# fdrmrc/fictitious_domain_AL_preconditioners

Hardware: AMD Instinct MI355X
Metric: FGMRES iterations/sec to 1e-8 residual, 3D Stokes-immersed (AL-preconditioned) (higher is better)
Workload: dtype f64

## Files before the change

### fictitious_domain_al_preconditioners_amd/_abi.py

```python
import ctypes as C

ALFD_MAX_BLOCKS = 3

OK, E_INVALID, E_HIP, E_NO_CONVERGENCE_OUTER, E_NO_CONVERGENCE_INNER, E_BREAKDOWN, E_NOT_SETUP, \
    E_COMM, E_UNSUPPORTED = range(9)
A, BT, B, CT, C_, M, MP, A2, KIMM = range(9)
NSLOTS = 9
SLOT_BY_NAME = {"A": A, "Bt": BT, "B": B, "Ct": CT, "C": C_, "M": M, "Mp": MP, "A2": A2, "K": KIMM}
INVW, MP_LUMPED_INV = 0, 1
NDIAGS = 2
AL2, AL_STOKES, AL_STOKES_DIAG, AL_ELL_IDEAL, AL_ELL_MODIFIED, RATIONAL = range(6)
CTRL_ABS, CTRL_REDUCTION, CTRL_FIXED_ITERS = range(3)
PREC_IDENTITY, PREC_JACOBI, PREC_CHEBYSHEV, PREC_MULTILEVEL = range(4)
INNER_OP_AUG, INNER_OP_A22, INNER_OP_AUG2 = range(3)
SPECTRUM_CCT = 0
ORTH_MGS, ORTH_CGS, ORTH_CGS2 = range(3)
OUTER_FGMRES, OUTER_MINRES = range(2)
FGMRES_DEALII_96, FGMRES_DEALII_95 = range(2)
W_DIAGONAL, W_MASS_INV_SQUARED, W_MASS_INV = range(3)
INNER_THROW, INNER_ACCEPT = range(2)
T_SPMV_A, T_SPMV_OTHER, T_DOT, T_VEC = range(4)
T_NCLASSES = 4
SC_PRODUCTS_A, SC_PRODUCTS_C, SC_LEVEL_A_UPLOADS, SC_TRANSFER_UPLOADS, SC_PATCH_BUILDS, SC_POWER_ITERATIONS = range(6)
SC_NCOUNTS = 6
# ... 32 lines not shown
class Result(C.Structure):
    _fields_ = [
        ("status", C.c_int32), ("outer_iterations", C.c_int32),
        ("initial_residual", C.c_double), ("last_residual", C.c_double),
        ("inner_iterations", C.c_int64), ("mp_iterations", C.c_int64),
        ("inner_failures", C.c_int32), ("precond_applications", C.c_int32),
        ("solve_seconds", C.c_double), ("lambda_max", C.c_double),
        ("rational_iterations", C.c_int64), ("mass_iterations", C.c_int64),
    ]

    def as_dict(self):
        return {k: getattr(self, k) for k, _ in self._fields_}


class Spectrum(C.Structure):
    _fields_ = [
        ("converged", C.c_int32), ("steps", C.c_int32),
        ("initial_residual", C.c_double), ("last_residual", C.c_double),
        ("lambda_min", C.c_double), ("lambda_max", C.c_double), ("condition", C.c_double),
    ]

    def as_dict(self):
        return {k: getattr(self, k) for k, _ in self._fields_}


class MatrixInfo(C.Structure):
    _fields_ = [
        ("lanes", C.c_int32), ("windowed", C.c_int32), ("value_indexed", C.c_int32), ("batch_major", C.c_int32),
        ("nnz", C.c_int64), ("window_blocks", C.c_int64), ("window_fallback_blocks", C.c_int64),
        ("value_indexed_blocks", C.c_int64), ("value_indexed_nnz", C.c_int64),
        ("dictionary_entries", C.c_int64), ("value_wide_nnz", C.c_int64),
        ("algorithmic_bytes", C.c_double), ("streamed_bytes", C.c_double),
        ("shared_nnz", C.c_int64), ("batch_major_blocks", C.c_int64), ("batch_major_wide", C.c_int64),
        ("batch_major_interior_blocks", C.c_int64),
    ]


SPMV_PLAIN, SPMV_SPARSE_ROWS, SPMV_STREAM, SPMV_WINDOW, SPMV_WINDOW_VI, SPMV_WINDOW_VIB, SPMV_WINDOW_GROUP, \
    SPMV_BATCH_MAJOR, SPMV_BATCH_MAJOR_SHORT, SPMV_PLAIN_F32, SPMV_STREAM_F32, SPMV_WINDOW_F32 = range(12)
SPMV_NFAMILIES = 12
SPMV_FAMILY_NAMES = ("plain", "sparse_rows", "stream", "window", "window_vi", "window_vib", "window_group",
                     "batch_major", "batch_major_short", "plain_f32", "stream_f32", "window_f32")


class SpmvLaunch(C.Structure):
    _fields_ = [
        ("family", C.c_int32), ("lanes", C.c_int32), ("R", C.c_int32), ("U", C.c_int32), ("nontemporal", C.c_int32),
        ("epilogue", C.c_int32), ("xcd_order", C.c_int32),
        ("grid", C.c_int64), ("lds_bytes", C.c_int64),
    ]

    def as_dict(self):
        return {k: getattr(self, k) for k, _ in self._fields_}


class BatchMajorShape(C.Structure):
    _fields_ = [
        ("batch_major", C.c_int32), ("lanes", C.c_int32),
        ("nrows", C.c_int64), ("nnz", C.c_int64), ("shared_nnz", C.c_int64),
        ("rows", C.c_int64), ("waves", C.c_int64), ("small", C.c_int64),
        ("blocks", C.c_int64), ("batches", C.c_int64), ("lds_bytes", C.c_int64), ("compute_units", C.c_int64),
    ]

    def as_dict(self):
        plain = ("batch_major", "lanes", "nrows", "nnz", "shared_nnz")
        return {(k if k in plain else "batch_major_" + k): getattr(self, k) for k, _ in self._fields_}


PREC_VALUES_FP64, PREC_VALUES_FP32 = range(2)
PREC_VALUES_BY_NAME = {"fp64": PREC_VALUES_FP64, "fp32": PREC_VALUES_FP32}
PV_NONE, PV_NOT_REQUESTED, PV_NO_MATRIX, PV_SHORT_ROWS, PV_SPARSE_ROWS, PV_DICTIONARY_FORM, PV_PARTITIONED, \
    PV_OUT_OF_RANGE, PV_NOT_APPLIED = range(9)
PREC_VALUES_REASON_NAMES = ("none", "not_requested", "no_matrix", "short_rows", "sparse_rows", "dictionary_form",
                            "partitioned", "out_of_range", "not_applied")
PREC_VALUES_FAMILY_NAMES = ("plain", "stream", "window")


class PrecValuesInfo(C.Structure):
    _fields_ = [
        ("requested", C.c_int32), ("stored", C.c_int32), ("used", C.c_int32), ("reason", C.c_int32),
        ("family", C.c_int32), ("reserved", C.c_int32),
        ("nnz", C.c_int64), ("flushed_to_zero", C.c_int64), ("copy_bytes", C.c_int64),
        ("streamed_bytes_fp64", C.c_double), ("streamed_bytes_fp32", C.c_double),
    ]


OPERATOR_LEVEL, OPERATOR_PATCH_SS, OPERATOR_PATCH_S = 0, 1, 2


class WindowPlanInfo(C.Structure):
    _fields_ = [
        ("windowed", C.c_int32), ("value_indexed", C.c_int32), ("row_block", C.c_int32), ("max_window", C.c_int32),
        ("blocks", C.c_int64), ("fallback_blocks", C.c_int64), ("segments", C.c_int64),
        ("value_indexed_blocks", C.c_int64), ("value_indexed_nnz", C.c_int64), ("value_wide_nnz", C.c_int64),
        ("dictionary_entries", C.c_int64), ("batches", C.c_int64), ("decode_mismatches", C.c_int64),
    ]


class StreamPlanInfo(C.Structure):
    _fields_ = [
        ("ok", C.c_int32), ("max_window", C.c_int32), ("max_rows", C.c_int32), ("max_batches", C.c_int32),
        ("blocks", C.c_int64), ("batches", C.c_int64), ("segments", C.c_int64), ("dictionary_entries", C.c_int64),
        ("stream_bytes", C.c_int64), ("decode_mismatches", C.c_int64), ("rows_covered", C.c_int64),
        ("shared_nnz", C.c_int64),
    ]

# ... 44 lines not shown
```

### fictitious_domain_al_preconditioners_amd/csrc/alfd.hip

```cpp

#include <hip/hip_runtime.h>
#include <rccl/rccl.h>

#include <algorithm>
#include <atomic>
#include <chrono>
#include <cmath>
#include <cstdio>
#include <cstdlib>
#include <cstring>
#include <memory>
#include <climits>
#include <condition_variable>
#include <functional>
#include <limits>
#include <mutex>
#include <string>
#include <thread>
#include <unordered_set>
#include <vector>

#include "alfd/alfd.h"
#include "kernels.hpp"
#include "kernels_vs.hpp"
// ... 7 lines not shown
    if (e__ != hipSuccess) {                                                                \
      ctx->err = std::string(#call) + ": " + hipGetErrorString(e__) + " (" + __FILE__ + ":" + \
                 std::to_string(__LINE__) + ")";                                            \
      return ALFD_E_HIP;                                                                    \
    }                                                                                       \
  } while (0)
#define RC(call)                  \
  do {                            \
    int rc__ = (call);            \
    if (rc__ != ALFD_OK) return rc__; \
  } while (0)

static inline int64_t pad_chunk(int64_t n) { return (n + kChunk - 1) / kChunk * kChunk; }

struct DevCsr {
  bool present = false;
  int64_t nrows = 0, ncols = 0, nnz = 0;
  int64_t n_list = 0;
  bool sparse = false;
  bool rep = false;
  bool derived = false;
  int L = 64;
  int32_t n_local_cols = 0;
  int64_t *rp = nullptr;
  int32_t *col = nullptr;
  double *val = nullptr;
  int32_t *rows = nullptr;
  std::vector<int64_t> send_off, recv_off;
  std::vector<int32_t> halo_globals;
  int32_t *send_idx = nullptr;
  double *send_buf = nullptr, *halo = nullptr;
  int64_t n_halo = 0;
  std::vector<void *> owned;
  bool win = false;
  bool win_deferred = false, win_user = true;
  int tag = 0;
  int32_t win_RB = 0, win_maxW = 0;
  int64_t win_nblocks = 0, win_fallback_blocks = 0, win_nseg = 0;
  uint16_t *lcol = nullptr;
  bool vi = false;
  uint8_t *vidx = nullptr;
  int32_t *blk_dict_off = nullptr, *blk_dict_n = nullptr;
  double *dict = nullptr;
  int64_t vi_blocks = 0, vi_nnz = 0, vi_dict_total = 0, vi_wide_nnz = 0;
  uint16_t *vidw = nullptr;
  uint64_t *vib_tab = nullptr;
  int32_t *vib_cnt = nullptr;
  int32_t vib_stride = 0;
  int32_t *blk_seg_begin = nullptr, *blk_W = nullptr, *seg_col = nullptr, *seg_off = nullptr;
  struct Vs {
    bool on = false, bricks = false;
    int64_t nb = 0, nseg = 0, stream_bytes = 0, nbatch = 0, dict_total = 0, shared_nnz = 0;
    int32_t stride = 0, maxW = 0;
    int32_t L = 64, tab_u64 = 16;
    int32_t wide = 0;
    int32_t RB = 0, NW = 4;
    bool small = false;
    uint8_t *stream = nullptr;
    int64_t *sb = nullptr;
    uint64_t *tab = nullptr;
    int32_t *cnt = nullptr, *seg_begin = nullptr, *blkW = nullptr, *seg_col = nullptr,
            *seg_off = nullptr, *doff = nullptr, *dn = nullptr;
    int32_t *hdrb = nullptr, *segx = nullptr;
    int32_t seg_stride = 0;
    int64_t nb_interior = 0;
    double *dict = nullptr;
  } vs;
  double streamed_bytes(bool use_vi, bool use_vs = false) const {
    const double vec = (double)(n_list + 1) * 8.0 + (double)n_list * 8.0 + (double)(sparse ? n_list : ncols) * 8.0;
    if (vs.on && use_vs && use_vi)
      return (double)vs.stream_bytes + 8.0 * vs.tab_u64 * (double)vs.nbatch + 28.0 * (double)vs.nb +
             8.0 * (double)vs.nseg + 8.0 * (double)vs.dict_total + 8.0 * (double)nrows +
             8.0 * (double)(sparse ? n_list : ncols);
    if (!win) return (double)nnz * 12.0 + vec;
    const double meta = (double)win_nblocks * 8.0 + (double)win_nseg * 8.0;
    if (!(vi && use_vi)) return (double)nnz * 10.0 + vec + meta;
    return (double)(vi_nnz - vi_wide_nnz) * 3.0 + (double)vi_wide_nnz * 4.0 + (double)(nnz - vi_nnz) * 10.0 + vec + meta + (double)vi_dict_total * 8.0 +
           (double)win_nblocks * (8.0 + (vib_tab ? 32.0 * vib_stride + 4.0 : 0.0));
  }
  float *val32 = nullptr;
  int64_t val32_flushed = 0;
  double streamed_bytes32() const {
    const double vec = (double)(n_list + 1) * 8.0 + (double)n_list * 8.0 + (double)ncols * 8.0;
    if (!win) return (double)nnz * 8.0 + vec;
    return (double)nnz * 6.0 + vec + (double)win_nblocks * 8.0 + (double)win_nseg * 8.0;
  }
  double algorithmic_bytes() const {
    return (double)nnz * 12.0 + (double)(n_list + 1) * 8.0 + (double)n_list * 8.0 +
           (double)(sparse ? n_list : ncols) * 8.0;
  }
};

struct HostCsr {
  int64_t nrows = 0, ncols = 0;
  std::vector<int64_t> rp;
  std::vector<int32_t> col;
  std::vector<double> val;
  int64_t nnz() const { return rp.empty() ? 0 : rp.back(); }
};

constexpr int kScratchSlot = ALFD_NSLOTS;

struct LevelStore {
  DevCsr A, C, Ct;
  DevCsr P, R;
  int64_t n = 0, npad = 0;
  double *dinv = nullptr, *r = nullptr, *z = nullptr, *t = nullptr, *cd = nullptr, *cres = nullptr, *ctmp = nullptr;
};

struct MlLevel {
  LevelStore loc, rep;
  double lmax = 0;
  uint8_t *tail_mask = nullptr;
  bool P_global_cols = false;
  std::vector<int64_t> offs;
  int64_t maxpiece = 0;
  double *send = nullptr, *stage = nullptr;
};

enum State { ITERATE = 0, SUCCESS = 1, FAILURE = 2 };
struct Control {
  alfd_control c;
  double initial = 0, reduced_tol = 0, last_value = 0;
  int last_step = 0;
  State check(int step, double v) {
    last_step = step;
    last_value = v;
    if (step == 0) {
      initial = v;
      reduced_tol = v * c.reduce;
    }
    if (c.kind == ALFD_CTRL_REDUCTION && v < reduced_tol) return SUCCESS;
    if (c.kind == ALFD_CTRL_FIXED_ITERS && step >= c.max_steps) return SUCCESS;
    if (v <= c.tol) return SUCCESS;
    if (step >= c.max_steps || std::isnan(v)) return FAILURE;
    return ITERATE;
  }
};

struct TimedLaunch {
  int cls;
  hipEvent_t a, b;
};

}

using namespace alfd;

struct alfd_ctx {
  int device = 0;
  hipStream_t stream = nullptr;
  hipStream_t xstream = nullptr;
  hipEvent_t ev_x = nullptr, ev_halo = nullptr;
  hipEvent_t ev_in = nullptr;
  int overlap_halo = -1;
  std::string err;
  int rank = 0, nranks = 1;
  ncclComm_t nccl = nullptr;
  struct alfd_local_group *local = nullptr;
  alfd_host_allgather_fn host_allgather = nullptr;
  alfd_host_alltoallv_fn host_alltoallv = nullptr;
  void *host_user = nullptr;
  std::vector<char> host_send, host_recv;
  std::vector<std::vector<int64_t>> part;
  int nblocks = 0;
  int64_t n[ALFD_MAX_BLOCKS] = {0, 0, 0};
// ... 30 lines not shown
    DevCsr own_Cs, own_Cts;
    DevCsr *Cs = nullptr, *Cts = nullptr;
    int64_t m = 0;
    double *t = nullptr, *ones = nullptr, *x = nullptr, *coef = nullptr, *linf = nullptr;
    int64_t coef_cap = 0;
    std::vector<void *> owned;
    std::vector<double> alpha, beta;
    bool have = false;
  } spec;
  int spec_group = 16;
  int spec_host_stepped = 0;
  HostCsr h_M, h_K;
  struct Hierarchy {
    std::vector<int32_t> agg[ALFD_MAX_LEVELS];
    std::vector<double> wgt[ALFD_MAX_LEVELS];
    int64_t ncoarse[ALFD_MAX_LEVELS] = {0, 0, 0, 0, 0, 0, 0, 0};
    HostCsr P[ALFD_MAX_LEVELS];
    DevCsr inv;
    HostCsr coarse_A, coarse_C, coarse_Ct;
    std::vector<MlLevel> ml;
    TailTable *tail_tab = nullptr;
    bool built_partitioned = false;
    void clear_input() {
      for (int l = 0; l < ALFD_MAX_LEVELS; ++l) agg[l].clear(), wgt[l].clear(), P[l] = HostCsr(), ncoarse[l] = 0;
      built_partitioned = false;
    }
  } hier[2];
  struct Patch {
    bool on = false;
    int64_t m = 0, mpad = 0;
    DevCsr Ass, As, Ats, Cs, Cts;
    int32_t *S = nullptr;
    double *dinv = nullptr, *rS = nullptr, *zS = nullptr, *uS = nullptr, *eS = nullptr, *cd = nullptr,
           *cres = nullptr, *ctmp = nullptr, *rr = nullptr;
    double lmax = 0;
    uint8_t *tail_mask = nullptr;
    bool rep = false;
    int64_t m_loc = 0, piece = 1, lam_piece = 1;
    std::vector<int64_t> soff;
    DevCsr Cts_loc, Ctg;
    double *send = nullptr, *stage = nullptr, *lam_send = nullptr, *lam_stage = nullptr, *loc = nullptr;
  } patch;
  struct StrengthGraph {
    bool have = false, on_device = false;
    int64_t n_nodes = 0, node0 = 0;
    std::vector<int64_t> gp;
    std::vector<int32_t> gc, fixed;
    std::vector<double> gw, d;
  } sg;
  int ml_rep_level = -1;
  bool dots_replicated = false;
  int64_t ml_rep_threshold = 300000;
  int ml_fuse = 2;
  int ml_tail_rows = 0;
  int ml_gpu_galerkin = 1;
  double *g_w = nullptr, *g_tlam = nullptr;
  std::vector<int64_t> ml_coff[ALFD_MAX_LEVELS];
  const int64_t *up_col_offsets = nullptr;
  bool up_local_only = false;
  DevCsr rat_mat;
  double *rt_r = nullptr, *rt_z = nullptr, *rt_p = nullptr, *rt_Ap = nullptr, *rt_x = nullptr;
  double *rt_dinv = nullptr, *rt_partial = nullptr, *rt_scb = nullptr, *rt_coef = nullptr;
  double *rt_scb_host = nullptr;
  int64_t rational_its = 0;
  int64_t wmax = 0;
  std::vector<void *> ws_allocs;
  double *w_r = nullptr, *w_z = nullptr, *w_p = nullptr, *w_Ap = nullptr;
  double *c_d = nullptr, *c_res = nullptr, *c_tmp = nullptr;
  double *t_lam = nullptr;
  double *q_tmp = nullptr, *rhs_tmp = nullptr;
  double *V = nullptr, *Z = nullptr, *xb = nullptr, *bb = nullptr, *io = nullptr;
  double *st_in = nullptr, *st_out = nullptr;
  double lambda_max = 0, lambda_min = 0;
  int64_t inner_its = 0, mp_its = 0;
  int64_t inner_its_op[3] = {0, 0, 0};
  int inner_failures = 0, precond_applications = 0;
  std::vector<double> history;
  int timing = 0;
  std::vector<TimedLaunch> timed;
  double t_ms[ALFD_T_NCLASSES] = {0, 0, 0, 0};
  int64_t t_launches[ALFD_T_NCLASSES] = {0, 0, 0, 0};
  double t_bytes[ALFD_T_NCLASSES] = {0, 0, 0, 0};
  double t_fbytes[ALFD_T_NCLASSES] = {0, 0, 0, 0};
  double setup_s[ALFD_SETUP_NPHASES] = {0, 0, 0, 0, 0, 0, 0, 0};
  bool upload_since_setup = false;
  uint64_t gen[ALFD_NSLOTS + 1] = {}, gen_setup[ALFD_NSLOTS + 1] = {};
  uint64_t dgen[ALFD_NDIAGS] = {}, dgen_setup[ALFD_NDIAGS] = {};
  alfd_config cfg_setup;
  const char *needs_full = nullptr;
  bool coupling_ready = false;
  int64_t setup_counts[ALFD_SC_NCOUNTS] = {};
  std::vector<void *> cp_allocs[2];
  std::vector<void *> allocs;
  int spmv_stream_R = 2, spmv_stream_U = 8, spmv_nt = 0, spmv_grid_mult = 8;
  int spmv_group_R = 4, spmv_group_U = 4;
  bool vi_off = false;
  int vi_rows_R = 4, vi_rows_J = 2;
  int vi_xcd = 0;
  int vi_levels = 1;
  int vi_batched = 1;
  int win_RB_vi = 96;
  int win_vi = 1;
  int win_short_scale = 2;
  int vs_enable = 1, vs_NW = 4, vs_RB = 96, vs_xcd = 0, vs_share = 1, vs_wide = 1;
  int vs_small = 1;
  int vs_cus = 0;
// ... 463 lines not shown
  const DevCsr::Vs &v = m.vs;
  const size_t lds = (size_t)kVsWinOff + (size_t)v.maxW * sizeof(double);
#define ALFD_VSS(EPI, TAG)                                                                                            \
  do {                                                                                                                \
    note_spmv(ctx, ALFD_SPMV_BATCH_MAJOR_SHORT, L, 0, 0, false, EPI, 0, v.nb, lds);                                   \
    hipLaunchKernelGGL((spmv_vss_kernel<L, EPI, TAG>), dim3((unsigned)v.nb), dim3(256), lds, ctx->stream, v.stream, \
                       v.sb, v.tab, v.cnt, v.stride, v.seg_begin, v.blkW, v.seg_col, v.seg_off, v.doff, v.dn, v.dict, \
                       x, m.halo, m.n_local_cols, y, alpha, d, y2);                                                   \
  } while (0)
  if (m.tag == 0) {
    if (epi == 0) ALFD_VSS(0, 0);
    else if (epi == 1) ALFD_VSS(1, 0);
    else if (epi == 2) ALFD_VSS(2, 0);
    else ALFD_VSS(3, 0);
  } else {
    if (epi == 0) ALFD_VSS(0, 1);
    else if (epi == 1) ALFD_VSS(1, 1);
    else if (epi == 2) ALFD_VSS(2, 1);
    else ALFD_VSS(3, 1);
  }
#undef ALFD_VSS
}

static bool vs_lds_base_ok(alfd_ctx *ctx) {
  if (ctx->vs_lds_base_ok < 0) {
    uint32_t *probe = nullptr, base = 1;
    if (hipMalloc((void **)&probe, sizeof(uint32_t)) == hipSuccess) {
      hipLaunchKernelGGL(vs_lds_base_probe_kernel, dim3(1), dim3(64), 4096, ctx->stream, probe);
      hipMemcpyAsync(&base, probe, sizeof(uint32_t), hipMemcpyDeviceToHost, ctx->stream);
      hipStreamSynchronize(ctx->stream);
      hipFree(probe);
    }
    ctx->vs_lds_base_ok = base == 0 ? 1 : 0;
    if (!ctx->vs_lds_base_ok)
      std::fprintf(stderr, "[alfd] dynamic LDS does not start at offset 0 (%u): batch-major SpMV formats disabled\n", base);
  }
  return ctx->vs_lds_base_ok != 0;
}

static bool launch_vs(alfd_ctx *ctx, const DevCsr &m, const double *x, double *y, int epi, double alpha,
                      const double *d, double *y2, int64_t first_block = 0, int64_t n_blocks = -1) {
  const DevCsr::Vs &v = m.vs;
  if (!vs_lds_base_ok(ctx)) return false;
  if (v.L == 32) return launch_vss<32>(ctx, m, x, y, epi, alpha, d, y2), true;
  if (v.L == 16) return launch_vss<16>(ctx, m, x, y, epi, alpha, d, y2), true;
  if (v.L == 8) return launch_vss<8>(ctx, m, x, y, epi, alpha, d, y2), true;
  const int NW = v.NW;
  const size_t lds = (size_t)(v.wide ? VsFmt<1>::kWinOff : VsFmt<0>::kWinOff) + (size_t)v.maxW * sizeof(double);
  if (n_blocks < 0) n_blocks = v.nb - first_block;
  if (n_blocks <= 0) return true;
  const unsigned grid = (unsigned)n_blocks;
  const int32_t base = (int32_t)first_block;
#define ALFD_VS_ARGS \
  v.stream, v.tab, v.stride, v.hdrb, v.segx, v.seg_stride, v.dict, x, m.halo, m.n_local_cols, y, alpha, d, y2, ctx->vs_xcd, base, NoPair()
#define ALFD_VS(EPI, NWV)                                                                                        \
  do {                                                                                                           \
    if (v.wide) {                                   \
      note_spmv(ctx, ALFD_SPMV_BATCH_MAJOR, 64, 4, 1, false, EPI, ctx->vs_xcd, grid, lds);                       \
      hipLaunchKernelGGL((spmv_vs_kernel<EPI, 0, 4, 1>), dim3(grid), dim3(256), lds, ctx->stream,     \
                         ALFD_VS_ARGS);                                                                          \
    } else if (m.tag == 0) {                                                                                     \
      note_spmv(ctx, ALFD_SPMV_BATCH_MAJOR, 64, NWV, 0, false, EPI, ctx->vs_xcd, grid, lds);                     \
      hipLaunchKernelGGL((spmv_vs_kernel<EPI, 0, NWV>), dim3(grid), dim3(64 * NWV), lds, ctx->stream, \
                         ALFD_VS_ARGS);                                                                          \
    } else {   \
      note_spmv(ctx, ALFD_SPMV_BATCH_MAJOR, 64, (NWV > 4 ? 4 : NWV), 0, false, EPI, ctx->vs_xcd, grid, lds);     \
      hipLaunchKernelGGL((spmv_vs_kernel<EPI, 1, (NWV > 4 ? 4 : NWV)>), dim3(grid), dim3(64 * (NWV > 4 ? 4 : NWV)), lds, \
                         ctx->stream, ALFD_VS_ARGS);                                                             \
    }                                                                                                            \
  } while (0)
#define ALFD_VS_E(NWV)                  \
  do {                                  \
    if (epi == 0) ALFD_VS(0, NWV);      \
    else if (epi == 1) ALFD_VS(1, NWV); \
    else if (epi == 2) ALFD_VS(2, NWV); \
    else ALFD_VS(3, NWV);               \
  } while (0)
  if (NW == 8) ALFD_VS_E(8);
  else if (NW == 2) ALFD_VS_E(2);
  else if (NW == 1) ALFD_VS_E(1);
  else ALFD_VS_E(4);
#undef ALFD_VS_E
#undef ALFD_VS
#undef ALFD_VS_ARGS
  return true;
}

static int halo_exchange(alfd_ctx *ctx, DevCsr &m, const double *x, hipStream_t st = nullptr);
static int spmv_launch_local(alfd_ctx *ctx, DevCsr &m, const double *x, double *y, int epi, double alpha, const double *d,
                             double *y2);

static int spmv_m(alfd_ctx *ctx, DevCsr &m, int cls, const double *x, double *y, int epi, double alpha = 0.0,
                  const double *d = nullptr, double *y2 = nullptr) {
  if (!m.present) return ctx->err = "matrix not set", ALFD_E_NOT_SETUP;
  if (a32_active(ctx, m)) {
    if (m.n_list == 0) return ALFD_OK;
    Timer tm(ctx, cls, m.algorithmic_bytes(), m.streamed_bytes32());
    return spmv_launch_a32(ctx, m, x, y, epi, alpha);
  }
  const bool exchange = ctx->nranks > 1 && !m.rep && (ctx->local || ctx->host_alltoallv || m.n_halo > 0 || m.send_off.back() > 0);
  const bool overlap = exchange && (ctx->overlap_halo > 0 || (ctx->overlap_halo < 0 && (ctx->local || ctx->host_alltoallv))) && ctx->xstream && m.vs.on && m.vs.L == 64 && ctx->vs_enable && !ctx->vi_off &&
                       m.vs.nb_interior > 0 && !m.sparse && m.n_list > 0;
  if (overlap) {
    Timer tm(ctx, cls, m.algorithmic_bytes(), m.streamed_bytes(true, true));
    HIPC(hipEventRecord(ctx->ev_x, ctx->stream));
    if (!launch_vs(ctx, m, x, y, epi, alpha, d, y2, 0, m.vs.nb_interior)) return ctx->err = "batch-major launch failed", ALFD_E_HIP;
    HIPC(hipStreamWaitEvent(ctx->xstream, ctx->ev_x, 0));
// ... 141 lines not shown
                                          c.variant == ALFD_AL_STOKES_DIAG || c.variant == ALFD_AL_ELL_MODIFIED);
  ctx->a32_reason = ctx->a32_used ? ALFD_PREC_VALUES_NONE : ALFD_PREC_VALUES_NOT_APPLIED;
}

static int spmv(alfd_ctx *ctx, int slot, const double *x, double *y, int epi, double alpha = 0.0,
                const double *d = nullptr, double *y2 = nullptr) {
  DevCsr &m = ctx->mat[slot];
  if (!m.present) return ctx->err = "matrix slot " + std::to_string(slot) + " not set", ALFD_E_NOT_SETUP;
  return spmv_m(ctx, m, slot == ALFD_A ? ALFD_T_SPMV_A : ALFD_T_SPMV_OTHER, x, y, epi, alpha, d, y2);
}

static bool tail_form(const DevCsr &m) { return m.present && !m.vs.on && !m.win; }


static int pair_form_A(alfd_ctx *ctx, const DevCsr &A) {
  if (!A.present || A.sparse || A.n_list == 0) return 0;
  if (a32_active(ctx, A)) return 0;
  if (A.vs.on && ctx->vs_enable && !ctx->vi_off)
    return A.vs.L == 64 && !A.vs.wide && A.vs.NW <= 4 && A.vs.nb > 0 && vs_lds_base_ok(ctx) ? 1 : 0;
  if (A.win) return 0;
  return A.L == 64 && ctx->spmv_stream_R == 2 && ctx->spmv_stream_U == 8 && !ctx->spmv_nt ? 2 : 0;
}

static inline bool gd_nested(const alfd_ctx *ctx);
static int pair_forms(alfd_ctx *ctx, const DevCsr &A, const DevCsr &C) {
  const bool ok = ctx->nranks == 1 && ctx->cfg.w_inverse == ALFD_W_DIAGONAL && !ctx->cfg.aug_assembled && !gd_nested(ctx) &&
                  tail_form(C) && !C.sparse && C.nrows > 0 && (C.L == 16 || C.L == 32 || C.L == 64) && A.ncols == C.ncols;
  return ok ? pair_form_A(ctx, A) : 0;
}
static int pair_ok(alfd_ctx *ctx, const DevCsr &A, const DevCsr &C) {
  const bool fine = &A == &ctx->mat[ALFD_A] || &A == &ctx->mat[ALFD_A2];
  return ctx->ml_fuse >= (fine ? 3 : 2) ? pair_forms(ctx, A, C) : 0;
}

static int launch_pair(alfd_ctx *ctx, int form, const DevCsr &A, int clsA, const DevCsr &C, const double *w,
                       const double *x, double *y, double *t) {
  const bool vi = !ctx->vi_off, vs = ctx->vs_enable != 0 && !ctx->vi_off;
  Timer tm(ctx, clsA, A.algorithmic_bytes() + C.algorithmic_bytes(), A.streamed_bytes(vi, vs) + C.streamed_bytes(vi, vs));
  PairC pc;
  pc.nrows = C.n_list, pc.rp = C.rp, pc.col = C.col, pc.val = C.val, pc.x_halo = C.halo, pc.d = w, pc.t = t;
  pc.n_local = C.n_local_cols, pc.L = C.L;
  pc.nC = (uint32_t)grid_for_rows(C.n_list, C.L);
  if (form == 1) {
    const DevCsr::Vs &v = A.vs;
    const size_t lds = (size_t)VsFmt<0>::kWinOff + (size_t)v.maxW * sizeof(double);
    pc.nA = (uint32_t)v.nb;
    const int64_t rpb = 64 * v.NW / C.L;
    pc.nC = (uint32_t)std::max<int64_t>(1, std::min<int64_t>((C.n_list + rpb - 1) / rpb, 256 * 8));
#define ALFD_VS_PAIR(TAG, NWV)                                                                                               \
  do {                                                                                                                       \
    note_spmv(ctx, ALFD_SPMV_BATCH_MAJOR, 64, NWV, 0, false, 0, ctx->vs_xcd, (int64_t)pc.nA + pc.nC, lds);                   \
    hipLaunchKernelGGL((spmv_vs_kernel<0, TAG, NWV, 0, true>), dim3(pc.nA + pc.nC), dim3(64 * NWV), lds, ctx->stream,       \
                       v.stream, v.tab, v.stride, v.hdrb, v.segx, v.seg_stride, v.dict, x, A.halo, A.n_local_cols, y, 0.0,  \
                       (const double *)nullptr, (double *)nullptr, ctx->vs_xcd, 0, pc);                                      \
  } while (0)
#define ALFD_VS_PAIR_T(TAG)              \
  do {                                   \
    if (v.NW == 1) ALFD_VS_PAIR(TAG, 1); \
    else if (v.NW == 2) ALFD_VS_PAIR(TAG, 2); \
    else ALFD_VS_PAIR(TAG, 4);           \
  } while (0)
    if (A.tag == 0) ALFD_VS_PAIR_T(0);
    else ALFD_VS_PAIR_T(1);
#undef ALFD_VS_PAIR_T
#undef ALFD_VS_PAIR
  } else {
    const int64_t nbatches = (A.nrows + 1) / 2;
    pc.nA = (uint32_t)std::max<int64_t>(1, std::min<int64_t>((nbatches + 3) / 4, 256 * ctx->spmv_grid_mult));
    note_spmv(ctx, ALFD_SPMV_STREAM, 64, 2, 8, false, 0, 0, (int64_t)pc.nA + pc.nC, 0);
    hipLaunchKernelGGL((spmv_stream_kernel<2, 8, 0, false, true>), dim3(pc.nA + pc.nC), dim3(kBlock), 0, ctx->stream,
                       A.nrows, A.rp, A.col, A.val, x, A.halo, A.n_local_cols, y, 0.0, (const double *)nullptr,
                       (double *)nullptr, pc);
  }
  HIPC(hipGetLastError());
  return ALFD_OK;
}

static int spmv_AC(alfd_ctx *ctx, DevCsr &A, int clsA, DevCsr &C, const double *w, const double *x, double *y, double *t) {
  if (const int form = pair_ok(ctx, A, C)) return launch_pair(ctx, form, A, clsA, C, w, x, y, t);
  RC(spmv_m(ctx, A, clsA, x, y, 0));
  return spmv_m(ctx, C, ALFD_T_SPMV_OTHER, x, t, 2, 0.0, w);
}

static int finish_dots(alfd_ctx *ctx, int64_t nb, int count, int out, int fin) {
  if (ctx->nranks == 1 || ctx->dots_replicated) {
    hipLaunchKernelGGL(dot_final_kernel, dim3(count), dim3(kBlock), 0, ctx->stream, ctx->partial, nb,
                       ctx->pstride, ctx->sc, out, fin);
    HIPC(hipGetLastError());
    return ALFD_OK;
  }
  hipLaunchKernelGGL(dot_final_kernel, dim3(count), dim3(kBlock), 0, ctx->stream, ctx->partial, nb,
                     ctx->pstride, ctx->sc, (int)S_STAGE, (int)FIN_STORE);
  HIPC(hipGetLastError());
  RC(comm_allgather(ctx, ctx->sc + S_STAGE, ctx->gather, (size_t)count * sizeof(double)));
  const int tgt = fin == FIN_STORE ? out : (int)S_TMP;
  hipLaunchKernelGGL(rank_sum_kernel, dim3(1), dim3(64), 0, ctx->stream, ctx->gather, ctx->nranks, count,
                     ctx->sc, tgt);
  if (fin != FIN_STORE) {
    hipLaunchKernelGGL(dot_final_kernel, dim3(1), dim3(kBlock), 0, ctx->stream, ctx->sc + S_TMP,
                       (int64_t)1, (int64_t)0, ctx->sc, out, fin);
  }
  HIPC(hipGetLastError());
  return ALFD_OK;
}

static int dot_async(alfd_ctx *ctx, int64_t npad, const double *x, const double *y, int out,
                     int fin = FIN_STORE) {
// ... 1998 lines not shown
  const int64_t nlc = (ctx->nranks > 1 && !m.rep) ? (int64_t)m.n_local_cols : -1;
  bool hint = slot >= 0 && slot < ALFD_NSLOTS && !ctx->rb_ptr[slot].empty();
  if (hint && ctx->rb_ptr[slot].back() != m.nrows) {
    if (ctx->cfg.log_level > 0)
      std::fprintf(stderr, "[alfd] row-block hint of slot %d dropped: it lists %lld rows, the matrix has %lld\n", slot,
                   (long long)ctx->rb_ptr[slot].back(), (long long)m.nrows);
    ctx->rb_ptr[slot].clear();
    ctx->rb_rows[slot].clear();
    hint = false;
  }
  if (hint) {
    const auto &bp = ctx->rb_ptr[slot];
    const auto &br = ctx->rb_rows[slot];
    bool good = bp.front() == 0 && bp.back() == m.nrows && (int64_t)br.size() == m.nrows;
    std::vector<uint8_t> seen(good ? m.nrows : 0, 0);
    for (size_t i = 0; good && i < br.size(); ++i) {
      good = br[i] >= 0 && br[i] < m.nrows && !seen[br[i]];
      if (good) seen[br[i]] = 1;
    }
    for (size_t i = 0; good && i + 1 < bp.size(); ++i) good = bp[i] <= bp[i + 1];
    if (!good) return ctx->err = "alfd_set_row_blocks: the blocks are not a partition of the matrix rows", ALFD_E_INVALID;
    plan_vs(m.nrows, rp, col, val, RB, ctx->win_maxW, ctx->win_gap, (int64_t)bp.size() - 1, bp.data(),
            br.data(), pl, ctx->vs_share != 0, 0, nlc);
  } else {
    plan_vs(m.nrows, rp, col, val, RB, ctx->win_maxW, ctx->win_gap, 0, nullptr, nullptr, pl, ctx->vs_share != 0, 0, nlc);
  }
  if (ctx->vs_wide && (!pl.ok || pl.dict_split)) {
    VsPlan pw;
    if (hint)
      plan_vs(m.nrows, rp, col, val, RB, ctx->win_maxW, ctx->win_gap, (int64_t)ctx->rb_ptr[slot].size() - 1,
              ctx->rb_ptr[slot].data(), ctx->rb_rows[slot].data(), pw, ctx->vs_share != 0, 1, nlc);
    else
      plan_vs(m.nrows, rp, col, val, RB, ctx->win_maxW, ctx->win_gap, 0, nullptr, nullptr, pw, ctx->vs_share != 0, 1, nlc);
    if (pw.ok && (!pl.ok || pw.stream.size() + 128 * (size_t)pw.nbatch < pl.stream.size() + 128 * (size_t)pl.nbatch)) pl = std::move(pw);
  }
  if (!pl.ok) return ALFD_OK;
  bool small = false;
  if (ctx->vs_small && !forced && !hint && slot == kScratchSlot && !pl.wide) {
    int rs = RB, ws = NW;
    vs_small_shape(m.nrows, pl.nb, pl.nbatch, RB, NW, ctx->vs_cus, &rs, &ws);
    if (rs != RB || ws != NW) {
      VsPlan ps;
      plan_vs(m.nrows, rp, col, val, rs, ctx->win_maxW, ctx->win_gap, 0, nullptr, nullptr, ps, ctx->vs_share != 0, 0, nlc);
      if (ps.ok && !ps.dict_split) {
        pl = std::move(ps);
        RB = rs, NW = ws, small = true;
      }
    }
  }
  DevCsr::Vs &v = m.vs;
  v.RB = RB;
  v.NW = pl.wide ? 4 : NW;
  v.small = small;
  int32_t max_nseg = 0;
  for (int64_t b = 0; b < pl.nb; ++b) max_nseg = std::max(max_nseg, pl.seg_begin[b + 1] - pl.seg_begin[b]);
  const int32_t S = std::max(max_nseg + 1, 33);
  if ((double)pl.nb * S * 8.0 > 2.0e9) return ALFD_OK;
  std::vector<int32_t> hdrb((size_t)pl.nb * 8, 0), segx((size_t)pl.nb * S * 2 + 16, 0);
  for (int64_t b = 0; b < pl.nb; ++b) {
    const int32_t s0 = pl.seg_begin[b], ns = pl.seg_begin[b + 1] - s0;
    int32_t *h = &hdrb[(size_t)b * 8];
    h[0] = pl.cnt[b];
    h[1] = pl.blkW[b];
    h[2] = ns;
    h[3] = pl.dn[b];
    h[4] = pl.doff[b];
    h[5] = (int32_t)(uint32_t)((uint64_t)pl.sb[b] & 0xffffffffull);
    h[6] = (int32_t)((uint64_t)pl.sb[b] >> 32);
    for (int32_t q = 0; q < ns; ++q) {
      segx[((size_t)b * S + q) * 2] = pl.seg_col[s0 + q];
      segx[((size_t)b * S + q) * 2 + 1] = pl.seg_off[s0 + q];
    }
  }
  pl.tab.resize(pl.tab.size() + (size_t)16 * kVsBatchRows, 0);
  RC(upload_vec(ctx, m, &v.stream, pl.stream));
  RC(upload_vec(ctx, m, &v.tab, pl.tab));
  RC(upload_vec(ctx, m, &v.hdrb, hdrb));
  RC(upload_vec(ctx, m, &v.segx, segx));
  RC(upload_vec(ctx, m, &v.dict, pl.dict));
  HIPC(hipStreamSynchronize(ctx->stream));
  v.seg_stride = S;
  v.nb_interior = pl.nb_interior;
  v.nb = pl.nb;
  v.nseg = (int64_t)pl.seg_col.size();
  v.stream_bytes = (int64_t)pl.stream.size() - 4096;
  v.nbatch = pl.nbatch;
  v.shared_nnz = pl.shared_nnz;
  v.dict_total = (int64_t)pl.dict.size();
  v.stride = pl.stride;
  v.maxW = pl.maxW;
  v.wide = pl.wide;
  v.bricks = hint;
  v.on = true;
  if (ctx->cfg.log_level > 0)
    std::fprintf(stderr,
                 "[alfd] batch-major format%s: %lld blocks (%s), %lld batches, window <= %d slots, %.2f B/nnz, %.1f %% of the "
                 "entries in template-shared batches\n", pl.wide ? " (10-bit codes)" : "",
                 (long long)pl.nb, hint ? "caller's row blocks" : "runs of the numbering", (long long)pl.nbatch, pl.maxW,
                 (double)v.stream_bytes / (double)std::max<int64_t>(m.nnz, 1),
                 100.0 * (double)pl.shared_nnz / (double)std::max<int64_t>(m.nnz, 1));
  return ALFD_OK;
}

static int build_vss(alfd_ctx *ctx, DevCsr &m, const int64_t *rp, const int32_t *col, const double *val) {
  VsPlan pl;
  const int RB = std::min(kVssMaxRows, std::max(64, ctx->win_RB * std::max(1, ctx->win_short_scale) * 64 / m.L));
  plan_vss(m.nrows, m.L, rp, col, val, RB, ctx->win_maxW, ctx->win_gap, pl);
  if (!pl.ok || pl.shared_nnz * 2 < m.nnz) return ALFD_OK;
  DevCsr::Vs &v = m.vs;
  RC(upload_vec(ctx, m, &v.stream, pl.stream));
  RC(upload_vec(ctx, m, &v.sb, pl.sb));
  RC(upload_vec(ctx, m, &v.tab, pl.tab));
  RC(upload_vec(ctx, m, &v.cnt, pl.cnt));
  RC(upload_vec(ctx, m, &v.seg_begin, pl.seg_begin));
  RC(upload_vec(ctx, m, &v.blkW, pl.blkW));
  RC(upload_vec(ctx, m, &v.seg_col, pl.seg_col));
  RC(upload_vec(ctx, m, &v.seg_off, pl.seg_off));
  RC(upload_vec(ctx, m, &v.doff, pl.doff));
  RC(upload_vec(ctx, m, &v.dn, pl.dn));
  RC(upload_vec(ctx, m, &v.dict, pl.dict));
  HIPC(hipStreamSynchronize(ctx->stream));
  v.nb = pl.nb;
  v.nseg = (int64_t)pl.seg_col.size();
  v.stream_bytes = (int64_t)pl.stream.size() - 4096;
  v.nbatch = pl.nbatch;
  v.shared_nnz = pl.shared_nnz;
  v.dict_total = (int64_t)pl.dict.size();
  v.stride = pl.stride;
  v.maxW = pl.maxW;
  v.L = m.L;
  v.tab_u64 = 1 + 4 * (64 / m.L);
  v.bricks = false;
  v.on = true;
  if (ctx->cfg.log_level > 0)
    std::fprintf(stderr, "[alfd] batch-major format (L = %d): %lld blocks, %lld batches, window <= %d slots, %.2f B/nnz, "
                 "%.1f %% of the entries in shared batches\n", m.L, (long long)pl.nb, (long long)pl.nbatch, pl.maxW,
                 (double)(v.stream_bytes + 8.0 * v.tab_u64 * v.nbatch) / (double)std::max<int64_t>(m.nnz, 1),
                 100.0 * (double)pl.shared_nnz / (double)std::max<int64_t>(m.nnz, 1));
  return ALFD_OK;
}

static int upload_matrix(alfd_ctx *ctx, int slot, int64_t nrows, int64_t ncols, const int64_t *rp,
                         const int32_t *col, const double *val) {
  DevCsr &m = ctx->mat[slot];
  csr_free(m);
  const auto t_up0 = std::chrono::steady_clock::now();
// ... 427 lines not shown
              marker[J] = (int64_t)row.size();
              row.emplace_back(J, c);
            } else {
              row[marker[J]].second = row[marker[J]].second + c;
            }
          }
        }
        for (auto &e : row) marker[e.first] = -1;
        std::sort(row.begin(), row.end(), [](const auto &a, const auto &b) { return a.first < b.first; });
        t_cnt[t].push_back((int64_t)row.size());
        for (auto &e : row) {
          t_col[t].push_back(e.first);
          t_val[t].push_back(e.second);
        }
      }
    });
  for (auto &x : th) x.join();
  out.nrows = n_rows_c;
  out.ncols = n_cols_c;
  out.rp.assign(1, 0);
  out.col.clear();
  out.val.clear();
  for (int t = 0; t < T; ++t) {
    for (int64_t c : t_cnt[t]) out.rp.push_back(out.rp.back() + c);
    out.col.insert(out.col.end(), t_col[t].begin(), t_col[t].end());
    out.val.insert(out.val.end(), t_val[t].begin(), t_val[t].end());
  }
}

static int upload_matrix(alfd_ctx *ctx, int slot, int64_t nrows, int64_t ncols, const int64_t *rp,
                         const int32_t *col, const double *val);
static int upload_level(alfd_ctx *ctx, DevCsr &dst, const HostCsr &h) {
  static const int32_t no_col = 0;
  static const double no_val = 0;
  RC(upload_matrix(ctx, kScratchSlot, h.nrows, h.ncols, h.rp.data(), h.col.empty() ? &no_col : h.col.data(),
                   h.val.empty() ? &no_val : h.val.data()));
  csr_free(dst);
  dst = std::move(ctx->mat[kScratchSlot]);
  ctx->mat[kScratchSlot] = DevCsr();
  dst.tag = 1;
  return ALFD_OK;
}

struct AugOp {
  DevCsr *A = nullptr, *C = nullptr, *Ct = nullptr;
  int clsA = ALFD_T_SPMV_OTHER;
  const double *w = nullptr;
  double gamma = 0;
  double *tlam = nullptr;
  const uint8_t *mask = nullptr;
  int64_t npad = 0;
  const double *dinv = nullptr;
  double *cd = nullptr, *cres = nullptr, *ctmp = nullptr;
  double lmax = 0;
};

struct LevelView {
  AugOp op;
  double *r = nullptr, *z = nullptr, *t = nullptr;
  DevCsr *R = nullptr, *P = nullptr;
  double *rc = nullptr, *zc = nullptr;
};

static LevelView level_view(alfd_ctx *ctx, int h, int l) {
  MlLevel &L = ctx->hier[h].ml[l];
  const bool rep = h == 0 && ctx->ml_rep_level >= 0 && l >= ctx->ml_rep_level;
  LevelStore &S = rep ? L.rep : L.loc;
  LevelView V;
  AugOp &F = V.op;
  F.A = l > 0 ? &S.A : &ctx->mat[h == 0 ? ALFD_A : ALFD_A2];
  F.C = l > 0 ? &S.C : &ctx->mat[h == 0 ? ALFD_C : ALFD_M];
  F.Ct = l > 0 ? &S.Ct : &ctx->mat[h == 0 ? ALFD_CT : ALFD_M];
  F.clsA = l == 0 && h == 0 ? ALFD_T_SPMV_A : ALFD_T_SPMV_OTHER;
  F.w = rep ? ctx->g_w : ctx->diag[ALFD_INVW];
  F.gamma = h == 0 ? ctx->cfg.gamma : ctx->cfg.gamma2;
  F.tlam = rep ? ctx->g_tlam : ctx->t_lam;
  F.mask = L.tail_mask;
  F.npad = S.npad;
  F.dinv = S.dinv;
  F.cd = S.cd, F.cres = S.cres, F.ctmp = S.ctmp;
  F.lmax = L.lmax;
  V.r = S.r, V.z = S.z, V.t = S.t;
  if (l + 1 < (int)ctx->hier[h].ml.size()) {
    MlLevel &M = ctx->hier[h].ml[l + 1];
    LevelStore &N = rep ? M.rep : M.loc;
    V.R = &N.R, V.P = &N.P;
    V.rc = N.r, V.zc = N.z;
  }
  return V;
}

static AugOp patch_aug(alfd_ctx *ctx) {
  alfd_ctx::Patch &Q = ctx->patch;
  AugOp F;
  F.A = &Q.Ass, F.C = &Q.Cs, F.Ct = &Q.Cts;
  F.w = Q.rep ? ctx->g_w : ctx->diag[ALFD_INVW];
  F.tlam = Q.rep ? ctx->g_tlam : ctx->t_lam;
  F.gamma = ctx->cfg.gamma;
  F.mask = Q.tail_mask;
  F.npad = Q.mpad;
  F.dinv = Q.dinv;
  F.cd = Q.cd, F.cres = Q.cres, F.ctmp = Q.ctmp;
  F.lmax = Q.lmax;
  return F;
}

static int fused_AC(alfd_ctx *ctx, const AugOp &F, const double *x, double *y) {
  return spmv_AC(ctx, *F.A, F.clsA, *F.C, F.w, x, y, F.tlam);
}

static int aug_apply(alfd_ctx *ctx, const AugOp &F, const double *x, double *y) {
  if (ctx->cfg.aug_assembled) return spmv_m(ctx, *F.A, F.clsA, x, y, 0);
  RC(fused_AC(ctx, F, x, y));
  return spmv_m(ctx, *F.Ct, ALFD_T_SPMV_OTHER, F.tlam, y, 1, F.gamma);
}

static int aug_lambda_max(alfd_ctx *ctx, const AugOp &F, int64_t n, int64_t goff, double *v, double *wv, double *lmax) {
  if (n > 0)
    hipLaunchKernelGGL(hash_vector_kernel, dim3((unsigned)((n + 255) / 256)), dim3(256), 0, ctx->stream, n, goff, v);
  double lam = 0;
  RC(power_lambda(ctx, F.npad, F.dinv, v, wv, [&](const double *x, double *y) { return aug_apply(ctx, F, x, y); }, &lam));
  *lmax = lam * ctx->cfg.cheb_safety;
  HIPC(hipMemsetAsync(v, 0, F.npad * sizeof(double), ctx->stream));
  HIPC(hipMemsetAsync(wv, 0, F.npad * sizeof(double), ctx->stream));
  return ALFD_OK;
}


static bool plain_form(const alfd_ctx *ctx, const DevCsr &m) {
  return m.present && !m.vs.on && !m.win && !(m.L == 64 && !m.sparse && ctx->spmv_stream_R > 0);
}

static bool fused_ok(const alfd_ctx *ctx, const AugOp &F) {
  return ctx->ml_fuse && ctx->nranks == 1 && !ctx->cfg.aug_assembled && !gd_nested(ctx) &&
         ctx->cfg.w_inverse == ALFD_W_DIAGONAL && F.mask && F.A->present && F.C->present && plain_form(ctx, *F.Ct);
}

static int aug_tail(alfd_ctx *ctx, const AugOp &F, int mode, const AugTailArgs &p, double vec_bytes) {
  const DevCsr &m = *F.Ct;
  const int nb_rows = m.n_list > 0 ? grid_for_rows(m.n_list, m.L) : 0;
  const unsigned grid = (unsigned)nb_rows + (unsigned)(F.npad / kChunk);
  if (grid == 0) return ALFD_OK;
  Timer tm(ctx, ALFD_T_SPMV_OTHER, m.algorithmic_bytes() + vec_bytes * (double)F.npad,
           m.streamed_bytes(false) + vec_bytes * (double)F.npad);
#define ALFD_TAIL(LL, MM)                                                                                         \
  hipLaunchKernelGGL((aug_tail_kernel<LL, MM>), dim3(grid), dim3(kBlock), 0, ctx->stream, m.n_list, m.rp, m.col,  \
                     m.val, m.sparse ? m.rows : (const int32_t *)nullptr, F.tlam, nb_rows, F.mask, p)
#define ALFD_TAIL_L(LL)                                      \
  switch (mode) {                                            \
    case TAIL_STEP: ALFD_TAIL(LL, TAIL_STEP); break;         \
    case TAIL_LAST: ALFD_TAIL(LL, TAIL_LAST); break;         \
    case TAIL_LAST_ADD: ALFD_TAIL(LL, TAIL_LAST_ADD); break; \
    case TAIL_RES: ALFD_TAIL(LL, TAIL_RES); break;           \
    case TAIL_RES_INIT: ALFD_TAIL(LL, TAIL_RES_INIT); break; \
    default: ALFD_TAIL(LL, TAIL_RES_INIT_ADD); break;        \
  }
  switch (m.L) {
    case 4: ALFD_TAIL_L(4) break;
    case 8: ALFD_TAIL_L(8) break;
    case 16: ALFD_TAIL_L(16) break;
    case 32: ALFD_TAIL_L(32) break;
    default: ALFD_TAIL_L(64) break;
  }
#undef ALFD_TAIL_L
#undef ALFD_TAIL
  HIPC(hipGetLastError());
  return ALFD_OK;
}

static int cheb_fused(alfd_ctx *ctx, const AugOp &F, int degree, double ratio, const double *r, double *z, double *zout,
                      bool have_init) {
  ChebCoef k(F.lmax, ratio);
  if (!have_init) VEC_LAUNCH(cheb_init_z_kernel, F.npad, 24, 1.0 / k.theta, F.dinv, r, z);
  for (int j = 1; j < degree; ++j) {
    RC(fused_AC(ctx, F, j == 1 ? z : F.cd, F.ctmp));
    AugTailArgs p;
    k.step(p.c1, p.c2);
    p.gamma = F.gamma;
    p.dinv = F.dinv, p.y = F.ctmp, p.rin = j == 1 ? r : F.cres, p.din = j == 1 ? z : F.cd;
    p.res = F.cres, p.d = F.cd, p.z = z, p.zout = zout;
    const bool last = j == degree - 1;
    RC(aug_tail(ctx, F, !last ? TAIL_STEP : zout ? TAIL_LAST_ADD : TAIL_LAST, p, last && zout ? 88.0 : 64.0));
  }
  HIPC(hipGetLastError());
  return ALFD_OK;
}

static int aug_cheb(alfd_ctx *ctx, const AugOp &F, int degree, double ratio, const double *r, double *z) {
  if (fused_ok(ctx, F)) return cheb_fused(ctx, F, degree, ratio, r, z, nullptr, false);
  return cheb_sweep(ctx, F.npad, F.dinv, F.lmax, ratio, degree, F.cd, F.cres, F.ctmp, r, z,
                    [&](const double *x, double *y) { return aug_apply(ctx, F, x, y); });
}

static int fused_residual(alfd_ctx *ctx, const AugOp &F, const double *r, double *t) {
  AugTailArgs p;
  p.gamma = F.gamma, p.y = t, p.rin = r, p.res = t;
  return aug_tail(ctx, F, TAIL_RES, p, 24.0);
}

static int fused_correct(alfd_ctx *ctx, const AugOp &F, int degree, double ratio, const double *r, double *t, double *zc,
                         double *zout) {
  AugTailArgs p;
  p.gamma = F.gamma, p.c1 = 1.0 / ChebCoef(F.lmax, ratio).theta;
  p.dinv = F.dinv, p.y = t, p.rin = r, p.res = t, p.z = zc, p.zout = zout;
  p.store_res = degree > 1;
  if (degree <= 1 && zout) return aug_tail(ctx, F, TAIL_RES_INIT_ADD, p, 24.0 + 32.0 + 24.0);
  RC(aug_tail(ctx, F, TAIL_RES_INIT, p, 24.0 + (degree > 1 ? 40.0 : 32.0)));
  return cheb_fused(ctx, F, degree, ratio, t, zc, zout, true);
}

static int build_tail_mask(alfd_ctx *ctx, int h, const DevCsr &m, int64_t npad, uint8_t **mask) {
  *mask = nullptr;
  if (ctx->nranks > 1 || !m.present || npad == 0 || m.nrows > npad) return ALFD_OK;
  double *q = nullptr;
  RC(cp_alloc_zero(ctx, h, &q, npad / 8));
  *mask = reinterpret_cast<uint8_t *>(q);
  if (m.n_list > 0)
    hipLaunchKernelGGL(mark_rows_kernel, dim3((unsigned)((m.n_list + 255) / 256)), dim3(256), 0, ctx->stream, m.n_list,
                       m.sparse ? m.rows : (const int32_t *)nullptr, *mask);
  HIPC(hipGetLastError());
  return ALFD_OK;
}

static_assert(kTailMaxLevels == ALFD_MAX_LEVELS + 1, "TailTable holds every level of a hierarchy");

static TailCsr tail_csr(const DevCsr &m) {
  TailCsr t;
  t.rp = m.rp, t.col = m.col, t.val = m.val, t.rows = m.sparse ? m.rows : nullptr;
  t.n_list = m.n_list, t.nrows = m.nrows;
  t.L = m.L, t.sparse = m.sparse ? 1 : 0;
  return t;
}

static int build_tail_table(alfd_ctx *ctx) {
  const alfd_config &c = ctx->cfg;
  alfd_ctx::Hierarchy &H = ctx->hier[1];
  const int last = (int)H.ml.size() - 1;
  std::vector<TailTable> tab(1);
  TailTable &T = tab[0];
  std::memset(&T, 0, sizeof(T));
  T.nlev = last + 1;
  T.has_inv = H.inv.present ? 1 : 0;
  if (H.inv.present) T.inv = tail_csr(H.inv);
  for (int l = 1; l <= last; ++l) {
    const LevelView V = level_view(ctx, 1, l);
    TailLevel &F = T.lev[l];
    F.A = tail_csr(*V.op.A), F.C = tail_csr(*V.op.C), F.Ct = tail_csr(*V.op.Ct);
    if (l < last) F.R = tail_csr(*V.R), F.P = tail_csr(*V.P);
    F.dinv = V.op.dinv, F.w = V.op.w, F.tlam = V.op.tlam;
    F.r = V.r, F.z = V.z, F.t = V.t, F.cd = V.op.cd, F.cres = V.op.cres, F.ctmp = V.op.ctmp;
    F.gamma = V.op.gamma, F.npad = V.op.npad;
    F.degree = l == last ? c.ml_coarse_degree : c.ml_smooth_degree_coarse > 0 ? c.ml_smooth_degree_coarse : c.ml_smooth_degree;
    ChebCoef k(V.op.lmax, l == last ? c.ml_coarse_ratio : c.ml_smooth_ratio);
    F.inv_theta = 1.0 / k.theta;
    for (int j = 1; j < F.degree && j <= kTailMaxDegree; ++j) k.step(F.c1[j - 1], F.c2[j - 1]);
  }
  double *q = nullptr;
  RC(cp_alloc_zero(ctx, 1, &q, (int64_t)((sizeof(TailTable) + 7) / 8)));
  H.tail_tab = reinterpret_cast<TailTable *>(q);
  HIPC(hipMemcpyAsync(H.tail_tab, &T, sizeof(TailTable), hipMemcpyHostToDevice, ctx->stream));
  HIPC(hipStreamSynchronize(ctx->stream));
// ... 1 lines not shown
}

static bool tail_ok(alfd_ctx *ctx, int l, const double *r, const double *z) {
  const alfd_config &c = ctx->cfg;
  alfd_ctx::Hierarchy &H = ctx->hier[1];
  const int last = (int)H.ml.size() - 1;
  if (!H.tail_tab || l < 1 || H.ml[l].loc.n > ctx->ml_tail_rows || r != H.ml[l].loc.r || z != H.ml[l].loc.z) return false;
  if (ctx->nranks != 1 || c.aug_assembled || c.w_inverse != ALFD_W_DIAGONAL) return false;
  const int sdeg = c.ml_smooth_degree_coarse > 0 ? c.ml_smooth_degree_coarse : c.ml_smooth_degree;
  if (sdeg - 1 > kTailMaxDegree || (!H.inv.present && c.ml_coarse_degree - 1 > kTailMaxDegree)) return false;
  if (H.inv.present && !tail_form(H.inv)) return false;
  for (int j = l; j <= last; ++j) {
    const LevelStore &L = H.ml[j].loc;
    if (!tail_form(L.A) || !tail_form(L.C) || !tail_form(L.Ct)) return false;
    if (j > l && (!tail_form(L.R) || !tail_form(L.P))) return false;
  }
  return true;
}

static int allgather_pieces(alfd_ctx *ctx, const double *mine, const std::vector<int64_t> &offs, int64_t piece, double *send,
                            double *stage, double *whole) {
  const int64_t n_me = offs[ctx->rank + 1] - offs[ctx->rank];
  if (n_me > 0) HIPC(hipMemcpyAsync(send, mine, n_me * sizeof(double), hipMemcpyDeviceToDevice, ctx->stream));
  RC(comm_allgather(ctx, send, stage, (size_t)piece * sizeof(double)));
  for (int p = 0; p < ctx->nranks; ++p) {
    const int64_t np = offs[p + 1] - offs[p];
    if (np > 0)
      HIPC(hipMemcpyAsync(whole + offs[p], stage + (int64_t)p * piece, np * sizeof(double), hipMemcpyDeviceToDevice, ctx->stream));
  }
  return ALFD_OK;
}

static int ml_cycle(alfd_ctx *ctx, int h, int l, const double *r, double *z) {
  const alfd_config &c = ctx->cfg;
  alfd_ctx::Hierarchy &H = ctx->hier[h];
  const int last = (int)H.ml.size() - 1;
  if (h == 1 && ctx->ml_tail_rows > 0 && tail_ok(ctx, l, r, z)) {
    Timer tm(ctx, ALFD_T_SPMV_OTHER, 0.0);
    hipLaunchKernelGGL(ml_tail_kernel, dim3(1), dim3(kTailBlock), 0, ctx->stream, H.tail_tab, l);
    HIPC(hipGetLastError());
    return ALFD_OK;
  }
  const LevelView L = level_view(ctx, h, l);
  const AugOp &F = L.op;
  const A32Scope a32(ctx, h == 0 && l == 0 && ctx->a32_used);
  if (l == last) {
    if (H.inv.present) return spmv_m(ctx, H.inv, ALFD_T_SPMV_OTHER, r, z, 0);
    return aug_cheb(ctx, F, c.ml_coarse_degree, c.ml_coarse_ratio, r, z);
  }
  const int sdeg = l > 0 && c.ml_smooth_degree_coarse > 0 ? c.ml_smooth_degree_coarse : c.ml_smooth_degree;
  const bool fuse = fused_ok(ctx, F);
  RC(aug_cheb(ctx, F, sdeg, c.ml_smooth_ratio, r, z));
  if (fuse) {
    RC(fused_AC(ctx, F, z, L.t));
    RC(fused_residual(ctx, F, r, L.t));
  } else {
    RC(aug_apply(ctx, F, z, L.t));
    VEC_LAUNCH(sub_from_kernel, F.npad, 24, r, L.t);
  }
  RC(spmv_m(ctx, *L.R, ALFD_T_SPMV_OTHER, L.t, L.rc, 0));
  if (h == 0 && l + 1 == ctx->ml_rep_level) {
    MlLevel &N = H.ml[l + 1];
    RC(allgather_pieces(ctx, N.loc.r, N.offs, N.maxpiece, N.send, N.stage, N.rep.r));
    RC(ml_cycle(ctx, h, l + 1, N.rep.r, N.rep.z));
    RC(spmv_m(ctx, N.loc.P, ALFD_T_SPMV_OTHER, N.P_global_cols ? N.rep.z : N.rep.z + N.offs[ctx->rank], z, 1, 1.0));
  } else {
    RC(ml_cycle(ctx, h, l + 1, L.rc, L.zc));
    RC(spmv_m(ctx, *L.P, ALFD_T_SPMV_OTHER, L.zc, z, 1, 1.0));
  }
  if (fuse) {
    RC(fused_AC(ctx, F, z, L.t));
    RC(fused_correct(ctx, F, sdeg, c.ml_smooth_ratio, r, L.t, L.r, z));
    return ALFD_OK;
  }
  RC(aug_apply(ctx, F, z, L.t));
  VEC_LAUNCH(sub_from_kernel, F.npad, 24, r, L.t);
  RC(aug_cheb(ctx, F, sdeg, c.ml_smooth_ratio, L.t, L.r));
  VEC_LAUNCH(axpy_kernel, F.npad, 24, (const double *)nullptr, 0, 1.0, L.r, z);
  HIPC(hipGetLastError());
  return ALFD_OK;
}

static int ml_apply_rep(alfd_ctx *ctx, const double *r, double *z) {
  alfd_ctx::Patch &Q = ctx->patch;
  const int64_t n0p = pad_chunk(ctx->n[0]);
  const unsigned gm = (unsigned)std::max<int64_t>(1, (Q.m_loc + 255) / 256);
  const bool pen = !ctx->cfg.aug_assembled;
  const int last = ctx->nblocks - 1;
  const int64_t s0 = Q.soff[ctx->rank];
  const AugOp F = patch_aug(ctx);
  const int pdeg = ctx->cfg.ml_patch_degree;
  const double pratio = ctx->cfg.ml_patch_ratio;
  if (Q.m_loc > 0) hipLaunchKernelGGL(gather_kernel, dim3(gm), dim3(256), 0, ctx->stream, Q.m_loc, Q.S, r, Q.loc);
  RC(allgather_pieces(ctx, Q.loc, Q.soff, Q.piece, Q.send, Q.stage, Q.rS));
  RC(aug_cheb(ctx, F, pdeg, pratio, Q.rS, Q.zS));
  VEC_LAUNCH(scale_copy_kernel, n0p, 16, 1.0, r, Q.rr);
  RC(spmv_m(ctx, Q.Ats, ALFD_T_SPMV_OTHER, Q.zS, Q.rr, 1, -1.0));
  if (pen) {
    RC(spmv_m(ctx, Q.Cs, ALFD_T_SPMV_OTHER, Q.zS, ctx->g_tlam, 2, 0.0, ctx->g_w));
    RC(spmv_m(ctx, Q.Ctg, ALFD_T_SPMV_OTHER, ctx->g_tlam, Q.rr, 1, -ctx->cfg.gamma));
  }
  RC(ml_cycle(ctx, 0, 0, Q.rr, z));
  if (Q.m_loc > 0) hipLaunchKernelGGL(scatter_add_kernel, dim3(gm), dim3(256), 0, ctx->stream, Q.m_loc, Q.S, Q.zS + s0, z);
  RC(spmv_m(ctx, Q.As, ALFD_T_SPMV_OTHER, z, Q.loc, 0));
  if (pen) {
    RC(spmv(ctx, ALFD_C, z, ctx->t_lam, 2, 0.0, ctx->diag[ALFD_INVW]));
    RC(allgather_pieces(ctx, ctx->t_lam, ctx->part[last], Q.lam_piece, Q.lam_send, Q.lam_stage, ctx->g_tlam));
    RC(spmv_m(ctx, Q.Cts_loc, ALFD_T_SPMV_OTHER, ctx->g_tlam, Q.loc, 1, ctx->cfg.gamma));
  }
  RC(allgather_pieces(ctx, Q.loc, Q.soff, Q.piece, Q.send, Q.stage, Q.uS));
  VEC_LAUNCH(sub_from_kernel, Q.mpad, 24, Q.rS, Q.uS);
  RC(aug_cheb(ctx, F, pdeg, pratio, Q.uS, Q.eS));
  if (Q.m_loc > 0) hipLaunchKernelGGL(scatter_add_kernel, dim3(gm), dim3(256), 0, ctx->stream, Q.m_loc, Q.S, Q.eS + s0, z);
  HIPC(hipGetLastError());
  return ALFD_OK;
}

static int ml_apply(alfd_ctx *ctx, const double *r, double *z) {
  alfd_ctx::Patch &Q = ctx->patch;
  if (!Q.on) return ml_cycle(ctx, 0, 0, r, z);
  if (Q.rep) return ml_apply_rep(ctx, r, z);
  const int64_t n0p = pad_chunk(ctx->n[0]);
  const unsigned gm = (unsigned)((Q.m + 255) / 256);
  const bool pen = !ctx->cfg.aug_assembled;
  const double *w = ctx->diag[ALFD_INVW];
  const AugOp F = patch_aug(ctx);
  const int pdeg = ctx->cfg.ml_patch_degree;
  const double pratio = ctx->cfg.ml_patch_ratio;
  hipLaunchKernelGGL(gather_kernel, dim3(gm), dim3(256), 0, ctx->stream, Q.m, Q.S, r, Q.rS);
  RC(aug_cheb(ctx, F, pdeg, pratio, Q.rS, Q.zS));
  VEC_LAUNCH(scale_copy_kernel, n0p, 16, 1.0, r, Q.rr);
  RC(spmv_m(ctx, Q.Ats, ALFD_T_SPMV_OTHER, Q.zS, Q.rr, 1, -1.0));
  if (pen) {
    RC(spmv_m(ctx, Q.Cs, ALFD_T_SPMV_OTHER, Q.zS, ctx->t_lam, 2, 0.0, w));
    RC(spmv(ctx, ALFD_CT, ctx->t_lam, Q.rr, 1, -ctx->cfg.gamma));
  }
  RC(ml_cycle(ctx, 0, 0, Q.rr, z));
  hipLaunchKernelGGL(scatter_add_kernel, dim3(gm), dim3(256), 0, ctx->stream, Q.m, Q.S, Q.zS, z);
  if (pen) RC(spmv_AC(ctx, Q.As, ALFD_T_SPMV_OTHER, ctx->mat[ALFD_C], w, z, Q.uS, ctx->t_lam));
  else RC(spmv_m(ctx, Q.As, ALFD_T_SPMV_OTHER, z, Q.uS, 0));
  if (fused_ok(ctx, F)) {
    RC(fused_correct(ctx, F, pdeg, pratio, Q.rS, Q.uS, Q.eS, nullptr));
  } else {
    if (pen) RC(spmv_m(ctx, Q.Cts, ALFD_T_SPMV_OTHER, ctx->t_lam, Q.uS, 1, ctx->cfg.gamma));
    VEC_LAUNCH(sub_from_kernel, Q.mpad, 24, Q.rS, Q.uS);
    RC(aug_cheb(ctx, F, pdeg, pratio, Q.uS, Q.eS));
  }
  hipLaunchKernelGGL(scatter_add_kernel, dim3(gm), dim3(256), 0, ctx->stream, Q.m, Q.S, Q.eS, z);
  HIPC(hipGetLastError());
  return ALFD_OK;
}

static void spgemm_host(const HostCsr &A, const HostCsr &Pm, HostCsr &out) {
  const int64_t nrows = A.nrows, nc = Pm.ncols;
  const int T = (int)std::max<int64_t>(1, std::min<int64_t>(std::min(16u, std::max(1u, std::thread::hardware_concurrency())),
                                                           (nrows + 4095) / 4096));
  std::vector<std::vector<int32_t>> t_cnt(T), t_col(T);
  std::vector<std::vector<double>> t_val(T);
  std::vector<std::thread> th;
  for (int t = 0; t < T; ++t)
    th.emplace_back([&, t]() {
      const int64_t i0 = nrows * t / T, i1 = nrows * (t + 1) / T;
      std::vector<int64_t> stamp(nc, -1);
      std::vector<double> acc(nc, 0.0);
      std::vector<int32_t> touched;
      t_cnt[t].reserve(i1 - i0);
      for (int64_t i = i0; i < i1; ++i) {
        touched.clear();
        for (int64_t k = A.rp[i]; k < A.rp[i + 1]; ++k) {
          const double a = A.val[k];
          const int64_t j = A.col[k];
          for (int64_t e = Pm.rp[j]; e < Pm.rp[j + 1]; ++e) {
            const int32_t J = Pm.col[e];
            if (stamp[J] != i) {
              stamp[J] = i;
              acc[J] = std::fma(a, Pm.val[e], 0.0);
              touched.push_back(J);
            } else {
              acc[J] = std::fma(a, Pm.val[e], acc[J]);
            }
          }
        }
        std::sort(touched.begin(), touched.end());
        t_cnt[t].push_back((int32_t)touched.size());
        for (int32_t J : touched) {
          t_col[t].push_back(J);
          t_val[t].push_back(acc[J]);
        }
      }
    });
  for (auto &x : th) x.join();
  out.nrows = nrows;
  out.ncols = nc;
  out.rp.assign(1, 0);
  out.rp.reserve(nrows + 1);
// ... 1971 lines not shown
    RC(upload_level_part(ctx, Nx.R, R, nullptr, true));
    ctx->setup_counts[ALFD_SC_PRODUCTS_A] += 2;
    ctx->setup_counts[ALFD_SC_PRODUCTS_C]++;
    ctx->setup_counts[ALFD_SC_LEVEL_A_UPLOADS]++;
    ctx->setup_counts[ALFD_SC_TRANSFER_UPLOADS] += 2;
    if (rep_from > 0 && l + 1 >= rep_from) {
      stash[l + 1].A = An;
      stash[l + 1].C = Cn;
      stash[l + 1].Ct = Ctn;
      stash[l + 1].P = P;
      stash[l + 1].R = R;
    }
    if (l + 1 < nlev) {
      RC(download_csr(ctx, Nx.A, A));
      RC(download_csr(ctx, Nx.C, C));
      RC(download_csr(ctx, Nx.Ct, Ct));
    }
  }
  if (c.ml_coarse_direct > 0 && ctx->hier[0].ml[nlev].loc.n > 0 && ctx->hier[0].ml[nlev].loc.n <= c.ml_coarse_direct) {
    alfd_ctx::Hierarchy &H = ctx->hier[0];
    if (full) H.coarse_A = std::move(An);
    if (full || c_changed) H.coarse_C = std::move(Cn), H.coarse_Ct = std::move(Ctn);
    std::vector<double> w(ctx->n[last]);
    HIPC(hipMemcpyAsync(w.data(), ctx->diag[ALFD_INVW], w.size() * sizeof(double), hipMemcpyDeviceToHost, ctx->stream));
    HIPC(hipStreamSynchronize(ctx->stream));
    PhaseClock pc(ctx, ALFD_SETUP_ML_COARSE);
    RC(coarse_inverse(ctx, H.coarse_A, H.coarse_C, H.coarse_Ct, w, c.gamma, H.inv));
  }
  if (rep_from > 0) {
    const int64_t lam_pad = pad_chunk(lam_global);
    RC(ws_alloc_zero(ctx, &ctx->g_w, lam_pad));
    RC(ws_alloc_zero(ctx, &ctx->g_tlam, lam_pad));
    RC(gather_vec(ctx, ctx->diag[ALFD_INVW], ctx->n[last], ctx->g_w));
    for (int l = rep_from; l <= nlev; ++l) {
      MlLevel &L = ctx->hier[0].ml[l];
      const int64_t n_all = off[l].back();
      HostCsr wholeA, wholeC, wholeCt, g;
      RC(gather_csr(ctx, stash[l].A, nullptr, n_all, wholeA));
      RC(gather_csr(ctx, stash[l].C, nullptr, n_all, wholeC));
      RC(gather_csr(ctx, stash[l].Ct, nullptr, lam_global, wholeCt));
      RC(replicate_level(ctx, l, wholeA, wholeC, wholeCt, off[l], l == rep_from));
      if (l > rep_from) {
        RC(gather_csr(ctx, stash[l].P, off[l].data(), n_all, g));
        RC(upload_level_part(ctx, L.rep.P, g, nullptr, true));
        RC(gather_csr(ctx, stash[l].R, off[l - 1].data(), off[l - 1].back(), g));
        RC(upload_level_part(ctx, L.rep.R, g, nullptr, true));
        L.rep.P.rep = L.rep.R.rep = true;
      }
      RC(gather_vec(ctx, L.loc.dinv, L.loc.n, L.rep.dinv));
    }
    ctx->ml_rep_level = rep_from;
  }
  for (int l = 0; l <= nlev; ++l)
    RC(build_tail_mask(ctx, 0, l == 0 ? ctx->mat[ALFD_CT] : ctx->hier[0].ml[l].loc.Ct, ctx->hier[0].ml[l].loc.npad, &ctx->hier[0].ml[l].tail_mask));
  return ALFD_OK;
}

static int ml_setup_immersed(alfd_ctx *ctx, bool full, bool c_changed) {
  const alfd_config &c = ctx->cfg;
  alfd_ctx::Hierarchy &H = ctx->hier[1];
  int nlev = 0;
  H.tail_tab = nullptr;
  while (nlev < ALFD_MAX_LEVELS && !H.P[nlev].rp.empty()) ++nlev;
  if (nlev == 0) return ALFD_OK;
  if (!is_elliptic(c.variant))
    return ctx->err = "a block-1 hierarchy needs the immersed operators A2 and M of the elliptic-interface variants", ALFD_E_INVALID;
  if (ctx->nranks > 1) return ctx->err = "the block-1 hierarchy is single-rank", ALFD_E_UNSUPPORTED;
  for (int l = 0; l < nlev; ++l)
    if (H.P[l].nrows != (l == 0 ? ctx->n[1] : H.P[l - 1].ncols))
      return ctx->err = "block-1 prolongator of level " + std::to_string(l) + " does not match the unknowns of that level",
             ALFD_E_INVALID;
  if (full)
    H.ml.assign(nlev + 1, MlLevel());
  else
    free_coupling(ctx, 1, c_changed);
  const bool gpu_products = ctx->ml_gpu_galerkin != 0;
  HostCsr An, Cn, Ctn, A, C;
  for (int l = 0; l <= nlev; ++l) {
    LevelStore &L = H.ml[l].loc;
    if (full) RC(level_vectors(ctx, 1, l, l == 0 ? ctx->n[1] : H.ncoarse[l - 1]));
    RC(level_penalty(ctx, 1, l, 0));
    if (l == nlev) break;
    LevelStore &Nx = H.ml[l + 1].loc;
    if (full) RC(csr_level_A(ctx, H.P[l], l == 0 ? ctx->mat[ALFD_A2] : L.A, gpu_products, l == 0 ? nullptr : &A, Nx, An));
    if (full || c_changed)
      RC(csr_level_C(ctx, H.P[l], l == 0 ? ctx->mat[ALFD_M] : L.C, gpu_products, l == 0 ? nullptr : &C, Nx, Cn, Ctn));
    if (l + 1 < nlev) {
      if (full) A = std::move(An);
      if (full || c_changed) C = std::move(Cn);
    }
  }
  if (c.ml_coarse_direct > 0 && H.ml[nlev].loc.n <= c.ml_coarse_direct) {
    if (full) H.coarse_A = std::move(An);
    if (full || c_changed) H.coarse_C = std::move(Cn), H.coarse_Ct = std::move(Ctn);
    std::vector<double> w(ctx->n[2]);
    HIPC(hipMemcpyAsync(w.data(), ctx->diag[ALFD_INVW], w.size() * sizeof(double), hipMemcpyDeviceToHost, ctx->stream));
    HIPC(hipStreamSynchronize(ctx->stream));
    PhaseClock pc(ctx, ALFD_SETUP_ML_COARSE);
    RC(coarse_inverse(ctx, H.coarse_A, H.coarse_C, H.coarse_Ct, w, c.gamma2, H.inv));
  }
  for (int l = 0; l <= nlev; ++l)
    RC(build_tail_mask(ctx, 1, l == 0 ? ctx->mat[ALFD_M] : H.ml[l].loc.Ct, H.ml[l].loc.npad, &H.ml[l].tail_mask));
  return build_tail_table(ctx);
}

static int mass_diagonal(alfd_ctx *ctx) {
  const HostCsr &M = ctx->h_M;
  const int last = ctx->nblocks - 1;
  if (!ctx->mat[ALFD_M].present || M.rp.empty() || M.nrows != ctx->n[last])
    return ctx->err = "slot M (immersed mass matrix) must be set for the exact W^-1", ALFD_E_NOT_SETUP;
  const int64_t nlp = pad_chunk(ctx->n[last]);
  const int64_t row0 = ctx->nranks > 1 ? ctx->part[last][ctx->rank] : 0;
  std::vector<double> dm(nlp, 0.0);
  for (int64_t i = 0; i < M.nrows; ++i) {
    double dii = 0.0;
    for (int64_t k = M.rp[i]; k < M.rp[i + 1]; ++k)
      if (M.col[k] == row0 + i) dii = M.val[k];
    if (!(dii > 0.0)) return ctx->err = "mass matrix needs a positive diagonal", ALFD_E_INVALID;
    dm[i] = 1.0 / dii;
  }
  HIPC(hipMemcpyAsync(ctx->dinv_m, dm.data(), nlp * sizeof(double), hipMemcpyHostToDevice, ctx->stream));
  HIPC(hipStreamSynchronize(ctx->stream));
  return ALFD_OK;
}

static int diag_lambda(alfd_ctx *ctx) {
  const alfd_config &c = ctx->cfg;
  const bool ell = is_elliptic(c.variant);
  const bool gd_off = !c.grad_div_in_A && (c.variant == ALFD_AL_STOKES || c.variant == ALFD_AL_STOKES_DIAG);
  const bool cheb = c.inner_prec == ALFD_PREC_CHEBYSHEV || c.inner_prec == ALFD_PREC_MULTILEVEL;
  const int64_t n0p = pad_chunk(ctx->n[0]);
  for (int k = 0; k < 7; ++k) ctx->lam_max[k] = 0;
  PhaseClock diag_clock(ctx, ALFD_SETUP_DIAG_LAMBDA);
  if (gd_off) {
    RC(diag_plus_m(ctx, &ctx->mat[ALFD_A], ctx->mat[ALFD_CT], ctx->diag[ALFD_INVW], c.gamma, ctx->n[0], ctx->dA, false));
    RC(diag_plus_m(ctx, nullptr, ctx->mat[ALFD_BT], ctx->diag[ALFD_MP_LUMPED_INV], c.gamma_grad_div, ctx->n[0],
                   ctx->dinv_aug, true));
  } else {
    RC(diag_plus(ctx, ALFD_A, ALFD_CT, c.aug_assembled ? 0.0 : c.gamma, ctx->n[0], ctx->dinv_aug));
  }
  if (ell) {
    RC(diag_plus(ctx, ALFD_A2, ALFD_M, c.gamma2, ctx->n[1], ctx->dinv_a22));
    if (c.variant == ALFD_AL_ELL_IDEAL) {
      HIPC(hipMemcpyAsync(ctx->dinv_aug2, ctx->dinv_aug, n0p * sizeof(double), hipMemcpyDeviceToDevice,
                          ctx->stream));
      HIPC(hipMemcpyAsync(ctx->dinv_aug2 + ctx->off[1], ctx->dinv_a22, pad_chunk(ctx->n[1]) * sizeof(double),
                          hipMemcpyDeviceToDevice, ctx->stream));
      if (cheb) RC(power_iteration(ctx, OP_AUG2));
    }
    if (cheb && (c.variant == ALFD_AL_ELL_MODIFIED || c.inner_prec == ALFD_PREC_MULTILEVEL)) {
      RC(power_iteration(ctx, OP_AUG));
      RC(power_iteration(ctx, OP_A22));
    }
  } else if (cheb) {
    RC(power_iteration(ctx, OP_AUG));
// ... 451 lines not shown

int alfd_abi_version(void) { return ALFD_ABI_VERSION; }

const char *alfd_strerror(int s) {
  switch (s) {
    case ALFD_OK: return "ok";
    case ALFD_E_INVALID: return "invalid argument";
    case ALFD_E_HIP: return "HIP runtime error";
    case ALFD_E_NO_CONVERGENCE_OUTER: return "FGMRES: no convergence (SolverControl::NoConvergence)";
    case ALFD_E_NO_CONVERGENCE_INNER: return "inner CG: no convergence (SolverControl::NoConvergence)";
    case ALFD_E_BREAKDOWN: return "breakdown (NaN residual)";
    case ALFD_E_NOT_SETUP: return "context not set up";
    case ALFD_E_COMM: return "RCCL error";
    case ALFD_E_UNSUPPORTED: return "not implemented";
    default: return "unknown status";
  }
}

const char *alfd_last_error(alfd_ctx_t ctx) { return ctx ? ctx->err.c_str() : "null context"; }

int alfd_create(alfd_ctx_t *out, int device_id) {
  if (!out) return ALFD_E_INVALID;
  *out = nullptr;
  int ndev = 0;
  if (hipGetDeviceCount(&ndev) != hipSuccess || ndev <= 0 || device_id < 0 || device_id >= ndev)
    return ALFD_E_HIP;
  if (hipSetDevice(device_id) != hipSuccess) return ALFD_E_HIP;
  alfd_ctx *ctx = new alfd_ctx;
  ctx->device = device_id;
  if (hipStreamCreateWithFlags(&ctx->xstream, hipStreamNonBlocking) != hipSuccess ||
      hipEventCreateWithFlags(&ctx->ev_x, hipEventDisableTiming) != hipSuccess ||
      hipEventCreateWithFlags(&ctx->ev_halo, hipEventDisableTiming) != hipSuccess)
    ctx->xstream = nullptr;
  if (const char *e = std::getenv("ALFD_SPMV_OVERLAP_HALO")) ctx->overlap_halo = std::atoi(e);
  if (hipStreamCreateWithFlags(&ctx->stream, hipStreamNonBlocking) != hipSuccess) {
    delete ctx;
    return ALFD_E_HIP;
  }
  alfd_default_config(&ctx->cfg, ALFD_AL_STOKES);
  if (const char *e = std::getenv("ALFD_SPMV_STREAM_R")) ctx->spmv_stream_R = std::atoi(e);
  if (const char *e = std::getenv("ALFD_SPMV_STREAM_U")) ctx->spmv_stream_U = std::atoi(e);
  if (const char *e = std::getenv("ALFD_SPMV_PREC32_R")) ctx->a32_R = std::atoi(e);
  if (const char *e = std::getenv("ALFD_SPMV_PREC32_U")) ctx->a32_U = std::atoi(e);
  if (const char *e = std::getenv("ALFD_SPMV_NT")) ctx->spmv_nt = std::atoi(e);
  if (const char *e = std::getenv("ALFD_SPMV_GRID")) ctx->spmv_grid_mult = std::max(1, std::atoi(e));
  if (const char *e = std::getenv("ALFD_SPMV_WINDOW")) ctx->win_enable = std::atoi(e);
  if (const char *e = std::getenv("ALFD_SPMV_WINDOW_RB")) ctx->win_RB = std::max(4, std::atoi(e));
  if (const char *e = std::getenv("ALFD_SPMV_WINDOW_MIN_BLOCKS")) ctx->win_min_blocks = std::max(1, std::atoi(e));
  if (const char *e = std::getenv("ALFD_SPMV_WINDOW_SHORT_MIN_BLOCKS")) ctx->win_short_min_blocks = std::max(1, std::atoi(e));
  if (const char *e = std::getenv("ALFD_SPMV_WINDOW_MAXW")) ctx->win_maxW = std::min(16384, std::max(256, std::atoi(e)));
  if (const char *e = std::getenv("ALFD_ML_REPLICATE")) ctx->ml_rep_threshold = std::atoll(e);
  if (const char *e = std::getenv("ALFD_ML_GPU_GALERKIN")) ctx->ml_gpu_galerkin = std::atoi(e);
  if (const char *e = std::getenv("ALFD_ML_FUSE")) ctx->ml_fuse = std::max(0, std::min(3, std::atoi(e)));
  if (const char *e = std::getenv("ALFD_SPMV_VI_LEVELS")) ctx->vi_levels = std::atoi(e);
  if (const char *e = std::getenv("ALFD_SPMV_BATCH_MAJOR")) ctx->vs_enable = std::atoi(e);
  if (const char *e = std::getenv("ALFD_SPMV_BATCH_MAJOR_ROWS")) ctx->vs_RB = std::max(4, std::min(kVsMaxRows, std::atoi(e)));
  if (const char *e = std::getenv("ALFD_SPMV_SMALL_SHAPES")) ctx->vs_small = std::atoi(e) != 0;
  {
    hipDeviceProp_t prop;
    if (hipGetDeviceProperties(&prop, device_id) == hipSuccess) ctx->vs_cus = prop.multiProcessorCount;
  }
  if (const char *e = std::getenv("ALFD_SPMV_VI_XCD")) ctx->vi_xcd = std::atoi(e);
  if (const char *e = std::getenv("ALFD_SPMV_VI_BATCHED")) ctx->vi_batched = std::atoi(e);
  if (const char *e = std::getenv("ALFD_SPMV_WINDOW_RB_VI")) ctx->win_RB_vi = std::atoi(e);
  if (const char *e = std::getenv("ALFD_SPMV_VI_R")) ctx->vi_rows_R = std::atoi(e);
  if (const char *e = std::getenv("ALFD_SPMV_VI_J")) ctx->vi_rows_J = std::atoi(e);
  if (const char *e = std::getenv("ALFD_SPMV_VALUE_INDEX")) ctx->win_vi = std::atoi(e);
  if (const char *e = std::getenv("ALFD_SPMV_GROUP_R")) ctx->spmv_group_R = std::atoi(e);
  if (const char *e = std::getenv("ALFD_SPMV_GROUP_U")) ctx->spmv_group_U = std::atoi(e);
  if (const char *e = std::getenv("ALFD_SPMV_WINDOW_SHORT")) ctx->win_short_scale = std::max(0, std::atoi(e));
  if (const char *e = std::getenv("ALFD_SPMV_WINDOW_GAP")) ctx->win_gap = std::max(1, std::atoi(e));
  if (const char *e = std::getenv("ALFD_SPMV_WINDOW_XCD")) ctx->win_xcd = std::atoi(e);
  *out = ctx;
  return ALFD_OK;
}

int alfd_destroy(alfd_ctx_t ctx) {
  if (!ctx) return ALFD_E_INVALID;
  hipSetDevice(ctx->device);
  hipStreamSynchronize(ctx->stream);
  flush_timers(ctx);
  free_levels(ctx);
  spectrum_release(ctx);
  csr_free(ctx->rat_mat);
  for (DevCsr &m : ctx->mat) csr_free(m);
  for (void *p : ctx->ws_allocs) hipFree(p);
  for (void *p : ctx->allocs) hipFree(p);
  if (ctx->sc_host) hipHostFree(ctx->sc_host);
  if (ctx->n_sc_host) hipHostFree(ctx->n_sc_host);
  if (ctx->rt_scb_host) hipHostFree(ctx->rt_scb_host);
  if (ctx->nccl) ncclCommDestroy(ctx->nccl);
  if (ctx->xstream) hipStreamDestroy(ctx->xstream);
  if (ctx->ev_x) hipEventDestroy(ctx->ev_x);
  if (ctx->ev_halo) hipEventDestroy(ctx->ev_halo);
  if (ctx->ev_in) hipEventDestroy(ctx->ev_in);
  hipStreamDestroy(ctx->stream);
  delete ctx;
  return ALFD_OK;
}

int alfd_comm_unique_id(void *id_out, size_t bytes) {
  static_assert(sizeof(ncclUniqueId) <= ALFD_UNIQUE_ID_BYTES, "unique id size");
  if (!id_out || bytes < sizeof(ncclUniqueId)) return ALFD_E_INVALID;
  ncclUniqueId id;
  if (ncclGetUniqueId(&id) != ncclSuccess) return ALFD_E_COMM;
  std::memset(id_out, 0, bytes);
// ... 1266 lines not shown
  const size_t rows = std::max<int64_t>(m.nrows, 1) * sizeof(double), nb = m.nrows * sizeof(double);
  double *dx = nullptr, *dd = nullptr, *dy = nullptr, *dy2 = nullptr;
  HIPC(hipMalloc((void **)&dx, std::max<int64_t>(nx, 1) * sizeof(double)));
  HIPC(hipMalloc((void **)&dd, rows));
  HIPC(hipMalloc((void **)&dy, rows));
  if (y2) HIPC(hipMalloc((void **)&dy2, rows));
  HIPC(hipMemcpyAsync(dx, x, nx * sizeof(double), hipMemcpyHostToDevice, ctx->stream));
  HIPC(hipMemcpyAsync(dd, d, nb, hipMemcpyHostToDevice, ctx->stream));
  HIPC(hipMemcpyAsync(dy, y, nb, hipMemcpyHostToDevice, ctx->stream));
  if (y2) HIPC(hipMemcpyAsync(dy2, y2, nb, hipMemcpyHostToDevice, ctx->stream));
  const int rc = spmv(ctx, slot, dx, dy, y2 ? 3 : 2, 0.0, dd, dy2);
  if (rc == ALFD_OK) {
    HIPC(hipMemcpyAsync(y, dy, nb, hipMemcpyDeviceToHost, ctx->stream));
    if (y2) HIPC(hipMemcpyAsync(y2, dy2, nb, hipMemcpyDeviceToHost, ctx->stream));
    HIPC(hipStreamSynchronize(ctx->stream));
  }
  hipFree(dx);
  hipFree(dd);
  hipFree(dy);
  hipFree(dy2);
  return rc;
}

int alfd_spmv_pair(alfd_ctx_t ctx, int slot_a, int slot_c, const double *x, const double *d, double *y, double *t) {
  CHECK_CTX();
  for (int slot : {slot_a, slot_c})
    if (slot < 0 || slot >= ALFD_NSLOTS || !ctx->mat[slot].present) return ALFD_E_INVALID;
  if (!x || !d || !y || !t || t == y) return ALFD_E_INVALID;
  const DevCsr &A = ctx->mat[slot_a], &Cm = ctx->mat[slot_c];
  const int form = pair_forms(ctx, A, Cm);
  if (!form) return ctx->err = "alfd_spmv_pair: the two slots do not qualify for the pair launch", ALFD_E_UNSUPPORTED;
  double *dx = nullptr, *dd = nullptr, *dy = nullptr, *dt = nullptr;
  HIPC(hipMalloc((void **)&dx, A.ncols * sizeof(double)));
  HIPC(hipMalloc((void **)&dd, Cm.nrows * sizeof(double)));
  HIPC(hipMalloc((void **)&dy, A.nrows * sizeof(double)));
  HIPC(hipMalloc((void **)&dt, Cm.nrows * sizeof(double)));
  HIPC(hipMemcpyAsync(dx, x, A.ncols * sizeof(double), hipMemcpyHostToDevice, ctx->stream));
  HIPC(hipMemcpyAsync(dd, d, Cm.nrows * sizeof(double), hipMemcpyHostToDevice, ctx->stream));
  HIPC(hipMemcpyAsync(dy, y, A.nrows * sizeof(double), hipMemcpyHostToDevice, ctx->stream));
  HIPC(hipMemcpyAsync(dt, t, Cm.nrows * sizeof(double), hipMemcpyHostToDevice, ctx->stream));
  const int rc = launch_pair(ctx, form, A, slot_a == ALFD_A ? ALFD_T_SPMV_A : ALFD_T_SPMV_OTHER, Cm, dd, dx, dy, dt);
  if (rc == ALFD_OK) {
    HIPC(hipMemcpyAsync(y, dy, A.nrows * sizeof(double), hipMemcpyDeviceToHost, ctx->stream));
    HIPC(hipMemcpyAsync(t, dt, Cm.nrows * sizeof(double), hipMemcpyDeviceToHost, ctx->stream));
    HIPC(hipStreamSynchronize(ctx->stream));
  }
  hipFree(dx);
  hipFree(dd);
  hipFree(dy);
  hipFree(dt);
  return rc;
}

int alfd_inner_prec_apply(alfd_ctx_t ctx, int op, const double *r, double *z) {
  CHECK_CTX();
  CHECK_SETUP();
  if (!r || !z) return ALFD_E_INVALID;
  const int v = ctx->cfg.variant;
  int kind = -1;
  if (op == ALFD_INNER_OP_AUG &&
      (v == ALFD_AL2 || v == ALFD_AL_STOKES || v == ALFD_AL_STOKES_DIAG || v == ALFD_AL_ELL_MODIFIED))
    kind = OP_AUG;
  else if (op == ALFD_INNER_OP_A22 && v == ALFD_AL_ELL_MODIFIED)
    kind = OP_A22;
  else if (op == ALFD_INNER_OP_AUG2 && v == ALFD_AL_ELL_IDEAL)
    kind = OP_AUG2;
  if (kind < 0)
    return ctx->err = "alfd_inner_prec_apply: the configured variant has no such inner operator", ALFD_E_INVALID;
  const int b0 = kind == OP_A22 ? 1 : 0, b1 = kind == OP_AUG2 ? 1 : b0;
  const int64_t npad = op_npad(ctx, kind);
  double *dr = ctx->st_in + ctx->off[b0], *dz = ctx->st_out + ctx->off[b0];
  HIPC(hipMemsetAsync(ctx->st_in, 0, ctx->ntot() * sizeof(double), ctx->stream));
  HIPC(hipMemsetAsync(ctx->st_out, 0, ctx->ntot() * sizeof(double), ctx->stream));
  int64_t at = 0;
  for (int b = b0; b <= b1; ++b) {
    HIPC(hipMemcpyAsync(ctx->st_in + ctx->off[b], r + at, ctx->n[b] * sizeof(double), hipMemcpyHostToDevice,
                        ctx->stream));
    at += ctx->n[b];
  }
  const int prec = ctx->cfg.inner_prec;
  if (prec == ALFD_PREC_IDENTITY) {
    HIPC(hipMemcpyAsync(dz, dr, npad * sizeof(double), hipMemcpyDeviceToDevice, ctx->stream));
  } else if (prec == ALFD_PREC_JACOBI) {
    VEC_LAUNCH(jacobi_dot_kernel, npad, 24, op_dinv(ctx, kind), dr, dz, ctx->partial);
    HIPC(hipGetLastError());
  } else if (prec == ALFD_PREC_MULTILEVEL && ml_covers(ctx, kind)) {
    RC(ml_prec(ctx, kind, dr, dz));
  } else {
    RC(cheb_apply(ctx, kind, dr, dz, npad));
  }
  at = 0;
  for (int b = b0; b <= b1; ++b) {
    HIPC(hipMemcpyAsync(z + at, ctx->st_out + ctx->off[b], ctx->n[b] * sizeof(double), hipMemcpyDeviceToHost,
                        ctx->stream));
    at += ctx->n[b];
  }
  HIPC(hipStreamSynchronize(ctx->stream));
  return ALFD_OK;
}

int alfd_dot(alfd_ctx_t ctx, int64_t n, const double *x, const double *y, double *result) {
  CHECK_CTX();
  if (n < 0 || !x || !y || !result) return ALFD_E_INVALID;
  const int64_t npad = pad_chunk(std::max<int64_t>(n, 1));
  double *dx = nullptr, *dy = nullptr, *part = nullptr, *sc = nullptr;
  HIPC(hipMalloc((void **)&dx, npad * sizeof(double)));
// ... 731 lines not shown
  size_t f = 0, t = 0;
  HIPC(hipMemGetInfo(&f, &t));
  if (free_bytes) *free_bytes = (int64_t)f;
  if (total_bytes) *total_bytes = (int64_t)t;
  return ALFD_OK;
}

int alfd_set_tunable(alfd_ctx_t ctx, const char *name, int value) {
  if (!ctx || !name) return ALFD_E_INVALID;
  if (std::strcmp(name, "value_index") == 0) {
    ctx->vi_off = value == 0;
    if (value == 0) RC(ensure_window_plans(ctx));
    return ALFD_OK;
  }
  if (std::strcmp(name, "batch_major") == 0) {
    ctx->vs_enable = value != 0;
    if (value == 0) RC(ensure_window_plans(ctx));
    return ALFD_OK;
  }
  if (std::strcmp(name, "batch_major_share") == 0) {
    ctx->vs_share = value != 0;
    return ALFD_OK;
  }
  if (std::strcmp(name, "batch_major_wide") == 0) {
    ctx->vs_wide = value != 0;
    return ALFD_OK;
  }
  if (std::strcmp(name, "batch_major_waves") == 0) {
    if (value != 1 && value != 2 && value != 4 && value != 8) return ctx->err = "batch_major_waves: 1, 2, 4 or 8", ALFD_E_INVALID;
    ctx->vs_NW = value;
    for (int sl = 0; sl < ALFD_NSLOTS; ++sl) {
      DevCsr::Vs &v = ctx->mat[sl].vs;
      if (v.on && v.L == 64 && !v.small && !v.wide) v.NW = value;
    }
    return ALFD_OK;
  }
  if (std::strcmp(name, "batch_major_small") == 0) {
    ctx->vs_small = value != 0;
    return ALFD_OK;
  }
  if (std::strcmp(name, "batch_major_rows") == 0) {
    if (value < 4 || value > kVsMaxRows) return ctx->err = "batch_major_rows: 4..250", ALFD_E_INVALID;
    ctx->vs_RB = value;
    return ALFD_OK;
  }
  if (std::strcmp(name, "batch_major_xcd") == 0) {
    ctx->vs_xcd = value != 0;
    return ALFD_OK;
  }
  if (std::strcmp(name, "ml_fuse") == 0) {
    ctx->ml_fuse = std::max(0, std::min(3, value));
    return ALFD_OK;
  }
  if (std::strcmp(name, "ml_gpu_galerkin") == 0) {
    if (value != 0 && value != 1) return ctx->err = "ml_gpu_galerkin: 0 or 1", ALFD_E_INVALID;
    ctx->ml_gpu_galerkin = value;
    return ALFD_OK;
  }
  if (std::strcmp(name, "ml_tail_rows") == 0) {
    if (value < 0) return ctx->err = "ml_tail_rows: >= 0", ALFD_E_INVALID;
    ctx->ml_tail_rows = value;
    return ALFD_OK;
  }
  if (std::strcmp(name, "nested_mp_group") == 0) {
    if (value < 1 || value > 1000) return ctx->err = "nested_mp_group: 1..1000", ALFD_E_INVALID;
    ctx->nmp_group = value;
    return ALFD_OK;
  }
  if (std::strcmp(name, "nested_mp_host_stepped") == 0) {
    ctx->nmp_host_stepped = value != 0;
    return ALFD_OK;
  }
  if (std::strcmp(name, "spectrum_group") == 0) {
    if (value < 1 || value > 1000) return ctx->err = "spectrum_group: 1..1000", ALFD_E_INVALID;
    ctx->spec_group = value;
    return ALFD_OK;
  }
  if (std::strcmp(name, "spectrum_host_stepped") == 0) {
    ctx->spec_host_stepped = value != 0;
    return ALFD_OK;
  }
  return ctx->err = std::string("unknown tunable ") + name, ALFD_E_INVALID;
}

int alfd_host_tridiagonal_extremes(int32_t k, const double *alpha, const double *beta, double *lambda_min,
                                   double *lambda_max) {
  return host_tridiagonal_extremes(k, alpha, beta, lambda_min, lambda_max);
}

int alfd_estimate_spectrum(alfd_ctx_t ctx, int op, const alfd_control *ctrl, alfd_spectrum *out) {
  CHECK_CTX();
  CHECK_SETUP();
  if (!out) return ALFD_E_INVALID;
  if (op != ALFD_SPECTRUM_CCT) return ctx->err = "alfd_estimate_spectrum: unknown operator", ALFD_E_INVALID;
  if (ctx->nranks > 1) return ctx->err = "alfd_estimate_spectrum: single rank only", ALFD_E_UNSUPPORTED;
  const int64_t nl = ctx->n[ctx->nblocks - 1];
  alfd_control c;
  if (ctrl) {
    c = *ctrl;
  } else {
    c.kind = ALFD_CTRL_ABS;
    c.max_steps = (int32_t)std::min<int64_t>(nl, INT32_MAX);
    c.tol = 1e-12;
    c.reduce = 0.0;
  }
  if (c.kind < ALFD_CTRL_ABS || c.kind > ALFD_CTRL_FIXED_ITERS || c.max_steps < 1)
// ... 70 lines not shown
```

### fictitious_domain_al_preconditioners_amd/csrc/kernels.hpp

```cpp
#pragma once
#include <hip/hip_runtime.h>
#include <stdint.h>
#include <type_traits>

namespace alfd {

constexpr int kBlock = 256;
constexpr int64_t kChunk = 4096;
constexpr int kMaxBasis = 64;

__device__ __forceinline__ double dpp_xor_mov(double v, int which) {
  int lo = __double2loint(v), hi = __double2hiint(v), rl, rh;
  if (which == 8) {
    rl = __builtin_amdgcn_update_dpp(0, lo, 0x128, 0xf, 0xf, true);
    rh = __builtin_amdgcn_update_dpp(0, hi, 0x128, 0xf, 0xf, true);
  } else if (which == 4) {
    rl = __builtin_amdgcn_update_dpp(0, lo, 0x104, 0xf, 0x5, false);
    rl = __builtin_amdgcn_update_dpp(rl, lo, 0x114, 0xf, 0xa, false);
    rh = __builtin_amdgcn_update_dpp(0, hi, 0x104, 0xf, 0x5, false);
    rh = __builtin_amdgcn_update_dpp(rh, hi, 0x114, 0xf, 0xa, false);
  } else if (which == 2) {
    rl = __builtin_amdgcn_update_dpp(0, lo, 0x4E, 0xf, 0xf, true);
    rh = __builtin_amdgcn_update_dpp(0, hi, 0x4E, 0xf, 0xf, true);
  } else {
// ... 1065 lines not shown
__global__ __launch_bounds__(kBlock) void xr_update_dot_kernel(const double *__restrict__ sc,
                                                               const double *__restrict__ p,
                                                               const double *__restrict__ Ap,
                                                               double *__restrict__ x,
                                                               double *__restrict__ r,
                                                               double *__restrict__ partial) {
  __shared__ double lds4[4];
  const double a = sc[S_ALPHA], na = sc[S_NALPHA];
  double acc = 0.0;
  ALFD_FOR_PAIRS(i) {
    const double2 pv = ld2(p, i), av = ld2(Ap, i);
    double2 xv = ld2(x, i), rv = ld2(r, i);
    xv.x = fma(a, pv.x, xv.x);
    xv.y = fma(a, pv.y, xv.y);
    rv.x = fma(na, av.x, rv.x);
    rv.y = fma(na, av.y, rv.y);
    st2(x, i, xv);
    st2(r, i, rv);
    acc = fma(rv.x, rv.x, acc);
    acc = fma(rv.y, rv.y, acc);
  }
  const double s = block_reduce_256(acc, lds4);
  if (threadIdx.x == 0) partial[blockIdx.x] = s;
}

__global__ __launch_bounds__(kBlock) void cheb_init_kernel(double inv_theta, const double *__restrict__ dinv,
                                                           const double *__restrict__ r,
                                                           double *__restrict__ d, double *__restrict__ z,
                                                           double *__restrict__ res, int keep_res) {
  ALFD_FOR_PAIRS(i) cheb_init_pair(i, inv_theta, dinv, r, d, z, res, keep_res);
}
__global__ __launch_bounds__(kBlock) void cheb_step_kernel(double c1, double c2,
                                                           const double *__restrict__ dinv,
                                                           const double *__restrict__ tmp,
                                                           double *__restrict__ res, double *__restrict__ d,
                                                           double *__restrict__ z) {
  ALFD_FOR_PAIRS(i) cheb_step_pair(i, c1, c2, dinv, tmp, res, d, z);
}

__global__ __launch_bounds__(kBlock) void cheb_init_z_kernel(double inv_theta, const double *__restrict__ dinv,
                                                             const double *__restrict__ r, double *__restrict__ z) {
  ALFD_FOR_PAIRS(i) {
    const double2 dv = ld2(dinv, i), rv = ld2(r, i);
    double2 o;
    o.x = inv_theta * (dv.x * rv.x);
    o.y = inv_theta * (dv.y * rv.y);
    st2(z, i, o);
  }
}

enum { TAIL_STEP = 0, TAIL_LAST = 1, TAIL_LAST_ADD = 2, TAIL_RES = 3, TAIL_RES_INIT = 4, TAIL_RES_INIT_ADD = 5 };
struct AugTailArgs {
  double gamma = 0, c1 = 0, c2 = 0;
  const double *dinv = nullptr, *y = nullptr, *rin = nullptr, *din = nullptr;
  double *res = nullptr, *d = nullptr, *z = nullptr, *zout = nullptr;
  int store_res = 0;
};

template <int MODE>
__device__ __forceinline__ void aug_tail_math(const AugTailArgs &p, double y, double dinv, double rin, double din,
                                              double zin, double zo, double &res, double &d, double &z, double &zout) {
  res = rin - y;
  if (MODE <= TAIL_LAST_ADD) {
    d = fma(p.c1, din, p.c2 * (dinv * res));
    z = zin + d;
    if (MODE == TAIL_LAST_ADD) zout = fma(1.0, z, zo);
  } else if (MODE >= TAIL_RES_INIT) {
    z = p.c1 * (dinv * res);
    if (MODE == TAIL_RES_INIT_ADD) zout = fma(1.0, z, zo);
  }
}

template <int MODE>
__device__ __forceinline__ void aug_tail_elem(const AugTailArgs &p, int64_t i, double y) {
  constexpr bool kStep = MODE <= TAIL_LAST_ADD, kAdd = MODE == TAIL_LAST_ADD || MODE == TAIL_RES_INIT_ADD;
  const double dinv = MODE != TAIL_RES ? p.dinv[i] : 0.0, rin = p.rin[i];
  const double din = kStep ? p.din[i] : 0.0, zin = kStep ? p.z[i] : 0.0, zo = kAdd ? p.zout[i] : 0.0;
  double res, d = 0.0, z = 0.0, zout = 0.0;
  aug_tail_math<MODE>(p, y, dinv, rin, din, zin, zo, res, d, z, zout);
  if (MODE == TAIL_STEP || MODE == TAIL_RES || (MODE == TAIL_RES_INIT && p.store_res)) p.res[i] = res;
  if (MODE == TAIL_STEP) p.d[i] = d;
  if (MODE == TAIL_STEP || MODE == TAIL_LAST || MODE == TAIL_RES_INIT) p.z[i] = z;
  if (kAdd) p.zout[i] = zout;
}

template <int L, int MODE>
__global__ __launch_bounds__(kBlock) void aug_tail_kernel(int64_t n_list, const int64_t *__restrict__ rp,
                                                          const int32_t *__restrict__ col,
                                                          const double *__restrict__ val,
                                                          const int32_t *__restrict__ rows,
                                                          const double *__restrict__ t, int nb_rows,
                                                          const uint8_t *__restrict__ mask, AugTailArgs p) {
  if ((int)blockIdx.x < nb_rows) {
    constexpr int RPB = kBlock / L;
    const int lane = threadIdx.x % L;
    const int sub = threadIdx.x / L;
    const int64_t ngroups = (n_list + RPB - 1) / RPB;
    for (int64_t g = blockIdx.x; g < ngroups; g += nb_rows) {
      const int64_t r = g * RPB + sub;
      if (r < n_list) {
        const int64_t k0 = rp[r], k1 = rp[r + 1];
        double acc = 0.0;
        for (int64_t k = k0 + lane; k < k1; k += L) acc = fma(val[k], t[col[k]], acc);
        acc = group_reduce<L>(acc);
        if (lane == 0) {
          const int64_t ro = rows ? (int64_t)rows[r] : r;
          aug_tail_elem<MODE>(p, ro, fma(p.gamma, acc, p.y[ro]));
        }
      }
    }
    return;
  }
  constexpr bool kStep = MODE <= TAIL_LAST_ADD, kAdd = MODE == TAIL_LAST_ADD || MODE == TAIL_RES_INIT_ADD;
  const int64_t base = (int64_t)((int)blockIdx.x - nb_rows) * kChunk;
#pragma unroll
  for (int e = 0; e < 8; ++e) {
    const int64_t i = base + e * 512 + 2 * threadIdx.x;
    const uchar2 mk = *reinterpret_cast<const uchar2 *>(mask + i);
    if (mk.x | mk.y) {
      if (!mk.x) aug_tail_elem<MODE>(p, i, p.y[i]);
      if (!mk.y) aug_tail_elem<MODE>(p, i + 1, p.y[i + 1]);
      continue;
    }
    const double2 zero = {0.0, 0.0};
    const double2 yv = ld2(p.y, i), rv = ld2(p.rin, i);
    const double2 dv = MODE != TAIL_RES ? ld2(p.dinv, i) : zero;
    const double2 dd = kStep ? ld2(p.din, i) : zero, zi = kStep ? ld2(p.z, i) : zero;
    const double2 zo = kAdd ? ld2(p.zout, i) : zero;
    double2 res, d = zero, z = zero, zout = zero;
    aug_tail_math<MODE>(p, yv.x, dv.x, rv.x, dd.x, zi.x, zo.x, res.x, d.x, z.x, zout.x);
    aug_tail_math<MODE>(p, yv.y, dv.y, rv.y, dd.y, zi.y, zo.y, res.y, d.y, z.y, zout.y);
    if (MODE == TAIL_STEP || MODE == TAIL_RES || (MODE == TAIL_RES_INIT && p.store_res)) st2(p.res, i, res);
    if (MODE == TAIL_STEP) st2(p.d, i, d);
    if (MODE == TAIL_STEP || MODE == TAIL_LAST || MODE == TAIL_RES_INIT) st2(p.z, i, z);
    if (kAdd) st2(p.zout, i, zout);
  }
}

__global__ void mark_rows_kernel(int64_t n_list, const int32_t *__restrict__ rows, uint8_t *__restrict__ mask) {
  const int64_t i = (int64_t)blockIdx.x * blockDim.x + threadIdx.x;
  if (i < n_list) mask[rows ? (int64_t)rows[i] : i] = 1;
}

constexpr int kTailBlock = 1024;
constexpr int kTailMaxDegree = 64;
constexpr int kTailMaxLevels = 9;
struct TailCsr {
  const int64_t *rp;
  const int32_t *col;
  const double *val;
  const int32_t *rows;
  int64_t n_list, nrows;
  int32_t L, sparse;
};
struct TailLevel {
  TailCsr A, C, Ct;
  TailCsr R, P;
  const double *dinv, *w;
  double *tlam, *r, *z, *t, *cd, *cres, *ctmp;
  double gamma, inv_theta;
  int64_t npad;
  int32_t degree, pad_;
  double c1[kTailMaxDegree], c2[kTailMaxDegree];
};
struct TailTable {
  int32_t nlev, has_inv;
  TailCsr inv;
  TailLevel lev[kTailMaxLevels];
};

template <int L>
__device__ __forceinline__ void tail_rows(const TailCsr &m, const double *x, double *y, int epi, double alpha,
                                          const double *d) {
  constexpr int RPB = kTailBlock / L;
  const int lane = threadIdx.x % L;
  const int sub = threadIdx.x / L;
  const int64_t ngroups = (m.n_list + RPB - 1) / RPB;
  for (int64_t g = 0; g < ngroups; ++g) {
    const int64_t r = g * RPB + sub;
    if (r < m.n_list) {
// ... 1217 lines not shown
```

### fictitious_domain_al_preconditioners_amd/csrc/kernels_vs.hpp

```cpp
#pragma once

namespace alfd {

constexpr int kVsMaxDict = 512;
constexpr int kVsDictOff = 0;
constexpr int kVsWinOff = kVsMaxDict * 8;
constexpr int kVsMaxRows = 250;
template <int WD>
struct VsFmt {
  static constexpr uint32_t kColMask = WD ? 0x3ff8u : 0x7ff8u;
  static constexpr int kDictShift = WD ? 11 : 12;
  static constexpr uint32_t kDictMask = WD ? 0x1ff8u : 0xff8u;
  static constexpr int kWinOff = WD ? 8192 : 4096;
  static constexpr int kCodeShift = WD ? 14 : 15;
  static constexpr int kMaxDict = WD ? 1024 : 512;
  static constexpr int kMaxSlots = WD ? 2048 : 4096;
};
constexpr int kVsMaxLen = 384;

__device__ __forceinline__ uint32_t vs_off(uint32_t d) { return d & 0xfffffu; }
__device__ __forceinline__ int32_t vs_len(uint32_t d) { return (int32_t)((d >> 20) & 0x1ffu); }
__device__ __forceinline__ int vs_cls(uint32_t d) { return (int)((d >> 29) & 7u); }

__device__ __forceinline__ double vs_lds_f64(uint32_t byte_off) {
// ... 44 lines not shown
  const int32_t rem = vs_len(d0) - 64 * (cls - 1);
  uint32_t l4 = 4u * (uint32_t)lane, r4 = 4u * (uint32_t)(lane < rem ? lane : rem - 1);
  asm volatile("" : "+v"(l4), "+v"(r4));
  w[0] = *(const uint32_t *)(fb + 256 * (cls - 1) + r4);
#pragma unroll
  for (int j = 0; j < 5; ++j)
    if (j < cls - 1) w[1 + j] = *(const uint32_t *)(fb + 256 * j + l4);
}

template <int NCH, int R, int WD>
__device__ __forceinline__ void vs_shared(int32_t rem, const int32_t (&sh)[R], int lane, const uint32_t (&w)[6],
                                          double (&acc)[R]) {
#pragma unroll
  for (int j = 0; j < NCH; ++j) {
    const uint32_t wj = j == NCH - 1 ? w[0] : w[1 + (j < 5 ? j : 0)];
    const uint32_t lc = wj & VsFmt<WD>::kColMask;
    double v = vs_lds_f64(kVsDictOff + ((wj >> VsFmt<WD>::kDictShift) & VsFmt<WD>::kDictMask));
    constexpr int G = R > 8 ? 4 : R;
    auto rounds = [&]() __attribute__((always_inline)) {
#pragma unroll
      for (int g = 0; g < R; g += G) {
        double xv[G];
#pragma unroll
        for (int i = 0; i < G; ++i) xv[i] = vs_lds_f64(VsFmt<WD>::kWinOff + (uint32_t)((int32_t)lc + sh[g + i]));
        if constexpr (G == 4) {
          if (g == 0)
            asm volatile("" : "+v"(xv[0]), "+v"(xv[1]), "+v"(xv[2]), "+v"(xv[3]), "+v"(v));
          else
            asm volatile("" : "+v"(xv[0]), "+v"(xv[1]), "+v"(xv[2]), "+v"(xv[3]));
        } else {
          static_assert(G == 8, "one pinning statement per round: written out for rounds of 4 and of 8 gathers");
          asm volatile("" : "+v"(xv[0]), "+v"(xv[1]), "+v"(xv[2]), "+v"(xv[3]), "+v"(xv[4]), "+v"(xv[5]), "+v"(xv[6]),
                       "+v"(xv[7]), "+v"(v));
        }
#pragma unroll
        for (int i = 0; i < G; ++i) acc[g + i] = fma(v, xv[i], acc[g + i]);
        if (R > 8) {
#pragma unroll
          for (int i = 0; i < G; ++i) asm volatile("" : "+v"(acc[g + i]));
        }
      }
    };
    if (j == NCH - 1) {
      if (lane < rem) {
        asm volatile("");
        rounds();
      }
    } else {
      rounds();
    }
  }
}

template <int EPI, int TAG, int NW, int WD = 0, bool PAIR = false>
__global__ __launch_bounds__(64 * NW) __attribute__((amdgpu_waves_per_eu(8, 8))) void spmv_vs_kernel(
    const uint8_t *__restrict__ stream, const uint64_t *__restrict__ tab, int32_t stride,
    const int32_t *__restrict__ hdrb, const int32_t *__restrict__ segx, int32_t seg_stride,
    const double *__restrict__ dict, const double *__restrict__ x, const double *__restrict__ x_halo,
    int32_t n_local, double *__restrict__ y, double alpha, const double *__restrict__ d, double *__restrict__ y2,
    int xcd_remap, int32_t block_base, PairArg<PAIR> pc) {
  static_assert(!PAIR || NW <= 4, "the second party needs a lane group of 64 within 64 NW <= kBlock threads");
  if (pair_rows<64 * NW>(pc, x)) return;
  extern __shared__ double xs[];
  char *sm = (char *)xs;
  double *ds = (double *)(sm + kVsDictOff);
  double *xw = (double *)(sm + VsFmt<WD>::kWinOff);
  const int lane = threadIdx.x & 63;
  const int wave = __builtin_amdgcn_readfirstlane(threadIdx.x >> 6);
  int64_t b = blockIdx.x;
  if (xcd_remap) {
    const int64_t nwg = pair_nA(pc), q = nwg / 8, rm = nwg % 8, xcd = b % 8, idx = b / 8;
    b = (xcd < rm ? xcd * (q + 1) : rm * (q + 1) + (xcd - rm) * q) + idx;
  }
  b += block_base;
  const int32_t *hb = hdrb + 8 * b;
  const int32_t nbatch = hb[0], W = hb[1], nseg = hb[2], nd = hb[3], doff = hb[4];
  const uint8_t *sbase = stream + (int64_t)(((uint64_t)(uint32_t)hb[6] << 32) | (uint64_t)(uint32_t)hb[5]);
  const int32_t *sx = segx + 2 * b * (int64_t)seg_stride;
  const uint32_t *tb = (const uint32_t *)(tab + (int64_t)b * stride * 16);
  const int hl = lane & 31;
  auto hdr_at = [&](int32_t q) {
    uint32_t h4 = 4u * (uint32_t)hl;
    asm volatile("" : "+v"(h4));
    return *(const uint32_t *)((const char *)(tb + 32 * (int64_t)q) + h4);
  };
  auto hdr_load = [&](int32_t q) {
    return hdr_at(q < nbatch ? q : (nbatch > 0 ? nbatch - 1 : 0));
  };
  auto hdr = [](uint32_t hv, int k) { return (uint32_t)__builtin_amdgcn_readlane((int)hv, k); };
  uint32_t hv1 = hdr_at(wave);
  uint32_t hv2 = hdr_at(wave + NW);
  uint32_t w[6];
  {
    constexpr int U = 4;
    auto stage = [&](int32_t s) {
      int32_t c0[U], o0[U], sl[U];
      double v[U];
#pragma unroll
      for (int u = 0; u < U; ++u) {
        const int32_t q = s + u;
        c0[u] = sx[2 * q];
        o0[u] = sx[2 * q + 1];
        const int32_t on = sx[2 * q + 3];
        sl[u] = q < nseg ? ((q + 1 < nseg ? on : W) - o0[u]) : 0;
      }
#pragma unroll
      for (int u = 0; u < U; ++u) {
        const int32_t c = c0[u] + (lane < sl[u] ? lane : 0);
        v[u] = (c < n_local) ? x[c] : x_halo[c - n_local];
      }
#pragma unroll
      for (int u = 0; u < U; ++u)
        if (lane < sl[u]) xw[o0[u] + lane] = v[u];
    };
    for (int t = threadIdx.x; t < nd; t += 64 * NW) ds[t] = dict[doff + t];
    if (wave < nbatch && (int32_t)hdr(hv1, 1) < 0) vs_shared_fetch(hdr(hv1, 0), sbase, lane, w);
    stage(wave * U);
    for (int32_t s = (wave + NW) * U; s < nseg; s += NW * U) stage(s);
  }
  __syncthreads();
  const int q16 = lane >> 4;
  const int rsel = 4 * (2 * ((((q16 & 1) << 1) | (q16 >> 1)) + 4 * ((lane >> 3) & 1) + 8 * ((lane >> 2) & 1)) + 1);
  auto store = [&](double s, int32_t r, bool mine) {
    if (mine && r >= 0) {
      if (EPI == 0)
        y[r] = s;
      else if (EPI == 1)
        y[r] = fma(alpha, s, y[r]);
      else if (EPI == 2)
        y[r] = d[r] * s;
      else {
        y[r] = s;
        y2[r] = d[r] * s;
      }
    }
  };
  auto batch = [&](uint32_t &hc, uint32_t &hn, const int32_t bi) __attribute__((always_inline)) {
    uint32_t lo[16];
#pragma unroll
    for (int i = 0; i < 16; ++i) lo[i] = hdr(hc, 2 * i);
    const bool shared = (int32_t)hdr(hc, 1) < 0;
    const bool sixteen = shared && (int32_t)hdr(hc, 17) >= 0;
    const bool eight = shared && !sixteen && (int32_t)hdr(hc, 9) >= 0;
    const uint32_t eb = vs_off(lo[0]);
    const int cls = vs_cls(lo[0]);
    const int32_t full = cls > 0 ? 64 * (cls - 1) : 0;
    const uint8_t *fb = sbase + 16u * (size_t)eb;
    double sres;
    int mstep;
    uint32_t n0, n1;
    if (sixteen) {
      const int32_t rem = vs_len(lo[0]) - full;
      int32_t sh[16];
      sh[0] = 0;
#pragma unroll
      for (int i = 1; i < 16; ++i) sh[i] = (int32_t)lo[i];
      double acc[16] = {0.0, 0.0, 0.0, 0.0, 0.0, 0.0, 0.0, 0.0, 0.0, 0.0, 0.0, 0.0, 0.0, 0.0, 0.0, 0.0};
      switch (cls) {
        case 1: vs_shared<1, 16, WD>(rem, sh, lane, w, acc); break;
        case 2: vs_shared<2, 16, WD>(rem, sh, lane, w, acc); break;
        case 3: vs_shared<3, 16, WD>(rem, sh, lane, w, acc); break;
        case 4: vs_shared<4, 16, WD>(rem, sh, lane, w, acc); break;
        case 5: vs_shared<5, 16, WD>(rem, sh, lane, w, acc); break;
        default: vs_shared<6, 16, WD>(rem, sh, lane, w, acc); break;
      }
      sres = reduce_rows16(acc, lane);
      mstep = 4;
    } else if (eight) {
      const int32_t rem = vs_len(lo[0]) - full;
      int32_t sh[8];
      sh[0] = 0;
#pragma unroll
      for (int i = 1; i < 8; ++i) sh[i] = (int32_t)lo[i];
      double acc[8] = {0.0, 0.0, 0.0, 0.0, 0.0, 0.0, 0.0, 0.0};
      switch (cls) {
        case 1: vs_shared<1, 8, WD>(rem, sh, lane, w, acc); break;
        case 2: vs_shared<2, 8, WD>(rem, sh, lane, w, acc); break;
        case 3: vs_shared<3, 8, WD>(rem, sh, lane, w, acc); break;
        case 4: vs_shared<4, 8, WD>(rem, sh, lane, w, acc); break;
        case 5: vs_shared<5, 8, WD>(rem, sh, lane, w, acc); break;
        default: vs_shared<6, 8, WD>(rem, sh, lane, w, acc); break;
      }
      sres = reduce_rows8(acc[0], acc[1], acc[2], acc[3], acc[4], acc[5], acc[6], acc[7], lane);
      mstep = 8;
    } else if (shared) {
      double acc[4] = {0.0, 0.0, 0.0, 0.0};
      const int32_t rem = vs_len(lo[0]) - full;
      const int32_t sh[4] = {0, (int32_t)lo[1], (int32_t)lo[2], (int32_t)lo[3]};
      switch (cls) {
        case 1: vs_shared<1, 4, WD>(rem, sh, lane, w, acc); break;
        case 2: vs_shared<2, 4, WD>(rem, sh, lane, w, acc); break;
        case 3: vs_shared<3, 4, WD>(rem, sh, lane, w, acc); break;
        case 4: vs_shared<4, 4, WD>(rem, sh, lane, w, acc); break;
        case 5: vs_shared<5, 4, WD>(rem, sh, lane, w, acc); break;
        default: vs_shared<6, 4, WD>(rem, sh, lane, w, acc); break;
      }
      sres = reduce_rows4(acc[0], acc[1], acc[2], acc[3]);
      mstep = 16;
    } else {
      double acc[4] = {0.0, 0.0, 0.0, 0.0};
      int32_t rem[4], maxrem = 1;
#pragma unroll
      for (int i = 0; i < 4; ++i) {
        rem[i] = vs_len(lo[i]) - full;
        maxrem = rem[i] > maxrem ? rem[i] : maxrem;
      }
      switch (cls) {
        case 1: vs_batch<1, WD>(rem, maxrem, lane, fb, sm, acc); break;
        case 2: vs_batch<2, WD>(rem, maxrem, lane, fb, sm, acc); break;
        case 3: vs_batch<3, WD>(rem, maxrem, lane, fb, sm, acc); break;
        case 4: vs_batch<4, WD>(rem, maxrem, lane, fb, sm, acc); break;
        case 5: vs_batch<5, WD>(rem, maxrem, lane, fb, sm, acc); break;
        case 6: vs_batch<6, WD>(rem, maxrem, lane, fb, sm, acc); break;
        default: break;
      }
      n0 = hdr(hn, 0);
      n1 = hdr(hn, 1);
      store(reduce_rows4(acc[0], acc[1], acc[2], acc[3]), (int32_t)__builtin_amdgcn_ds_bpermute(rsel, (int)hc), (lane & 15) == 0);
      mstep = 0;
    }
    int32_t rid = -1;
    if (mstep) {
      rid = (int32_t)((uint32_t)__builtin_amdgcn_ds_bpermute(rsel, (int)hc) &
                      (lane < 8 ? 0x7fffffffu : 0xffffffffu));
      n0 = hdr(hn, 0);
      n1 = hdr(hn, 1);
    }
    if (bi + NW < nbatch && (int32_t)n1 < 0) vs_shared_fetch(n0, sbase, lane, w);
    hc = hdr_load(bi + 2 * NW);
    if (mstep) store(sres, rid, (lane & (mstep - 1)) == 0);
  };
  for (int32_t bi = wave; bi < nbatch; bi += 2 * NW) {
    batch(hv1, hv2, bi);
    if (bi + NW >= nbatch) break;
    batch(hv2, hv1, bi + NW);
  }
}

template <int L, int EPI, int TAG>
__global__ __launch_bounds__(256) __attribute__((amdgpu_waves_per_eu(8, 8))) void spmv_vss_kernel(
    const uint8_t *__restrict__ stream, const int64_t *__restrict__ sb, const uint64_t *__restrict__ tab,
    const int32_t *__restrict__ cnt, int32_t stride, const int32_t *__restrict__ blk_seg_begin,
    const int32_t *__restrict__ blk_W, const int32_t *__restrict__ seg_col, const int32_t *__restrict__ seg_off,
    const int32_t *__restrict__ blk_dict_off, const int32_t *__restrict__ blk_dict_n,
    const double *__restrict__ dict, const double *__restrict__ x, const double *__restrict__ x_halo,
    int32_t n_local, double *__restrict__ y, double alpha, const double *__restrict__ d, double *__restrict__ y2) {
  extern __shared__ double xs[];
  constexpr int G = 64 / L, W64 = 1 + 4 * G, NW = 4;
  char *sm = (char *)xs;
  double *ds = (double *)(sm + kVsDictOff);
  double *xw = (double *)(sm + kVsWinOff);
  const int lane = threadIdx.x & 63;
  const int wave = __builtin_amdgcn_readfirstlane(threadIdx.x >> 6);
  const int l = lane & (L - 1), g = lane / L;
  const int64_t b = blockIdx.x;
  const int32_t nbatch = cnt[b];
  const uint8_t *sbase = stream + sb[b];
  {
    const int32_t nd = blk_dict_n[b];
    for (int t = threadIdx.x; t < nd; t += 64 * NW) ds[t] = dict[blk_dict_off[b] + t];
    const int32_t W = blk_W[b];
    const int32_t s0 = blk_seg_begin[b], s1 = blk_seg_begin[b + 1];
    constexpr int U = 4;
    for (int32_t s = s0 + wave * U; s < s1; s += NW * U) {
      int32_t c0[U], o0[U], sl[U];
      double v[U];
#pragma unroll
      for (int u = 0; u < U; ++u) {
        const int32_t q = s + u < s1 ? s + u : s1 - 1;
        c0[u] = seg_col[q];
        o0[u] = seg_off[q];
        sl[u] = ((q + 1 < s1) ? seg_off[q + 1] : W) - o0[u];
      }
#pragma unroll
      for (int u = 0; u < U; ++u) {
        const int32_t c = c0[u] + (lane < sl[u] ? lane : 0);
        v[u] = (c < n_local) ? x[c] : x_halo[c - n_local];
      }
#pragma unroll
      for (int u = 0; u < U; ++u)
        if (lane < sl[u]) xw[o0[u] + lane] = v[u];
    }
  }
  __syncthreads();
  const uint64_t *dsc = tab + ((int64_t)b * stride + wave) * W64;
  auto load_batch = [&](const uint64_t *dp, uint64_t hh, uint64_t (&e)[4], uint32_t (&f)[4]) {
    const uint8_t *fbp = sbase + 16u * (size_t)vs_off(hh);
    const int32_t ln = vs_len(hh);
// ... 107 lines not shown
```

### fictitious_domain_al_preconditioners_amd/solver.py

```python
from __future__ import annotations

import ctypes as C
import os

import numpy as np

from . import _abi

_HERE = os.path.dirname(os.path.abspath(__file__))
LIB_PATH = os.path.join(_HERE, "lib", "libalfd.so")
_lib = None

ABI_SYMBOLS = [
    "alfd_abi_version", "alfd_strerror", "alfd_last_error", "alfd_create", "alfd_destroy",
    "alfd_comm_unique_id", "alfd_comm_init", "alfd_set_partition", "alfd_set_matrix", "alfd_set_diag",
    "alfd_configure", "alfd_default_config", "alfd_setup", "alfd_precond_apply", "alfd_system_apply",
    "alfd_augment_rhs", "alfd_solve", "alfd_upload_rhs", "alfd_solve_resident", "alfd_download_solution",
    "alfd_get_history", "alfd_spmv", "alfd_dot", "alfd_matrix_lanes", "alfd_bench_spmv",
    "alfd_enable_timing", "alfd_get_timing", "alfd_host_halo_plan", "alfd_local_group_create",
    "alfd_local_group_destroy", "alfd_comm_init_local", "alfd_set_aggregates",
    "alfd_set_aggregate_partition", "alfd_get_matrix_info", "alfd_bench_spmv_format",
    "alfd_host_window_plan", "alfd_set_tunable", "alfd_build_aggregates", "alfd_get_aggregates",
    "alfd_host_aggregate_level", "alfd_comm_init_host",
    "alfd_get_device_memory", "alfd_set_row_blocks", "alfd_host_stream_plan",
    "alfd_host_row_blocks_from_points", "alfd_host_stream_plan_short", "alfd_set_prolongator", "alfd_set_controls", "alfd_get_timing_streamed", "alfd_get_setup_seconds",
    "alfd_host_numbering_from_points", "alfd_host_brick_blocks_from_points", "alfd_host_permute_csr",
    "alfd_build_smoothed_aggregation", "alfd_get_prolongator", "alfd_host_smoothed_prolongator",
    "alfd_build_smoothed_aggregation_truncated", "alfd_host_truncate_prolongator",
    "alfd_inner_prec_apply", "alfd_spmv_scaled", "alfd_spmv_pair", "alfd_get_last_spmv_launch",
    "alfd_estimate_spectrum", "alfd_get_cg_coefficients", "alfd_host_tridiagonal_extremes",
    "alfd_constraint_residual",
    "alfd_set_prolongator_block", "alfd_build_smoothed_aggregation_block", "alfd_get_prolongator_block",
    "alfd_clear_hierarchy", "alfd_get_inner_iterations", "alfd_get_aggregates_block",
    "alfd_host_strength_graph", "alfd_host_aggregate_graph", "alfd_build_strength_graph", "alfd_get_strength_graph",
    "alfd_upload_rhs_device", "alfd_download_solution_device", "alfd_solve_device", "alfd_precond_apply_device",
    "alfd_system_apply_device", "alfd_augment_rhs_device",
    "alfd_get_matrix_shape", "alfd_get_operator_shape", "alfd_bench_operator", "alfd_host_small_shape",
    "alfd_host_sparse_product", "alfd_sparse_product", "alfd_smoothed_prolongator",
    "alfd_setup_coupling", "alfd_get_setup_counts",
    "alfd_set_preconditioner_values", "alfd_get_preconditioner_values", "alfd_spmv_preconditioner",
    "alfd_bench_spmv_preconditioner",
]


class AlfdError(RuntimeError):

    def __init__(self, status, message):
        super().__init__(f"alfd status {status}: {message}")
        self.status = status


class NoConvergence(AlfdError):
    pass


def load_library():
    global _lib
    if _lib is not None:
        return _lib
    if not os.path.exists(LIB_PATH):
        raise ImportError(f"{LIB_PATH} is missing: the HIP extension is required (no CPU fallback). "
                          "Build it with `python -c 'import __graft_entry__ as g; g.build()'`.")
    lib = C.CDLL(LIB_PATH)
    vp, i32, i64, dbl = C.c_void_p, C.c_int32, C.c_int64, C.c_double
    PP = C.POINTER(C.c_void_p)
    sig = {
        "alfd_abi_version": (C.c_int, []),
        "alfd_strerror": (C.c_char_p, [C.c_int]),
        "alfd_last_error": (C.c_char_p, [vp]),
        "alfd_create": (C.c_int, [C.POINTER(vp), C.c_int]),
        "alfd_destroy": (C.c_int, [vp]),
        "alfd_comm_unique_id": (C.c_int, [vp, C.c_size_t]),
        "alfd_comm_init": (C.c_int, [vp, C.c_int, C.c_int, vp, C.c_size_t]),
        "alfd_set_partition": (C.c_int, [vp, C.c_int, PP]),
        "alfd_set_matrix": (C.c_int, [vp, C.c_int, i64, i64, vp, vp, vp]),
        "alfd_set_diag": (C.c_int, [vp, C.c_int, i64, vp]),
        "alfd_configure": (C.c_int, [vp, C.POINTER(_abi.Config)]),
        "alfd_default_config": (None, [C.POINTER(_abi.Config), C.c_int]),
        "alfd_setup": (C.c_int, [vp]),
        "alfd_setup_coupling": (C.c_int, [vp]),
        "alfd_get_setup_counts": (C.c_int, [vp, vp]),
        "alfd_precond_apply": (C.c_int, [vp, PP, PP, C.POINTER(_abi.Result)]),
        "alfd_system_apply": (C.c_int, [vp, PP, PP]),
        "alfd_augment_rhs": (C.c_int, [vp, PP]),
        "alfd_solve": (C.c_int, [vp, PP, PP, C.POINTER(_abi.Result)]),
        "alfd_upload_rhs": (C.c_int, [vp, PP, PP]),
        "alfd_solve_resident": (C.c_int, [vp, C.POINTER(_abi.Result)]),
        "alfd_download_solution": (C.c_int, [vp, PP]),
        "alfd_get_history": (C.c_int, [vp, vp, i32, C.POINTER(i32)]),
        "alfd_spmv": (C.c_int, [vp, C.c_int, vp, vp, C.c_int, dbl]),
        "alfd_spmv_scaled": (C.c_int, [vp, C.c_int, vp, vp, vp, vp]),
        "alfd_spmv_pair": (C.c_int, [vp, C.c_int, C.c_int, vp, vp, vp, vp]),
        "alfd_get_last_spmv_launch": (C.c_int, [vp, C.POINTER(_abi.SpmvLaunch)]),
        "alfd_dot": (C.c_int, [vp, i64, vp, vp, C.POINTER(dbl)]),
        "alfd_inner_prec_apply": (C.c_int, [vp, C.c_int, vp, vp]),
        "alfd_matrix_lanes": (C.c_int, [vp, C.c_int, C.POINTER(i32)]),
        "alfd_bench_spmv": (C.c_int, [vp, C.c_int, i32, C.POINTER(dbl), C.POINTER(dbl)]),
        "alfd_enable_timing": (C.c_int, [vp, C.c_int]),
        "alfd_get_timing": (C.c_int, [vp, vp, vp, vp]),
        "alfd_host_halo_plan": (C.c_int, [i64, vp, vp, C.c_int, C.c_int, vp, vp, i64, C.POINTER(i64), vp]),
        "alfd_local_group_create": (C.c_int, [C.c_int, C.POINTER(vp)]),
        "alfd_local_group_destroy": (C.c_int, [vp]),
        "alfd_comm_init_local": (C.c_int, [vp, vp, C.c_int]),
        "alfd_set_aggregates": (C.c_int, [vp, C.c_int, i64, vp, vp, i64]),
        "alfd_set_aggregate_partition": (C.c_int, [vp, C.c_int, vp]),
        "alfd_set_prolongator": (C.c_int, [vp, C.c_int, i64, i64, vp, vp, vp]),
        "alfd_set_controls": (C.c_int, [vp, vp, vp, vp]),
        "alfd_get_timing_streamed": (C.c_int, [vp, vp]),
        "alfd_get_setup_seconds": (C.c_int, [vp, vp]),
        "alfd_get_matrix_info": (C.c_int, [vp, C.c_int, C.POINTER(_abi.MatrixInfo)]),
        "alfd_bench_spmv_format": (C.c_int, [vp, C.c_int, i32, C.c_int, C.POINTER(dbl), C.POINTER(dbl)]),
        "alfd_get_matrix_shape": (C.c_int, [vp, C.c_int, C.POINTER(_abi.BatchMajorShape)]),
        "alfd_get_operator_shape": (C.c_int, [vp, C.c_int, C.c_int, C.POINTER(_abi.BatchMajorShape)]),
        "alfd_bench_operator": (C.c_int, [vp, C.c_int, C.c_int, i32, i32, i32, C.POINTER(dbl), C.POINTER(_abi.BatchMajorShape)]),
        "alfd_host_small_shape": (C.c_int, [i64, i64, i64, i32, i32, i32, C.POINTER(i32), C.POINTER(i32)]),
        "alfd_host_window_plan": (C.c_int, [i64, vp, vp, vp, i32, i32, C.POINTER(_abi.WindowPlanInfo)]),
        "alfd_set_tunable": (C.c_int, [vp, C.c_char_p, C.c_int]),
        "alfd_build_aggregates": (C.c_int, [vp, i32, dbl, i32, i64, i32, C.POINTER(i32)]),
        "alfd_get_aggregates": (C.c_int, [vp, C.c_int, vp, i64, C.POINTER(i64), C.POINTER(i64)]),
        "alfd_host_aggregate_level": (C.c_int, [i64, vp, vp, vp, i32, dbl, i32, vp, C.POINTER(i64)]),
        "alfd_build_smoothed_aggregation": (C.c_int, [vp, i32, dbl, i32, dbl, i64, i32, C.POINTER(i32), vp]),
        "alfd_build_smoothed_aggregation_truncated": (C.c_int, [vp, i32, dbl, i32, dbl, dbl, i32, i64, i32,
                                                                C.POINTER(i32), vp]),
        "alfd_host_truncate_prolongator": (C.c_int, [i64, i64, vp, vp, vp, vp, i32, dbl, i32, vp, vp, vp, i64,
                                                     C.POINTER(i64)]),
        "alfd_get_prolongator": (C.c_int, [vp, C.c_int, vp, vp, vp, i64, C.POINTER(i64), C.POINTER(i64),
                                           C.POINTER(i64)]),
        "alfd_host_smoothed_prolongator": (C.c_int, [i64, vp, vp, vp, i64, vp, vp, vp, vp, dbl, vp, i64, dbl,
                                                     vp, vp, vp, i64, C.POINTER(i64)]),
        "alfd_host_sparse_product": (C.c_int, [i64, i64, vp, vp, vp, i64, vp, vp, vp, vp, vp, vp, i64, C.POINTER(i64)]),
        "alfd_sparse_product": (C.c_int, [vp, i64, i64, vp, vp, vp, i64, vp, vp, vp, vp, vp, vp, i64, C.POINTER(i64),
                                          C.POINTER(i32)]),
        "alfd_smoothed_prolongator": (C.c_int, [vp, i64, vp, vp, vp, i64, vp, vp, vp, vp, dbl, vp, i64, dbl, i32, dbl, i32,
                                                vp, vp, vp, i64, C.POINTER(i64), C.POINTER(i32)]),
        "alfd_comm_init_host": (C.c_int, [vp, C.c_int, C.c_int, vp, vp, vp]),
        "alfd_get_device_memory": (C.c_int, [vp, C.POINTER(i64), C.POINTER(i64)]),
        "alfd_set_row_blocks": (C.c_int, [vp, C.c_int, i64, vp, vp]),
        "alfd_host_stream_plan": (C.c_int, [i64, vp, vp, vp, C.c_int32, i64, vp, vp, vp]),
        "alfd_host_row_blocks_from_points": (C.c_int, [i64, C.c_int32, vp, C.c_int32, vp, vp, vp]),
        "alfd_host_stream_plan_short": (C.c_int, [i64, vp, vp, vp, C.c_int32, vp]),
        "alfd_host_numbering_from_points": (C.c_int, [i64, C.c_int32, vp, vp]),
        "alfd_host_brick_blocks_from_points": (C.c_int, [i64, C.c_int32, vp, vp, C.c_int32, vp, vp, vp]),
        "alfd_host_permute_csr": (C.c_int, [i64, vp, vp, vp, vp, vp, vp, vp, vp]),
        "alfd_estimate_spectrum": (C.c_int, [vp, C.c_int, C.POINTER(_abi.Control), C.POINTER(_abi.Spectrum)]),
        "alfd_get_cg_coefficients": (C.c_int, [vp, vp, vp, i32, C.POINTER(i32)]),
        "alfd_host_tridiagonal_extremes": (C.c_int, [i32, vp, vp, C.POINTER(dbl), C.POINTER(dbl)]),
# ... 338 lines not shown
                                         self._stream(stream, rhs, x))
        if rc != _abi.OK and raise_on_failure:
            self._ck_dev(rc)
        return res

    def upload_rhs_device(self, rhs, x0=None, stream=None):
        x0t = self._dev(x0, "x0") if x0 is not None else None
        self._ck_dev(self._lib.alfd_upload_rhs_device(self._h, self._dev(rhs, "rhs"), x0t, self._stream(stream, rhs, x0)))

    def download_solution_device(self, x, stream=None):
        self._ck_dev(self._lib.alfd_download_solution_device(self._h, self._dev(x, "x", True), self._stream(stream, x)))

    def history(self):
        cnt = C.c_int32(0)
        self._lib.alfd_get_history(self._h, None, 0, C.byref(cnt))
        out = np.zeros(max(cnt.value, 1))
        self._lib.alfd_get_history(self._h, out.ctypes.data, cnt.value, C.byref(cnt))
        return out[:cnt.value]

    def spmv(self, slot, x, y=None, mode=0, alpha=1.0):
        x = np.ascontiguousarray(x, np.float64)
        lanes = C.c_int32()
        self._ck(self._lib.alfd_matrix_lanes(self._h, slot, C.byref(lanes)))
        if y is None:
            raise ValueError("pass y (its length is the row count)")
        y = np.ascontiguousarray(y, np.float64).copy()
        self._ck(self._lib.alfd_spmv(self._h, slot, x.ctypes.data, y.ctypes.data, mode, alpha))
        return y, lanes.value

    def spmv_scaled(self, slot, x, d, y, y2=None):
        x = np.ascontiguousarray(x, np.float64)
        d = np.ascontiguousarray(d, np.float64)
        y = np.ascontiguousarray(y, np.float64).copy()
        if d.size != y.size or (y2 is not None and np.size(y2) != y.size):
            raise ValueError("d, y and y2 have the row count of the slot")
        if y2 is None:
            self._ck(self._lib.alfd_spmv_scaled(self._h, slot, x.ctypes.data, d.ctypes.data, y.ctypes.data, None))
            return y
        y2 = np.ascontiguousarray(y2, np.float64).copy()
        self._ck(self._lib.alfd_spmv_scaled(self._h, slot, x.ctypes.data, d.ctypes.data, y.ctypes.data, y2.ctypes.data))
        return y, y2

    def spmv_pair(self, slot_a, slot_c, x, d, y, t):
        x = np.ascontiguousarray(x, np.float64)
        d = np.ascontiguousarray(d, np.float64)
        y = np.ascontiguousarray(y, np.float64).copy()
        t = np.ascontiguousarray(t, np.float64).copy()
        if d.size != t.size:
            raise ValueError("d and t have the row count of slot_c")
        self._ck(self._lib.alfd_spmv_pair(self._h, slot_a, slot_c, x.ctypes.data, d.ctypes.data, y.ctypes.data,
                                          t.ctypes.data))
        return y, t

    def last_spmv_launch(self):
        rec = _abi.SpmvLaunch()
        self._ck(self._lib.alfd_get_last_spmv_launch(self._h, C.byref(rec)))
        out = rec.as_dict()
        out["family_name"] = _abi.SPMV_FAMILY_NAMES[rec.family]
        return out

    def dot(self, x, y):
        x = np.ascontiguousarray(x, np.float64)
        y = np.ascontiguousarray(y, np.float64)
        out = C.c_double()
        self._ck(self._lib.alfd_dot(self._h, x.size, x.ctypes.data, y.ctypes.data, C.byref(out)))
        return out.value

    def inner_prec_apply(self, r, op=_abi.INNER_OP_AUG):
        r = np.ascontiguousarray(r, np.float64)
        bs = self.block_sizes
        if bs is None:
            n = r.size
        else:
            n = {_abi.INNER_OP_AUG: bs[0], _abi.INNER_OP_A22: bs[1]}.get(op, bs[0] + bs[1])
            if r.size != n:
                raise ValueError(f"r has {r.size} entries, the inner operator {n}")
        z = np.zeros(n)
        self._ck(self._lib.alfd_inner_prec_apply(self._h, int(op), r.ctypes.data, z.ctypes.data))
        return z

    def estimate_spectrum(self, op=_abi.SPECTRUM_CCT, control=None):
        out = _abi.Spectrum()
        self._ck(self._lib.alfd_estimate_spectrum(self._h, int(op), None if control is None else C.byref(control),
                                                  C.byref(out)))
        return out

    def cg_coefficients(self):
        cnt = C.c_int32(0)
        self._ck(self._lib.alfd_get_cg_coefficients(self._h, None, None, 0, C.byref(cnt)))
        alpha, beta = np.zeros(cnt.value), np.zeros(max(cnt.value, 1))
        self._ck(self._lib.alfd_get_cg_coefficients(self._h, alpha.ctypes.data, beta.ctypes.data, cnt.value,
                                                    C.byref(cnt)))
        return alpha, beta[:max(cnt.value - 1, 0)].copy()

    def constraint_residual(self, x, g=None):
        x = self._in(x)
        gv = None if g is None else np.ascontiguousarray(g, np.float64)
        if gv is not None and gv.size != self.block_sizes[-1]:
            raise ValueError(f"g has {gv.size} entries, the multiplier block {self.block_sizes[-1]}")
        out = C.c_double()
        self._ck(self._lib.alfd_constraint_residual(self._h, _blocks(x), None if gv is None else gv.ctypes.data,
                                                    C.byref(out)))
        return out.value

    def bench_spmv(self, slot, reps=20):
        ms, nbytes = C.c_double(), C.c_double()
# ... 580 lines not shown
```

### include/alfd/alfd.h

```cpp
#ifndef ALFD_H
#define ALFD_H

#include <stddef.h>
#include <stdint.h>

#ifdef __cplusplus
extern "C" {
#endif

#define ALFD_ABI_VERSION 12
#define ALFD_MAX_BLOCKS 3

enum alfd_status {
  ALFD_OK = 0,
  ALFD_E_INVALID = 1,
  ALFD_E_HIP = 2,
  ALFD_E_NO_CONVERGENCE_OUTER = 3,
  ALFD_E_NO_CONVERGENCE_INNER = 4,
  ALFD_E_BREAKDOWN = 5,
  ALFD_E_NOT_SETUP = 6,
  ALFD_E_COMM = 7,
  ALFD_E_UNSUPPORTED = 8
};

// ... 183 lines not shown
int alfd_host_sparse_product(int64_t a_nrows, int64_t a_ncols, const int64_t *a_row_ptr, const int32_t *a_col,
                             const double *a_val, int64_t p_ncols, const int64_t *p_row_ptr, const int32_t *p_col,
                             const double *p_val, int64_t *out_row_ptr, int32_t *out_col, double *out_val,
                             int64_t capacity, int64_t *nnz);
int alfd_sparse_product(alfd_ctx_t ctx, int64_t a_nrows, int64_t a_ncols, const int64_t *a_row_ptr, const int32_t *a_col,
                        const double *a_val, int64_t p_ncols, const int64_t *p_row_ptr, const int32_t *p_col,
                        const double *p_val, int64_t *out_row_ptr, int32_t *out_col, double *out_val, int64_t capacity,
                        int64_t *nnz, int32_t *on_device);
int alfd_smoothed_prolongator(alfd_ctx_t ctx, int64_t nrows, const int64_t *row_ptr, const int32_t *col, const double *val,
                              int64_t n_mult, const int64_t *ct_row_ptr, const int32_t *ct_col, const double *ct_val,
                              const double *w_inv, double gamma, const int32_t *agg, int64_t n_coarse, double omega,
                              int32_t block_size, double drop_tolerance, int32_t max_row_entries, int64_t *p_row_ptr,
                              int32_t *p_col, double *p_val, int64_t capacity, int64_t *nnz, int32_t *on_device);
int alfd_configure(alfd_ctx_t ctx, const alfd_config *cfg);
int alfd_set_controls(alfd_ctx_t ctx, const alfd_control *outer, const alfd_control *inner, const alfd_control *mp_inner);
void alfd_default_config(alfd_config *cfg, int variant);
int alfd_setup(alfd_ctx_t ctx);
int alfd_setup_coupling(alfd_ctx_t ctx);
enum alfd_setup_count {
  ALFD_SC_PRODUCTS_A = 0,
  ALFD_SC_PRODUCTS_C = 1,
  ALFD_SC_LEVEL_A_UPLOADS = 2,
  ALFD_SC_TRANSFER_UPLOADS = 3,
  ALFD_SC_PATCH_BUILDS = 4,
  ALFD_SC_POWER_ITERATIONS = 5,
  ALFD_SC_NCOUNTS = 6
};
int alfd_get_setup_counts(alfd_ctx_t ctx, int64_t *counts );

int alfd_precond_apply(alfd_ctx_t ctx, const double *const *src_blocks, double *const *dst_blocks,
                       alfd_result *res);
int alfd_system_apply(alfd_ctx_t ctx, const double *const *src_blocks, double *const *dst_blocks);
int alfd_augment_rhs(alfd_ctx_t ctx, double *const *rhs_blocks);
int alfd_solve(alfd_ctx_t ctx, const double *const *rhs_blocks, double *const *x_blocks,
               alfd_result *res);
int alfd_upload_rhs(alfd_ctx_t ctx, const double *const *rhs_blocks, const double *const *x0_blocks);
int alfd_solve_resident(alfd_ctx_t ctx, alfd_result *res);
int alfd_download_solution(alfd_ctx_t ctx, double *const *x_blocks);
int alfd_upload_rhs_device(alfd_ctx_t ctx, const double *const *rhs_blocks, const double *const *x0_blocks,
                           void *stream);
int alfd_download_solution_device(alfd_ctx_t ctx, double *const *x_blocks, void *stream);
int alfd_solve_device(alfd_ctx_t ctx, const double *const *rhs_blocks, double *const *x_blocks, alfd_result *res,
                      void *stream);
int alfd_precond_apply_device(alfd_ctx_t ctx, const double *const *src_blocks, double *const *dst_blocks,
                              alfd_result *res, void *stream);
int alfd_system_apply_device(alfd_ctx_t ctx, const double *const *src_blocks, double *const *dst_blocks, void *stream);
int alfd_augment_rhs_device(alfd_ctx_t ctx, double *const *rhs_blocks, void *stream);
int alfd_get_inner_iterations(alfd_ctx_t ctx, int64_t counts[3]);
int alfd_get_history(alfd_ctx_t ctx, double *out, int32_t capacity, int32_t *count);

int alfd_spmv(alfd_ctx_t ctx, int slot, const double *x, double *y, int mode, double alpha);
int alfd_spmv_scaled(alfd_ctx_t ctx, int slot, const double *x, const double *d, double *y, double *y2);
int alfd_spmv_pair(alfd_ctx_t ctx, int slot_a, int slot_c, const double *x, const double *d, double *y, double *t);
enum alfd_spmv_family {
  ALFD_SPMV_PLAIN = 0,
  ALFD_SPMV_SPARSE_ROWS = 1,
  ALFD_SPMV_STREAM = 2,
  ALFD_SPMV_WINDOW = 3,
  ALFD_SPMV_WINDOW_VI = 4,
  ALFD_SPMV_WINDOW_VIB = 5,
  ALFD_SPMV_WINDOW_GROUP = 6,
  ALFD_SPMV_BATCH_MAJOR = 7,
  ALFD_SPMV_BATCH_MAJOR_SHORT = 8,
  ALFD_SPMV_PLAIN_F32 = 9,
  ALFD_SPMV_STREAM_F32 = 10,
  ALFD_SPMV_WINDOW_F32 = 11,
  ALFD_SPMV_NFAMILIES = 12
};
typedef struct alfd_spmv_launch {
  int32_t family;
  int32_t lanes, R, U, nontemporal, epilogue, xcd_order;
  int64_t grid, lds_bytes;
} alfd_spmv_launch;
int alfd_get_last_spmv_launch(alfd_ctx_t ctx, alfd_spmv_launch *out);
int alfd_dot(alfd_ctx_t ctx, int64_t n, const double *x, const double *y, double *result);
enum alfd_inner_op { ALFD_INNER_OP_AUG = 0, ALFD_INNER_OP_A22 = 1, ALFD_INNER_OP_AUG2 = 2 };
int alfd_inner_prec_apply(alfd_ctx_t ctx, int op, const double *r, double *z);
typedef struct alfd_spectrum {
  int32_t converged;
  int32_t steps;
  double initial_residual, last_residual;
  double lambda_min, lambda_max, condition;
} alfd_spectrum;
enum alfd_spectrum_op { ALFD_SPECTRUM_CCT = 0 };
int alfd_estimate_spectrum(alfd_ctx_t ctx, int op, const alfd_control *ctrl ,
                           alfd_spectrum *out);
int alfd_get_cg_coefficients(alfd_ctx_t ctx, double *alpha, double *beta, int32_t capacity, int32_t *count);
int alfd_host_tridiagonal_extremes(int32_t k, const double *alpha, const double *beta, double *lambda_min, double *lambda_max);
int alfd_constraint_residual(alfd_ctx_t ctx, const double *const *x_blocks, const double *g , double *linf);
int alfd_matrix_lanes(alfd_ctx_t ctx, int slot, int32_t *lanes);
int alfd_bench_spmv(alfd_ctx_t ctx, int slot, int32_t reps, double *ms_per_launch,
                    double *algorithmic_bytes);
typedef struct alfd_matrix_info {
  int32_t lanes, windowed, value_indexed;
  int32_t batch_major;
  int64_t nnz, window_blocks, window_fallback_blocks;
  int64_t value_indexed_blocks, value_indexed_nnz, dictionary_entries, value_wide_nnz;
  double algorithmic_bytes, streamed_bytes;
  int64_t shared_nnz;
  int64_t batch_major_blocks;
  int64_t batch_major_wide;
  int64_t batch_major_interior_blocks;
} alfd_matrix_info;
int alfd_get_matrix_info(alfd_ctx_t ctx, int slot, alfd_matrix_info *out);
typedef struct alfd_batch_major_shape {
  int32_t batch_major, lanes;
// ... 103 lines not shown
```

Baseline: 16.16.

## Fuse Chebyshev smoother tail epilogue into the batch-major SpMV launch

Adds a block-end epilogue to the batch-major SpMV kernel. The row results are staged in LDS and the augmented-operator tail update (residual, direction, iterate) is applied in the same launch for rows outside the Ct mask. The remaining Ct rows are then handled by a rows-only tail kernel. Ping-pong z/d buffers are allocated per level so the product input is never overwritten mid-launch. This is meant to remove a full vector pass and a launch per Chebyshev step, at the cost of extra LDS per block, which may lower occupancy, and more template instantiations.

```diff
diff --git a/fictitious_domain_al_preconditioners_amd/_abi.py b/fictitious_domain_al_preconditioners_amd/_abi.py
--- a/fictitious_domain_al_preconditioners_amd/_abi.py
+++ b/fictitious_domain_al_preconditioners_amd/_abi.py
@@ -108,6 +108,21 @@
 
     def as_dict(self):
         return {k: getattr(self, k) for k, _ in self._fields_}
+
+
+TAIL_STEP, TAIL_LAST, TAIL_LAST_ADD, TAIL_RES, TAIL_RES_INIT, TAIL_RES_INIT_ADD = range(6)
+
+
+class TailStep(C.Structure):
+    _fields_ = [
+        ("mode", C.c_int32), ("store_res", C.c_int32), ("slot_c", C.c_int32), ("reserved", C.c_int32),
+        ("gamma", C.c_double), ("c1", C.c_double), ("c2", C.c_double),
+        ("ct_nrows", C.c_int64), ("ct_ncols", C.c_int64),
+        ("ct_rp", C.c_void_p), ("ct_col", C.c_void_p), ("ct_val", C.c_void_p),
+        ("x", C.c_void_p), ("w", C.c_void_p), ("t", C.c_void_p),
+        ("dinv", C.c_void_p), ("rin", C.c_void_p), ("din", C.c_void_p), ("zin", C.c_void_p),
+        ("y", C.c_void_p), ("res", C.c_void_p), ("d", C.c_void_p), ("z", C.c_void_p), ("zout", C.c_void_p),
+    ]
 
 
 class BatchMajorShape(C.Structure):
diff --git a/fictitious_domain_al_preconditioners_amd/csrc/alfd.hip b/fictitious_domain_al_preconditioners_amd/csrc/alfd.hip
--- a/fictitious_domain_al_preconditioners_amd/csrc/alfd.hip
+++ b/fictitious_domain_al_preconditioners_amd/csrc/alfd.hip
@@ -83,6 +83,7 @@
     bool on = false, bricks = false;
     int64_t nb = 0, nseg = 0, stream_bytes = 0, nbatch = 0, dict_total = 0, shared_nnz = 0;
     int32_t stride = 0, maxW = 0;
+    int32_t tail_lds = 0;
     int32_t L = 64, tab_u64 = 16;
     int32_t wide = 0;
     int32_t RB = 0, NW = 4;
@@ -143,6 +144,7 @@
   LevelStore loc, rep;
   double lmax = 0;
   uint8_t *tail_mask = nullptr;
+  double *tail_z2 = nullptr, *tail_d2 = nullptr;
   bool P_global_cols = false;
   std::vector<int64_t> offs;
   int64_t maxpiece = 0;
@@ -279,6 +281,8 @@
   bool dots_replicated = false;
   int64_t ml_rep_threshold = 300000;
   int ml_fuse = 2;
+  int ml_tail_in_spmv = 1;
+  int64_t fused_tail_launches = 0;
   int ml_tail_rows = 0;
   int ml_gpu_galerkin = 1;
   double *g_w = nullptr, *g_tlam = nullptr;
@@ -848,7 +852,7 @@
   const unsigned grid = (unsigned)n_blocks;
   const int32_t base = (int32_t)first_block;
 #define ALFD_VS_ARGS \
-  v.stream, v.tab, v.stride, v.hdrb, v.segx, v.seg_stride, v.dict, x, m.halo, m.n_local_cols, y, alpha, d, y2, ctx->vs_xcd, base, NoPair()
+  v.stream, v.tab, v.stride, v.hdrb, v.segx, v.seg_stride, v.dict, x, m.halo, m.n_local_cols, y, alpha, d, y2, ctx->vs_xcd, base, NoPair(), NoTail()
 #define ALFD_VS(EPI, NWV)                                                                                        \
   do {                                                                                                           \
     if (v.wide) {                                   \
@@ -1096,7 +1100,7 @@
     note_spmv(ctx, ALFD_SPMV_BATCH_MAJOR, 64, NWV, 0, false, 0, ctx->vs_xcd, (int64_t)pc.nA + pc.nC, lds);                   \
     hipLaunchKernelGGL((spmv_vs_kernel<0, TAG, NWV, 0, true>), dim3(pc.nA + pc.nC), dim3(64 * NWV), lds, ctx->stream,       \
                        v.stream, v.tab, v.stride, v.hdrb, v.segx, v.seg_stride, v.dict, x, A.halo, A.n_local_cols, y, 0.0,  \
-                       (const double *)nullptr, (double *)nullptr, ctx->vs_xcd, 0, pc);                                      \
+                       (const double *)nullptr, (double *)nullptr, ctx->vs_xcd, 0, pc, NoTail());                            \
   } while (0)
 #define ALFD_VS_PAIR_T(TAG)              \
   do {                                   \
@@ -3201,7 +3205,7 @@
   v.RB = RB;
   v.NW = pl.wide ? 4 : NW;
   v.small = small;
-  int32_t max_nseg = 0;
+  int32_t max_nseg = 0, tail_lds = 0, tail_W = 0, tail_cnt = 0, tail_nd = 0;
   for (int64_t b = 0; b < pl.nb; ++b) max_nseg = std::max(max_nseg, pl.seg_begin[b + 1] - pl.seg_begin[b]);
   const int32_t S = std::max(max_nseg + 1, 33);
   if ((double)pl.nb * S * 8.0 > 2.0e9) return ALFD_OK;
@@ -3216,6 +3220,8 @@
     h[4] = pl.doff[b];
     h[5] = (int32_t)(uint32_t)((uint64_t)pl.sb[b] & 0xffffffffull);
     h[6] = (int32_t)((uint64_t)pl.sb[b] >> 32);
+    const int32_t need = vs_tail_lds_need(pl.wide ? VsFmt<1>::kWinOff : VsFmt<0>::kWinOff, pl.dn[b], pl.blkW[b], pl.cnt[b]);
+    if (need > tail_lds) tail_lds = need, tail_W = pl.blkW[b], tail_cnt = pl.cnt[b], tail_nd = pl.dn[b];
     for (int32_t q = 0; q < ns; ++q) {
       segx[((size_t)b * S + q) * 2] = pl.seg_col[s0 + q];
       segx[((size_t)b * S + q) * 2 + 1] = pl.seg_off[s0 + q];
@@ -3238,9 +3244,15 @@
   v.dict_total = (int64_t)pl.dict.size();
   v.stride = pl.stride;
   v.maxW = pl.maxW;
+  v.tail_lds = tail_lds;
   v.wide = pl.wide;
   v.bricks = hint;
   v.on = true;
+  if (ctx->cfg.log_level > 0 || std::getenv("ALFD_LOG_UPLOAD"))
+    std::fprintf(stderr, "[alfd] batch-major format, %lld rows: with the row buffer of the block-end epilogue the largest block asks for "
+                 "%d bytes of LDS (dictionary region %d with %d values, %d window slots, %d batches)\n", (long long)m.nrows,
+                 (pl.wide ? VsFmt<1>::kWinOff : VsFmt<0>::kWinOff) + tail_lds, pl.wide ? VsFmt<1>::kWinOff : VsFmt<0>::kWinOff,
+                 tail_nd, tail_W, tail_cnt);
   if (ctx->cfg.log_level > 0)
     std::fprintf(stderr,
                  "[alfd] batch-major format%s: %lld blocks (%s), %lld batches, window <= %d slots, %.2f B/nnz, %.1f %% of the "
@@ -3774,6 +3786,7 @@
   int64_t npad = 0;
   const double *dinv = nullptr;
   double *cd = nullptr, *cres = nullptr, *ctmp = nullptr;
+  double *cd2 = nullptr, *z2 = nullptr;
   double lmax = 0;
 };
 
@@ -3801,6 +3814,7 @@
   F.npad = S.npad;
   F.dinv = S.dinv;
   F.cd = S.cd, F.cres = S.cres, F.ctmp = S.ctmp;
+  F.cd2 = rep ? nullptr : L.tail_d2, F.z2 = rep ? nullptr : L.tail_z2;
   F.lmax = L.lmax;
   V.r = S.r, V.z = S.z, V.t = S.t;
   if (l + 1 < (int)ctx->hier[h].ml.size()) {
@@ -3858,10 +3872,108 @@
          ctx->cfg.w_inverse == ALFD_W_DIAGONAL && F.mask && F.A->present && F.C->present && plain_form(ctx, *F.Ct);
 }
 
-static int aug_tail(alfd_ctx *ctx, const AugOp &F, int mode, const AugTailArgs &p, double vec_bytes) {
+
+constexpr size_t kVsTailLdsLimit = 20 * 1024;
+
+static bool tail_in_form(alfd_ctx *ctx, const DevCsr &A, const DevCsr &Ct, int64_t npad) {
+  if (!A.present || A.sparse || A.n_list == 0 || A.nrows > npad || A.nrows > INT32_MAX) return false;
+  if (!(A.vs.on && ctx->vs_enable && !ctx->vi_off) || A.vs.L != 64 || A.vs.NW != 4 || A.vs.nb <= 0) return false;
+  if ((size_t)(A.vs.wide ? VsFmt<1>::kWinOff : VsFmt<0>::kWinOff) + (size_t)A.vs.tail_lds > kVsTailLdsLimit) return false;
+  if (!Ct.present || 2 * Ct.n_list >= A.nrows) return false;
+  return vs_lds_base_ok(ctx);
+}
+
+static bool tail_in_ok(alfd_ctx *ctx, const AugOp &F) {
+  return ctx->ml_tail_in_spmv && fused_ok(ctx, F) && F.cd2 && F.z2 && !a32_active(ctx, *F.A) &&
+         tail_in_form(ctx, *F.A, *F.Ct, F.npad);
+}
+
+static int tail_outputs(int mode, const AugTailArgs &p, const double *out[3]) {
+  int n = 0;
+  if (mode == TAIL_STEP || mode == TAIL_RES || (mode == TAIL_RES_INIT && p.store_res)) out[n++] = p.res;
+  if (mode == TAIL_STEP) out[n++] = p.d;
+  if (mode == TAIL_STEP || mode == TAIL_LAST || mode == TAIL_RES_INIT) out[n++] = p.z;
+  if (mode == TAIL_LAST_ADD || mode == TAIL_RES_INIT_ADD) out[n++] = p.zout;
+  return n;
+}
+static bool tail_writes(int mode, const AugTailArgs &p, const double *y, const double *x) {
+  const double *out[3];
+  const int n = tail_outputs(mode, p, out);
+  bool hit = y == x;
+  for (int i = 0; i < n; ++i) hit = hit || out[i] == x;
+  return hit;
+}
+
+static int launch_vs_tail(alfd_ctx *ctx, const AugOp &F, const double *x, double *y, int mode, AugTailArgs p, double vec_bytes) {
+  const DevCsr &A = *F.A;
+  if (mode < TAIL_STEP || mode > TAIL_RES_INIT) return ctx->err = "tail mode without a block-end epilogue", ALFD_E_INVALID;
+  if (!tail_in_form(ctx, A, *F.Ct, F.npad) || !F.mask) return ctx->err = "operator without the block-end epilogue", ALFD_E_UNSUPPORTED;
+  if (!p.zin) p.zin = p.z;
+  if (tail_writes(mode, p, y, x))
+    return ctx->err = "block-end epilogue: an output vector is the vector the product reads", ALFD_E_INVALID;
+  const DevCsr::Vs &v = A.vs;
+  const bool pair = F.C && !v.wide && pair_ok(ctx, A, *F.C) == 1;
+  const bool vi = !ctx->vi_off, vs = ctx->vs_enable != 0 && !ctx->vi_off;
+  const double ew = (vec_bytes - 16.0) * (double)A.nrows;
+  const size_t lds = (size_t)(v.wide ? VsFmt<1>::kWinOff : VsFmt<0>::kWinOff) + (size_t)v.tail_lds;
+  VsTail ta;
+  ta.p = p;
+  ta.mask = F.mask;
+  {
+    Timer tm(ctx, F.clsA, A.algorithmic_bytes() + (pair ? F.C->algorithmic_bytes() : 0.0) + ew,
+             A.streamed_bytes(vi, vs) + (pair ? F.C->streamed_bytes(vi, vs) : 0.0) + ew);
+    PairC pc{};
+    if (pair) {
+      const DevCsr &C = *F.C;
+      pc.nrows = C.n_list, pc.rp = C.rp, pc.col = C.col, pc.val = C.val, pc.x_halo = C.halo, pc.d = F.w, pc.t = F.tlam;
+      pc.n_local = C.n_local_cols, pc.L = C.L;
+      pc.nA = (uint32_t)v.nb;
+      const int64_t rpb = 256 / C.L;
+      pc.nC = (uint32_t)std::max<int64_t>(1, std::min<int64_t>((C.n_list + rpb - 1) / rpb, 256 * 8));
+    }
+    const unsigned grid = (unsigned)v.nb + (pair ? pc.nC : 0u);
+    note_spmv(ctx, ALFD_SPMV_BATCH_MAJOR, 64, 4, v.wide ? 1 : 0, false, 0, ctx->vs_xcd, grid, lds);
+#define ALFD_VS_TAIL_ARGS \
+  v.stream, v.tab, v.stride, v.hdrb, v.segx, v.seg_stride, v.dict, x, A.halo, A.n_local_cols, y, 0.0, (const double *)nullptr, \
+      (double *)nullptr, ctx->vs_xcd, 0
+#define ALFD_VS_TAIL(TAG, TM)                                                                                               \
+  do {                                                                                                                      \
+    if (v.wide)                                                                                                             \
+      hipLaunchKernelGGL((spmv_vs_kernel<0, TAG, 4, 1, false, TM>), dim3(grid), dim3(256), lds, ctx->stream,                \
+                         ALFD_VS_TAIL_ARGS, NoPair(), ta);                                                                  \
+    else if (pair)                                                                                                          \
+      hipLaunchKernelGGL((spmv_vs_kernel<0, TAG, 4, 0, true, TM>), dim3(grid), dim3(256), lds, ctx->stream,                 \
+                         ALFD_VS_TAIL_ARGS, pc, ta);                                                                        \
+    else                                                                                                                    \
+      hipLaunchKernelGGL((spmv_vs_kernel<0, TAG, 4, 0, false, TM>), dim3(grid), dim3(256), lds, ctx->stream,                \
+                         ALFD_VS_TAIL_ARGS, NoPair(), ta);                                                                  \
+  } while (0)
+#define ALFD_VS_TAIL_M(TAG)                                             \
+  switch (mode) {                                                       \
+    case TAIL_STEP: ALFD_VS_TAIL(TAG, TAIL_STEP); break;                \
+    case TAIL_LAST: ALFD_VS_TAIL(TAG, TAIL_LAST); break;                \
+    case TAIL_LAST_ADD: ALFD_VS_TAIL(TAG, TAIL_LAST_ADD); break;        \
+    case TAIL_RES: ALFD_VS_TAIL(TAG, TAIL_RES); break;                  \
+    default: ALFD_VS_TAIL(TAG, TAIL_RES_INIT); break;                   \
+  }
+    if (A.tag == 0) ALFD_VS_TAIL_M(0)
+    else ALFD_VS_TAIL_M(1)
+#undef ALFD_VS_TAIL_M
+#undef ALFD_VS_TAIL
+#undef ALFD_VS_TAIL_ARGS
+    HIPC(hipGetLastError());
+    ++ctx->fused_tail_launches;
+    if (pair || !F.C) return ALFD_OK;
+  }
+  return spmv_m(ctx, *F.C, ALFD_T_SPMV_OTHER, x, F.tlam, 2, 0.0, F.w);
+}
+
+static int aug_tail(alfd_ctx *ctx, const AugOp &F, int mode, AugTailArgs p, double vec_bytes, bool rows_only = false) {
   const DevCsr &m = *F.Ct;
+  if (!p.zin) p.zin = p.z;
+  if (rows_only) vec_bytes = 0.0;
   const int nb_rows = m.n_list > 0 ? grid_for_rows(m.n_list, m.L) : 0;
-  const unsigned grid = (unsigned)nb_rows + (unsigned)(F.npad / kChunk);
+  const unsigned grid = (unsigned)nb_rows + (rows_only ? 0u : (unsigned)(F.npad / kChunk));
   if (grid == 0) return ALFD_OK;
   Timer tm(ctx, ALFD_T_SPMV_OTHER, m.algorithmic_bytes() + vec_bytes * (double)F.npad,
            m.streamed_bytes(false) + vec_bytes * (double)F.npad);
@@ -3890,19 +4002,34 @@
   return ALFD_OK;
 }
 
+static int aug_op_tail(alfd_ctx *ctx, const AugOp &F, const double *x, double *y, int mode, AugTailArgs p, double vec_bytes) {
+  p.y = y;
+  if (!p.zin) p.zin = p.z;
+  if (x && mode <= TAIL_RES_INIT && tail_in_ok(ctx, F) && !tail_writes(mode, p, y, x)) {
+    RC(launch_vs_tail(ctx, F, x, y, mode, p, vec_bytes));
+    return aug_tail(ctx, F, mode, p, vec_bytes, true);
+  }
+  if (x) RC(fused_AC(ctx, F, x, y));
+  return aug_tail(ctx, F, mode, p, vec_bytes);
+}
+
 static int cheb_fused(alfd_ctx *ctx, const AugOp &F, int degree, double ratio, const double *r, double *z, double *zout,
                       bool have_init) {
   ChebCoef k(F.lmax, ratio);
   if (!have_init) VEC_LAUNCH(cheb_init_z_kernel, F.npad, 24, 1.0 / k.theta, F.dinv, r, z);
+  const bool pingpong = tail_in_ok(ctx, F);
+  const double *zc = z, *dc = z;
   for (int j = 1; j < degree; ++j) {
-    RC(fused_AC(ctx, F, j == 1 ? z : F.cd, F.ctmp));
     AugTailArgs p;
     k.step(p.c1, p.c2);
     p.gamma = F.gamma;
-    p.dinv = F.dinv, p.y = F.ctmp, p.rin = j == 1 ? r : F.cres, p.din = j == 1 ? z : F.cd;
-    p.res = F.cres, p.d = F.cd, p.z = z, p.zout = zout;
     const bool last = j == degree - 1;
-    RC(aug_tail(ctx, F, !last ? TAIL_STEP : zout ? TAIL_LAST_ADD : TAIL_LAST, p, last && zout ? 88.0 : 64.0));
+    p.dinv = F.dinv, p.rin = j == 1 ? r : F.cres, p.din = dc, p.zin = zc;
+    p.res = F.cres, p.zout = zout;
+    p.d = pingpong && dc == F.cd ? F.cd2 : F.cd;
+    p.z = pingpong && !last && dc == z ? F.z2 : z;
+    RC(aug_op_tail(ctx, F, dc, F.ctmp, !last ? TAIL_STEP : zout ? TAIL_LAST_ADD : TAIL_LAST, p, last && zout ? 88.0 : 64.0));
+    dc = p.d, zc = p.z;
   }
   HIPC(hipGetLastError());
   return ALFD_OK;
@@ -3914,21 +4041,34 @@
                     [&](const double *x, double *y) { return aug_apply(ctx, F, x, y); });
 }
 
-static int fused_residual(alfd_ctx *ctx, const AugOp &F, const double *r, double *t) {
+static int fused_residual(alfd_ctx *ctx, const AugOp &F, const double *x, const double *r, double *t) {
   AugTailArgs p;
-  p.gamma = F.gamma, p.y = t, p.rin = r, p.res = t;
-  return aug_tail(ctx, F, TAIL_RES, p, 24.0);
-}
-
-static int fused_correct(alfd_ctx *ctx, const AugOp &F, int degree, double ratio, const double *r, double *t, double *zc,
-                         double *zout) {
+  p.gamma = F.gamma, p.rin = r, p.res = t;
+  return aug_op_tail(ctx, F, x, t, TAIL_RES, p, 24.0);
+}
+
+static int fused_correct(alfd_ctx *ctx, const AugOp &F, int degree, double ratio, const double *x, const double *r, double *t,
+                         double *zc, double *zout) {
   AugTailArgs p;
   p.gamma = F.gamma, p.c1 = 1.0 / ChebCoef(F.lmax, ratio).theta;
-  p.dinv = F.dinv, p.y = t, p.rin = r, p.res = t, p.z = zc, p.zout = zout;
+  p.dinv = F.dinv, p.rin = r, p.res = t, p.z = zc, p.zout = zout;
   p.store_res = degree > 1;
-  if (degree <= 1 && zout) return aug_tail(ctx, F, TAIL_RES_INIT_ADD, p, 24.0 + 32.0 + 24.0);
-  RC(aug_tail(ctx, F, TAIL_RES_INIT, p, 24.0 + (degree > 1 ? 40.0 : 32.0)));
+  if (degree <= 1 && zout) return aug_op_tail(ctx, F, x, t, TAIL_RES_INIT_ADD, p, 24.0 + 32.0 + 24.0);
+  RC(aug_op_tail(ctx, F, x, t, TAIL_RES_INIT, p, 24.0 + (degree > 1 ? 40.0 : 32.0)));
   return cheb_fused(ctx, F, degree, ratio, t, zc, zout, true);
+}
+
+static int build_tail_vectors(alfd_ctx *ctx, int h, int l) {
+  MlLevel &L = ctx->hier[h].ml[l];
+  L.tail_z2 = L.tail_d2 = nullptr;
+  const AugOp F = level_view(ctx, h, l).op;
+  const bool form = L.tail_mask && ctx->nranks == 1 && tail_in_form(ctx, *F.A, *F.Ct, F.npad);
+  if (ctx->cfg.log_level > 0 || std::getenv("ALFD_LOG_UPLOAD"))
+    std::fprintf(stderr, "[alfd] hierarchy %d level %d (%lld rows, %lld in Ct): tails inside the A launch %s\n", h, l,
+                 (long long)F.A->nrows, (long long)F.Ct->n_list, form ? "possible" : "not possible");
+  if (!form) return ALFD_OK;
+  RC(cp_alloc_zero(ctx, h, &L.tail_z2, F.npad));
+  return cp_alloc_zero(ctx, h, &L.tail_d2, F.npad);
 }
 
 static int build_tail_mask(alfd_ctx *ctx, int h, const DevCsr &m, int64_t npad, uint8_t **mask) {
@@ -4036,8 +4176,7 @@
   const bool fuse = fused_ok(ctx, F);
   RC(aug_cheb(ctx, F, sdeg, c.ml_smooth_ratio, r, z));
   if (fuse) {
-    RC(fused_AC(ctx, F, z, L.t));
-    RC(fused_residual(ctx, F, r, L.t));
+    RC(fused_residual(ctx, F, z, r, L.t));
   } else {
     RC(aug_apply(ctx, F, z, L.t));
     VEC_LAUNCH(sub_from_kernel, F.npad, 24, r, L.t);
@@ -4053,8 +4192,7 @@
     RC(spmv_m(ctx, *L.P, ALFD_T_SPMV_OTHER, L.zc, z, 1, 1.0));
   }
   if (fuse) {
-    RC(fused_AC(ctx, F, z, L.t));
-    RC(fused_correct(ctx, F, sdeg, c.ml_smooth_ratio, r, L.t, L.r, z));
+    RC(fused_correct(ctx, F, sdeg, c.ml_smooth_ratio, z, r, L.t, L.r, z));
     return ALFD_OK;
   }
   RC(aug_apply(ctx, F, z, L.t));
@@ -4124,7 +4262,7 @@
   if (pen) RC(spmv_AC(ctx, Q.As, ALFD_T_SPMV_OTHER, ctx->mat[ALFD_C], w, z, Q.uS, ctx->t_lam));
   else RC(spmv_m(ctx, Q.As, ALFD_T_SPMV_OTHER, z, Q.uS, 0));
   if (fused_ok(ctx, F)) {
-    RC(fused_correct(ctx, F, pdeg, pratio, Q.rS, Q.uS, Q.eS, nullptr));
+    RC(fused_correct(ctx, F, pdeg, pratio, nullptr, Q.rS, Q.uS, Q.eS, nullptr));
   } else {
     if (pen) RC(spmv_m(ctx, Q.Cts, ALFD_T_SPMV_OTHER, ctx->t_lam, Q.uS, 1, ctx->cfg.gamma));
     VEC_LAUNCH(sub_from_kernel, Q.mpad, 24, Q.rS, Q.uS);
@@ -6202,7 +6340,10 @@
     ctx->ml_rep_level = rep_from;
   }
   for (int l = 0; l <= nlev; ++l)
+  {
     RC(build_tail_mask(ctx, 0, l == 0 ? ctx->mat[ALFD_CT] : ctx->hier[0].ml[l].loc.Ct, ctx->hier[0].ml[l].loc.npad, &ctx->hier[0].ml[l].tail_mask));
+    RC(build_tail_vectors(ctx, 0, l));
+  }
   return ALFD_OK;
 }
 
@@ -6250,7 +6391,10 @@
     RC(coarse_inverse(ctx, H.coarse_A, H.coarse_C, H.coarse_Ct, w, c.gamma2, H.inv));
   }
   for (int l = 0; l <= nlev; ++l)
+  {
     RC(build_tail_mask(ctx, 1, l == 0 ? ctx->mat[ALFD_M] : H.ml[l].loc.Ct, H.ml[l].loc.npad, &H.ml[l].tail_mask));
+    RC(build_tail_vectors(ctx, 1, l));
+  }
   return build_tail_table(ctx);
 }
 
@@ -6808,6 +6952,7 @@
   if (const char *e = std::getenv("ALFD_ML_REPLICATE")) ctx->ml_rep_threshold = std::atoll(e);
   if (const char *e = std::getenv("ALFD_ML_GPU_GALERKIN")) ctx->ml_gpu_galerkin = std::atoi(e);
   if (const char *e = std::getenv("ALFD_ML_FUSE")) ctx->ml_fuse = std::max(0, std::min(3, std::atoi(e)));
+  if (const char *e = std::getenv("ALFD_ML_TAIL_IN_SPMV")) ctx->ml_tail_in_spmv = std::atoi(e) != 0 ? 1 : 0;
   if (const char *e = std::getenv("ALFD_SPMV_VI_LEVELS")) ctx->vi_levels = std::atoi(e);
   if (const char *e = std::getenv("ALFD_SPMV_BATCH_MAJOR")) ctx->vs_enable = std::atoi(e);
   if (const char *e = std::getenv("ALFD_SPMV_BATCH_MAJOR_ROWS")) ctx->vs_RB = std::max(4, std::min(kVsMaxRows, std::atoi(e)));
@@ -8180,6 +8325,104 @@
   return rc;
 }
 
+int alfd_get_fused_tail_launches(alfd_ctx_t ctx, int64_t *count) {
+  CHECK_CTX();
+  if (!count) return ALFD_E_INVALID;
+  *count = ctx->fused_tail_launches;
+  return ALFD_OK;
+}
+
+int alfd_spmv_tail_step(alfd_ctx_t ctx, int slot_a, int form, const alfd_tail_step *s) {
+  CHECK_CTX();
+  if (!s || (form != 0 && form != 1) || slot_a < 0 || slot_a >= ALFD_NSLOTS || !ctx->mat[slot_a].present) return ALFD_E_INVALID;
+  if (s->slot_c >= ALFD_NSLOTS || (s->slot_c >= 0 && (!ctx->mat[s->slot_c].present || !s->w))) return ALFD_E_INVALID;
+  if (s->mode < TAIL_STEP || s->mode > TAIL_RES_INIT_ADD || !s->x || !s->y || !s->t || !s->rin || !s->ct_rp) return ALFD_E_INVALID;
+  DevCsr &A = ctx->mat[slot_a];
+  DevCsr *Cm = s->slot_c >= 0 ? &ctx->mat[s->slot_c] : nullptr;
+  const int64_t n = A.nrows, nt = s->ct_ncols;
+  if (s->ct_nrows != n || nt < 1 || (Cm && (Cm->nrows != nt || Cm->ncols != A.ncols))) return ALFD_E_INVALID;
+  const int mode = s->mode;
+  const bool step = mode <= TAIL_LAST_ADD, add = mode == TAIL_LAST_ADD || mode == TAIL_RES_INIT_ADD;
+  const double *outs[3];
+  AugTailArgs hp;
+  hp.dinv = s->dinv, hp.rin = s->rin, hp.din = s->din, hp.zin = s->zin;
+  hp.res = s->res, hp.d = s->d, hp.z = s->z, hp.zout = s->zout, hp.store_res = s->store_res;
+  const int nout = tail_outputs(mode, hp, outs);
+  for (int i = 0; i < nout; ++i)
+    if (!outs[i]) return ALFD_E_INVALID;
+  if ((mode != TAIL_RES && !s->dinv) || (step && (!s->din || !s->zin))) return ALFD_E_INVALID;
+  if (ctx->nranks != 1 || ctx->cfg.w_inverse != ALFD_W_DIAGONAL || ctx->cfg.aug_assembled || gd_nested(ctx))
+    return ctx->err = "alfd_spmv_tail_step: one rank, the diagonal W^-1 and the factored operator", ALFD_E_UNSUPPORTED;
+  static const int32_t no_col = 0;
+  static const double no_val = 0;
+  const bool empty = s->ct_rp[n] == 0;
+  RC(upload_matrix(ctx, kScratchSlot, n, nt, s->ct_rp, empty ? &no_col : s->ct_col, empty ? &no_val : s->ct_val));
+  DevCsr Ct = std::move(ctx->mat[kScratchSlot]);
+  ctx->mat[kScratchSlot] = DevCsr();
+  const int64_t npad = pad_chunk(n);
+  struct Img { const double *h; double *d; int64_t len; bool out; };
+  std::vector<Img> img;
+  int rc = ALFD_OK;
+  auto dev = [&](const double *h, int64_t len, bool out) -> double * {
+    if (!h) return nullptr;
+    for (Img &g : img)
+      if (g.h == h) return g.out = g.out || out, g.d;
+    const int64_t cap = std::max<int64_t>(std::max(len, npad), 1);
+    double *d = nullptr;
+    if (hipMalloc((void **)&d, cap * sizeof(double)) != hipSuccess) return rc = ALFD_E_HIP, nullptr;
+    hipMemsetAsync(d, 0, cap * sizeof(double), ctx->stream);
+    hipMemcpyAsync(d, h, len * sizeof(double), hipMemcpyHostToDevice, ctx->stream);
+    img.push_back(Img{h, d, len, out});
+    return d;
+  };
+  AugOp F;
+  F.A = &A, F.C = Cm, F.Ct = &Ct;
+  F.clsA = slot_a == ALFD_A ? ALFD_T_SPMV_A : ALFD_T_SPMV_OTHER;
+  F.gamma = s->gamma, F.npad = npad;
+  const double *dx = dev(s->x, A.ncols, false);
+  double *dy = dev(s->y, n, true);
+  F.tlam = dev(s->t, nt, Cm != nullptr);
+  F.w = Cm ? dev(s->w, nt, false) : nullptr;
+  AugTailArgs p;
+  p.gamma = s->gamma, p.c1 = s->c1, p.c2 = s->c2, p.store_res = s->store_res;
+  p.rin = dev(s->rin, n, false);
+  if (mode != TAIL_RES) p.dinv = dev(s->dinv, n, false);
+  if (step) p.din = dev(s->din, n, false), p.zin = dev(s->zin, n, false);
+  p.res = dev(s->res, n, true), p.d = dev(s->d, n, true), p.z = dev(s->z, n, true), p.zout = dev(s->zout, n, true);
+  p.y = dy;
+  uint8_t *mask = nullptr;
+  if (rc == ALFD_OK && hipMalloc((void **)&mask, (size_t)npad) != hipSuccess) rc = ALFD_E_HIP;
+  if (rc == ALFD_OK) {
+    hipMemsetAsync(mask, 0, (size_t)npad, ctx->stream);
+    if (Ct.n_list > 0)
+      hipLaunchKernelGGL(mark_rows_kernel, dim3((unsigned)((Ct.n_list + 255) / 256)), dim3(256), 0, ctx->stream, Ct.n_list,
+                         Ct.sparse ? Ct.rows : (const int32_t *)nullptr, mask);
+    F.mask = mask;
+    if (!plain_form(ctx, Ct))
+      rc = (ctx->err = "alfd_spmv_tail_step: Ct is not resident as plain CSR rows", ALFD_E_UNSUPPORTED);
+  }
+  if (rc == ALFD_OK) {
+    if (form == 0) {
+      rc = launch_vs_tail(ctx, F, dx, dy, mode, p, 0.0);
+      if (rc == ALFD_OK) rc = aug_tail(ctx, F, mode, p, 0.0, true);
+    } else {
+      rc = Cm ? spmv_AC(ctx, A, F.clsA, *Cm, F.w, dx, dy, F.tlam) : spmv_m(ctx, A, F.clsA, dx, dy, 0);
+      if (rc == ALFD_OK) rc = aug_tail(ctx, F, mode, p, 0.0);
+    }
+  }
+  if (rc == ALFD_OK) {
+    for (const Img &g : img)
+      if (g.out) hipMemcpyAsync(const_cast<double *>(g.h), g.d, g.len * sizeof(double), hipMemcpyDeviceToHost, ctx->stream);
+    if (hipStreamSynchronize(ctx->stream) != hipSuccess) rc = ALFD_E_HIP;
+  } else {
+    hipStreamSynchronize(ctx->stream);
+  }
+  for (const Img &g : img) hipFree(g.d);
+  hipFree(mask);
+  csr_free(Ct);
+  return rc;
+}
+
 int alfd_inner_prec_apply(alfd_ctx_t ctx, int op, const double *r, double *z) {
   CHECK_CTX();
   CHECK_SETUP();
@@ -9017,6 +9260,11 @@
     ctx->ml_fuse = std::max(0, std::min(3, value));
     return ALFD_OK;
   }
+  if (std::strcmp(name, "ml_tail_in_spmv") == 0) {
+    if (value != 0 && value != 1) return ctx->err = "ml_tail_in_spmv: 0 or 1", ALFD_E_INVALID;
+    ctx->ml_tail_in_spmv = value;
+    return ALFD_OK;
+  }
   if (std::strcmp(name, "ml_gpu_galerkin") == 0) {
     if (value != 0 && value != 1) return ctx->err = "ml_gpu_galerkin: 0 or 1", ALFD_E_INVALID;
     ctx->ml_gpu_galerkin = value;
diff --git a/fictitious_domain_al_preconditioners_amd/csrc/kernels.hpp b/fictitious_domain_al_preconditioners_amd/csrc/kernels.hpp
--- a/fictitious_domain_al_preconditioners_amd/csrc/kernels.hpp
+++ b/fictitious_domain_al_preconditioners_amd/csrc/kernels.hpp
@@ -1141,7 +1141,7 @@
 enum { TAIL_STEP = 0, TAIL_LAST = 1, TAIL_LAST_ADD = 2, TAIL_RES = 3, TAIL_RES_INIT = 4, TAIL_RES_INIT_ADD = 5 };
 struct AugTailArgs {
   double gamma = 0, c1 = 0, c2 = 0;
-  const double *dinv = nullptr, *y = nullptr, *rin = nullptr, *din = nullptr;
+  const double *dinv = nullptr, *y = nullptr, *rin = nullptr, *din = nullptr, *zin = nullptr;
   double *res = nullptr, *d = nullptr, *z = nullptr, *zout = nullptr;
   int store_res = 0;
 };
@@ -1164,7 +1164,7 @@
 __device__ __forceinline__ void aug_tail_elem(const AugTailArgs &p, int64_t i, double y) {
   constexpr bool kStep = MODE <= TAIL_LAST_ADD, kAdd = MODE == TAIL_LAST_ADD || MODE == TAIL_RES_INIT_ADD;
   const double dinv = MODE != TAIL_RES ? p.dinv[i] : 0.0, rin = p.rin[i];
-  const double din = kStep ? p.din[i] : 0.0, zin = kStep ? p.z[i] : 0.0, zo = kAdd ? p.zout[i] : 0.0;
+  const double din = kStep ? p.din[i] : 0.0, zin = kStep ? p.zin[i] : 0.0, zo = kAdd ? p.zout[i] : 0.0;
   double res, d = 0.0, z = 0.0, zout = 0.0;
   aug_tail_math<MODE>(p, y, dinv, rin, din, zin, zo, res, d, z, zout);
   if (MODE == TAIL_STEP || MODE == TAIL_RES || (MODE == TAIL_RES_INIT && p.store_res)) p.res[i] = res;
@@ -1214,7 +1214,7 @@
     const double2 zero = {0.0, 0.0};
     const double2 yv = ld2(p.y, i), rv = ld2(p.rin, i);
     const double2 dv = MODE != TAIL_RES ? ld2(p.dinv, i) : zero;
-    const double2 dd = kStep ? ld2(p.din, i) : zero, zi = kStep ? ld2(p.z, i) : zero;
+    const double2 dd = kStep ? ld2(p.din, i) : zero, zi = kStep ? ld2(p.zin, i) : zero;
     const double2 zo = kAdd ? ld2(p.zout, i) : zero;
     double2 res, d = zero, z = zero, zout = zero;
     aug_tail_math<MODE>(p, yv.x, dv.x, rv.x, dd.x, zi.x, zo.x, res.x, d.x, z.x, zout.x);
diff --git a/fictitious_domain_al_preconditioners_amd/csrc/kernels_vs.hpp b/fictitious_domain_al_preconditioners_amd/csrc/kernels_vs.hpp
--- a/fictitious_domain_al_preconditioners_amd/csrc/kernels_vs.hpp
+++ b/fictitious_domain_al_preconditioners_amd/csrc/kernels_vs.hpp
@@ -120,14 +120,38 @@
   }
 }
 
-template <int EPI, int TAG, int NW, int WD = 0, bool PAIR = false>
+struct VsTail {
+  AugTailArgs p;
+  const uint8_t *mask;
+};
+struct NoTail {};
+inline __host__ __device__ int32_t vs_tail_lds_need(int32_t dict_region, int32_t nd, int32_t W, int32_t nbatch) {
+  const int32_t gap = (dict_region - 8 * nd) >> 7;
+  return 8 * W + 128 * (nbatch > gap ? nbatch - gap : 0);
+}
+template <int TM>
+using TailArg = typename std::conditional<(TM >= 0), VsTail, NoTail>::type;
+
+__device__ __forceinline__ void vs_lds_store_f64(uint32_t byte_off, double v) {
+  *(__attribute__((address_space(3))) double *)(uintptr_t)byte_off = v;
+}
+template <int TM>
+__device__ __forceinline__ void vs_tail_row(const NoTail &, int32_t, double, double *) {}
+template <int TM>
+__device__ __forceinline__ void vs_tail_row(const VsTail &t, int32_t r, double v, double *y) {
+  if (t.mask[r]) y[r] = v;
+  else aug_tail_elem<TM>(t.p, r, v);
+}
+
+template <int EPI, int TAG, int NW, int WD = 0, bool PAIR = false, int TM = -1>
 __global__ __launch_bounds__(64 * NW) __attribute__((amdgpu_waves_per_eu(8, 8))) void spmv_vs_kernel(
     const uint8_t *__restrict__ stream, const uint64_t *__restrict__ tab, int32_t stride,
     const int32_t *__restrict__ hdrb, const int32_t *__restrict__ segx, int32_t seg_stride,
     const double *__restrict__ dict, const double *__restrict__ x, const double *__restrict__ x_halo,
     int32_t n_local, double *__restrict__ y, double alpha, const double *__restrict__ d, double *__restrict__ y2,
-    int xcd_remap, int32_t block_base, PairArg<PAIR> pc) {
+    int xcd_remap, int32_t block_base, PairArg<PAIR> pc, TailArg<TM> ta) {
   static_assert(!PAIR || NW <= 4, "the second party needs a lane group of 64 within 64 NW <= kBlock threads");
+  static_assert(TM < 0 || EPI == 0, "the block-end epilogue consumes y = A x");
   if (pair_rows<64 * NW>(pc, x)) return;
   extern __shared__ double xs[];
   char *sm = (char *)xs;
@@ -189,9 +213,13 @@
   __syncthreads();
   const int q16 = lane >> 4;
   const int rsel = 4 * (2 * ((((q16 & 1) << 1) | (q16 >> 1)) + 4 * ((lane >> 3) & 1) + 8 * ((lane >> 2) & 1)) + 1);
-  auto store = [&](double s, int32_t r, bool mine) {
+  const int32_t rgap = (VsFmt<WD>::kWinOff - 8 * nd) >> 7;
+  const uint32_t rlow = 8u * (uint32_t)nd, rhigh = VsFmt<WD>::kWinOff + 8u * (uint32_t)W - 128u * (uint32_t)rgap;
+  auto store = [&](double s, int32_t r, bool mine, int32_t bi) {
     if (mine && r >= 0) {
-      if (EPI == 0)
+      if (TM >= 0)
+        vs_lds_store_f64((bi < rgap ? rlow : rhigh) + 128u * (uint32_t)bi + (uint32_t)rsel - 4u, s);
+      else if (EPI == 0)
         y[r] = s;
       else if (EPI == 1)
         y[r] = fma(alpha, s, y[r]);
@@ -284,7 +312,7 @@
       }
       n0 = hdr(hn, 0);
       n1 = hdr(hn, 1);
-      store(reduce_rows4(acc[0], acc[1], acc[2], acc[3]), (int32_t)__builtin_amdgcn_ds_bpermute(rsel, (int)hc), (lane & 15) == 0);
+      store(reduce_rows4(acc[0], acc[1], acc[2], acc[3]), (int32_t)__builtin_amdgcn_ds_bpermute(rsel, (int)hc), (lane & 15) == 0, bi);
       mstep = 0;
     }
     int32_t rid = -1;
@@ -296,12 +324,22 @@
     }
     if (bi + NW < nbatch && (int32_t)n1 < 0) vs_shared_fetch(n0, sbase, lane, w);
     hc = hdr_load(bi + 2 * NW);
-    if (mstep) store(sres, rid, (lane & (mstep - 1)) == 0);
+    if (mstep) store(sres, rid, (lane & (mstep - 1)) == 0, bi);
   };
   for (int32_t bi = wave; bi < nbatch; bi += 2 * NW) {
     batch(hv1, hv2, bi);
     if (bi + NW >= nbatch) break;
     batch(hv2, hv1, bi + NW);
+  }
+  if constexpr (TM >= 0) {
+    __syncthreads();
+    int32_t s0 = 64 * wave + lane;
+    asm volatile("" : "+v"(s0));
+    for (int32_t s = s0; s < 16 * nbatch; s += 64 * NW) {
+      const uint32_t rd = tb[2 * s + 1];
+      const int32_t r = (s & 15) ? (int32_t)rd : (int32_t)(rd & 0x7fffffffu);
+      if (r >= 0) vs_tail_row<TM>(ta, r, vs_lds_f64(((s >> 4) < rgap ? rlow : rhigh) + 8u * (uint32_t)s), y);
+    }
   }
 }
 
diff --git a/fictitious_domain_al_preconditioners_amd/solver.py b/fictitious_domain_al_preconditioners_amd/solver.py
--- a/fictitious_domain_al_preconditioners_amd/solver.py
+++ b/fictitious_domain_al_preconditioners_amd/solver.py
@@ -40,6 +40,7 @@
     "alfd_setup_coupling", "alfd_get_setup_counts",
     "alfd_set_preconditioner_values", "alfd_get_preconditioner_values", "alfd_spmv_preconditioner",
     "alfd_bench_spmv_preconditioner",
+    "alfd_spmv_tail_step", "alfd_get_fused_tail_launches",
 ]
 
 
@@ -92,6 +93,8 @@
         "alfd_spmv_scaled": (C.c_int, [vp, C.c_int, vp, vp, vp, vp]),
         "alfd_spmv_pair": (C.c_int, [vp, C.c_int, C.c_int, vp, vp, vp, vp]),
         "alfd_get_last_spmv_launch": (C.c_int, [vp, C.POINTER(_abi.SpmvLaunch)]),
+        "alfd_spmv_tail_step": (C.c_int, [vp, C.c_int, C.c_int, C.POINTER(_abi.TailStep)]),
+        "alfd_get_fused_tail_launches": (C.c_int, [vp, C.POINTER(C.c_int64)]),
         "alfd_dot": (C.c_int, [vp, i64, vp, vp, C.POINTER(dbl)]),
         "alfd_inner_prec_apply": (C.c_int, [vp, C.c_int, vp, vp]),
         "alfd_matrix_lanes": (C.c_int, [vp, C.c_int, C.POINTER(i32)]),
@@ -536,6 +539,51 @@
                                           t.ctypes.data))
         return y, t
 
+    def fused_tail_launches(self):
+        out = C.c_int64()
+        self._ck(self._lib.alfd_get_fused_tail_launches(self._h, C.byref(out)))
+        return out.value
+
+    def spmv_tail_step(self, slot_a, form, mode, ct, x, t, *, gamma=0.0, c1=0.0, c2=0.0, store_res=0, slot_c=-1,
+                       w=None, **vecs):
+        rp, col, val, ncols = ct
+        rp = np.ascontiguousarray(rp, np.int64)
+        col = np.ascontiguousarray(col, np.int32)
+        val = np.ascontiguousarray(val, np.float64)
+        x = np.ascontiguousarray(x, np.float64).copy()
+        t = np.ascontiguousarray(t, np.float64).copy()
+        s = _abi.TailStep()
+        s.mode, s.store_res, s.slot_c = int(mode), int(store_res), int(slot_c)
+        s.gamma, s.c1, s.c2 = float(gamma), float(c1), float(c2)
+        s.ct_nrows, s.ct_ncols = rp.size - 1, int(ncols)
+        s.ct_rp, s.ct_col, s.ct_val = rp.ctypes.data, col.ctypes.data, val.ctypes.data
+        s.x, s.t = x.ctypes.data, t.ctypes.data
+        keep = [rp, col, val, x, t]
+        if w is not None:
+            w = np.ascontiguousarray(w, np.float64)
+            keep.append(w)
+            s.w = w.ctypes.data
+        out, named = {}, {}
+        for name in ("dinv", "rin", "din", "zin", "y", "res", "d", "z", "zout"):
+            v = vecs.pop(name, None)
+            if v is None:
+                continue
+            if isinstance(v, str):
+                a = x if v == "x" else named[v]
+            else:
+                a = np.ascontiguousarray(v, np.float64).copy()
+            keep.append(a)
+            named[name] = a
+            setattr(s, name, a.ctypes.data)
+            if name in ("y", "res", "d", "z", "zout"):
+                out[name] = a
+        if vecs:
+            raise TypeError(f"unknown vectors {sorted(vecs)}")
+        self._ck(self._lib.alfd_spmv_tail_step(self._h, int(slot_a), int(form), C.byref(s)))
+        if slot_c >= 0:
+            out["t"] = t
+        return out
+
     def last_spmv_launch(self):
         rec = _abi.SpmvLaunch()
         self._ck(self._lib.alfd_get_last_spmv_launch(self._h, C.byref(rec)))
diff --git a/include/alfd/alfd.h b/include/alfd/alfd.h
--- a/include/alfd/alfd.h
+++ b/include/alfd/alfd.h
@@ -259,6 +259,20 @@
 int alfd_spmv(alfd_ctx_t ctx, int slot, const double *x, double *y, int mode, double alpha);
 int alfd_spmv_scaled(alfd_ctx_t ctx, int slot, const double *x, const double *d, double *y, double *y2);
 int alfd_spmv_pair(alfd_ctx_t ctx, int slot_a, int slot_c, const double *x, const double *d, double *y, double *t);
+typedef struct alfd_tail_step {
+  int32_t mode, store_res, slot_c, reserved;
+  double gamma, c1, c2;
+  int64_t ct_nrows, ct_ncols;
+  const int64_t *ct_rp;
+  const int32_t *ct_col;
+  const double *ct_val;
+  const double *x, *w;
+  double *t;
+  const double *dinv, *rin, *din, *zin;
+  double *y, *res, *d, *z, *zout;
+} alfd_tail_step;
+int alfd_spmv_tail_step(alfd_ctx_t ctx, int slot_a, int form, const alfd_tail_step *s);
+int alfd_get_fused_tail_launches(alfd_ctx_t ctx, int64_t *count);
 enum alfd_spmv_family {
   ALFD_SPMV_PLAIN = 0,
   ALFD_SPMV_SPARSE_ROWS = 1,
```

New measurement: 16.66, median of 6. 3.1% higher.
